# OpenDriveLab/Vista

Hardware: NVIDIA H100
Metric: denoised frames/sec at 25x576x1024, 50 EDM steps; UNet step ms (higher is better)
Workload: dtype f16 (fp32 accumulate, fp32 norms/softmax/sampler state)

## Files before the change

### include/vista_b200.h

```cpp
#ifndef VISTA_B200_H
#define VISTA_B200_H

#include <stdint.h>

#ifdef __cplusplus
extern "C" {
#endif

const char* b200v_last_error(void);
int b200v_version(void);
int b200v_device_info(int32_t* sm_count, int32_t* cc_major, int32_t* cc_minor);

typedef struct b200v_gemm_desc {
  const void* a;
  int64_t lda;
  int64_t tokens;
  int32_t a_mode;
  int32_t W, H, NB;
  int32_t box_w, box_h, box_b;
  int32_t cin;
  int32_t ntaps;
  int32_t dh[9];
  int32_t dw[9];
  const void* b;
  int32_t N;
  int32_t tile_n;
  int32_t bf16;
  void* out;
  int64_t ldo;
  int32_t out_f32;
  int32_t act;
  const float* bias;
  const float* rowvec;
  int64_t ld_rowvec;
  int32_t rv_div, rv_mod;
  const void* res1;
  int64_t ld_res1;
  float s_res1;
  const void* res2;
  int64_t ld_res2;
  float s_res2;
  float s_acc;
  float* stats;
  int64_t stats_ld;
  int32_t stats_col0;
  int32_t h_pad;
} b200v_gemm_desc;

int b200v_gemm(const b200v_gemm_desc* d, void* stream);

int b200v_groupnorm_from_partials(const float* partials, int64_t stats_ld, int32_t n_stats, int32_t frames_per_stat,
                                  int32_t tokens_per_frame, int32_t C, int32_t groups, float eps, float* mean_rstd,
                                  double* raw_sums, void* stream);

int b200v_attention_spatial_v3(const void* q, int64_t ld_q, const void* k, int64_t ld_k, const void* v, int64_t ld_v,
                               void* out, int64_t ld_o, int32_t frames, int32_t seq, int32_t heads, void* stream);


int b200v_attention_spatial_v7(const void* q, int64_t ld_q, const void* k, int64_t ld_k, const void* v, int64_t ld_v,
                               void* out, int64_t ld_o, int32_t frames, int32_t seq, int32_t heads, void* stream);

int b200v_attention_temporal(const void* q, int64_t ld_q, const void* k, int64_t ld_k, const void* v, int64_t ld_v,
                             void* out, int64_t ld_o, int32_t nb, int32_t T, int32_t S, int32_t heads, void* stream);

int b200v_attention_temporal_sharded(const void* q, int64_t ld_q, const void* k, int64_t ld_k, const void* v, int64_t ld_v,
                                     void* out, int64_t ld_o, int32_t nb, int32_t Tq, int32_t T, int32_t S, int32_t heads,
                                     const int64_t* kv_frame_tok, void* stream);

int b200v_groupnorm_chunk(void);
int b200v_groupnorm_chunk_for(int32_t frames, int32_t tokens_per_frame);
int b200v_groupnorm_stats(const void* x, int64_t ldx, int32_t frames, int32_t tokens_per_frame, int32_t C,
                          int32_t groups, int32_t frames_per_stat, float eps, double* partials, int32_t* counters,
                          float* mean_rstd, void* stream);
int b200v_groupnorm_apply(const void* x, int64_t ldx, void* y, int64_t ldy, int32_t frames, int32_t tokens_per_frame,
                          int32_t C, int32_t groups, int32_t frames_per_stat, const float* mean_rstd, const float* gamma,
                          const float* beta, int32_t silu, void* stream);

int b200v_groupnorm_sums(const void* x, int64_t ldx, int32_t frames, int32_t tokens_per_frame, int32_t C, int32_t groups,
                         int32_t frames_per_stat, double* partials, int32_t* counters, double* sums, void* stream);
int b200v_groupnorm_finalize(const double* sums, int32_t n_stat_groups, double count, float eps, float* mean_rstd,
                             void* stream);

int b200v_layernorm(const void* x, int64_t ldx, void* y, int64_t ldy, int64_t tokens, int32_t C, const float* gamma,
                    const float* beta, float eps, const float* addvec, int64_t ld_addvec, int32_t av_div,
                    int32_t av_mod, void* stream);

int b200v_conv3x3_small_cin(const void* x, int32_t cin, const float* w , const float* bias,
                            void* out, int64_t ldo, int32_t NB, int32_t H, int32_t W, int32_t cout, void* stream);
int b200v_conv3x3_small_cout(const void* x, int64_t ldx, int32_t cin, const float* w ,
                             const float* bias, float* out , int32_t NB, int32_t H, int32_t W,
                             int32_t cout, void* stream);

int b200v_im2col_s2(const void* x, int64_t ldx, void* out, int32_t NB, int32_t H, int32_t W, int32_t C, void* stream);
int b200v_im2col_s2_asym(const void* x, int64_t ldx, void* out, int32_t NB, int32_t H, int32_t W, int32_t C, void* stream);
int b200v_upsample2x(const void* x, int64_t ldx, void* out, int64_t ldo, int32_t NB, int32_t H, int32_t W, int32_t C,
                     void* stream);

int b200v_timestep_embedding(const float* t, int32_t n, int32_t dim, float max_period, void* out_f16, int64_t ldo,
                             void* stream);
int b200v_blend_emb(const float* e_plain, const float* e_cond, const float* label, const float* mask, float* emb_f32,
                    void* silu_emb_f16, int32_t rows, int32_t dim, void* stream);

int b200v_sampler_prepare(float* x, const float* cond_frame, const float* mask,
                          const float* concat_u ,
                          const float* concat_c , const float* sigmas, const int32_t* step_idx,
                          void* unet_in_f16 , int64_t ld_in,
                          float* c_noise, int32_t T, int32_t h, int32_t w, void* stream);
int b200v_sampler_update(float* x, const float* net_out ,
                         int64_t ld_net, const float* cond_frame, const float* mask, const float* scales , const float* sigmas, int32_t* step_idx,
                         int32_t num_steps, int32_t T, int32_t h, int32_t w, void* stream);

int b200v_softmax_rows(const float* x, int64_t ld_in, void* y_f16, int64_t ld_out, int64_t rows, int32_t cols,
                       void* stream);
int b200v_time_mix_small(const float* x , int64_t ldx,
                         const float* w , const float* bias,
                         float* out , const int32_t* blend, int32_t T, int32_t HW, int32_t C,
                         int32_t out_frame0, int32_t skip_frames, void* stream);

int b200v_time_mix_small_u8(const float* x, int64_t ldx, const float* w, const float* bias, float* out, uint8_t* out_u8,
                            const int32_t* blend, int32_t T, int32_t HW, int32_t C, int32_t out_frame0,
                            int32_t skip_frames, int32_t keep_f32_from, void* stream);
int b200v_rollout_advance(float* sample, const float* z0, float* samples_z, float* filled, int32_t T, int64_t frame_elems,
                          int32_t dst_frame0, int32_t src_frame0, int32_t n_cond, void* stream);
int b200v_ensemble_reward_scratch(void);
int b200v_ensemble_reward(const float* const* members_dev, int32_t K, int64_t n, double* partial, uint32_t* ticket,
                          float* out2, void* stream);

int b200v_peer_alloc(int64_t bytes, void** ptr, void* handle64);
int b200v_peer_open(const void* handle64, void** ptr);
int b200v_peer_close(void* ptr);
int b200v_peer_free(void* ptr);
int b200v_peer_allreduce_max(void);
int b200v_peer_allreduce_f64(double* data, int32_t n, void* const* windows_dev, int64_t slot_off, int64_t flag_off, int32_t rank,
                             int32_t world, uint32_t* counter, void* stream);
int b200v_peer_put(const void* src, int64_t src_pitch, int64_t rows, int64_t row_bytes, void* const* dsts_dev, int64_t dst_pitch,
                   uint32_t* const* flags_dev, int32_t n_dst, uint32_t* counter, uint32_t* ticket, void* stream);
int b200v_peer_wait(const uint32_t* const* flags_dev, int32_t n, uint32_t* counter, void* stream);

int b200v_clip_preprocess(const float* x, int32_t n, int32_t H, int32_t W, int32_t antialias, void* out, int64_t ldo,
                          int32_t out_f32, void* stream);
int b200v_attention_d80(const void* q, int64_t ld_q, const void* k, int64_t ld_k, const void* v, int64_t ld_v, void* out,
                        int64_t ld_o, int32_t batch, int32_t seq, int32_t heads, void* stream);

int b200v_nchw_to_tokens(const float* x, void* out_f16, int64_t ldo, int32_t NB, int32_t C, int32_t H, int32_t W,
                         void* stream);
int b200v_tokens_to_nchw(const void* x, int32_t x_is_f32, int64_t ldx, float* out, int32_t NB, int32_t C, int32_t H,
                         int32_t W, void* stream);

#ifdef __cplusplus
}
#endif
#endif
```

### vista_b200/clip.py

```python
from __future__ import annotations

import os
from typing import Dict, Optional, Union

import torch
import torch.nn as nn

from . import ops
from .diffusion import instantiate_from_config
from .modules import register_param_tree
from .spec import CLIP_TEXT_LEFTOVERS, ClipConfig, clip_param_specs, clip_preset
from .unet import Lin


class ClipRuntime:

    def __init__(self, cfg: ClipConfig, sd: Dict[str, torch.Tensor], device, prefix: str = "model.visual."):
        assert cfg.patch_size == 14 and cfg.image_size == 224 and cfg.head_width == 80, \
            "the native tower is the 224 px, patch 14, head width 80 ViT"
        self.cfg, self.dev, self.prefix = cfg, torch.device(device), prefix
        self._bufs = {}
        self._sd = sd
        self._pack()
        self._sd = None

    def _t(self, name, dtype=torch.float32):
        return self._sd[self.prefix + name].detach().to(self.dev, dtype).contiguous()

    def _lin(self, w: torch.Tensor, b: Optional[torch.Tensor]) -> Lin:
        return Lin(w.to(torch.float16).contiguous(), b, ops.pick_tile_n(w.shape[0]))

    def _norm(self, p):
        return self._t(f"{p}.weight"), self._t(f"{p}.bias")

    def _pack(self):
        cfg, C = self.cfg, self.cfg.width
        w = self._t("conv1.weight").reshape(C, cfg.patch_k)
        wp = torch.zeros(C, cfg.patch_k_pad, dtype=torch.float32, device=self.dev)
        wp[:, :cfg.patch_k] = w
        self.patch = self._lin(wp, None)
        tok = self._t("positional_embedding").clone()
        tok[0] += self._t("class_embedding")
        self.tok_rowvec = tok.contiguous()
        self.ln_pre = self._norm("ln_pre")
        self.blocks = []
        for i in range(cfg.layers):
            p = f"transformer.resblocks.{i}"
            self.blocks.append(dict(
                ln1=self._norm(f"{p}.ln_1"),
                qkv=self._lin(self._t(f"{p}.attn.in_proj_weight"), self._t(f"{p}.attn.in_proj_bias")),
                out=self._lin(self._t(f"{p}.attn.out_proj.weight"), self._t(f"{p}.attn.out_proj.bias")),
                ln2=self._norm(f"{p}.ln_2"),
                fc=self._lin(self._t(f"{p}.mlp.c_fc.weight"), self._t(f"{p}.mlp.c_fc.bias")),
                proj=self._lin(self._t(f"{p}.mlp.c_proj.weight"), self._t(f"{p}.mlp.c_proj.bias"))))
        self.ln_post = self._norm("ln_post")
        self.proj = self._lin(self._t("proj").t(), None)

    def buf(self, name, rows, cols, dtype=torch.float16):
        key = (name, rows, cols, dtype)
        t = self._bufs.get(key)
        if t is None:
            t = self._bufs[key] = torch.empty(rows, cols, dtype=dtype, device=self.dev)
        return t

    def gemm(self, a, lin: Lin, out, **kw):
        return ops.gemm(a, lin.w, out, bias=lin.b, tile_n=lin.tile_n, **kw)

    def forward(self, x: torch.Tensor, antialias: bool = True) -> torch.Tensor:
        cfg, C = self.cfg, self.cfg.width
        n, L = x.shape[0], cfg.tokens
        M = n * L
        rows = ops.clip_preprocess(x.float().contiguous(), self.buf("c.patch", M, cfg.patch_k_pad), antialias)
        x0 = self.gemm(rows, self.patch, self.buf("c.x1", M, C), rowvec=self.tok_rowvec, rv_mod=L)
        xa = ops.layernorm(x0, self.buf("c.x0", M, C), *self.ln_pre, eps=cfg.ln_eps)
        xb = self.buf("c.x1", M, C)
        h = self.buf("c.h", M, C)
        qkv = self.buf("c.qkv", M, 3 * C)
        o = self.buf("c.o", M, C)
        f = self.buf("c.f", M, cfg.mlp_width)
        for B in self.blocks:
            ops.layernorm(xa, h, *B["ln1"], eps=cfg.ln_eps)
            self.gemm(h, B["qkv"], qkv)
            ops.attention_d80(qkv[:, :C], qkv[:, C:2 * C], qkv[:, 2 * C:], o, n, L, cfg.heads)
            self.gemm(o, B["out"], xb, res1=xa)
            ops.layernorm(xb, h, *B["ln2"], eps=cfg.ln_eps)
            self.gemm(h, B["fc"], f, act=3)
            self.gemm(f, B["proj"], xa, res1=xb)
        cls = self.buf("c.cls", n, C)
        ops.layernorm(xa.view(n, L * C)[:, :C], cls, *self.ln_post, eps=cfg.ln_eps)
        return self.gemm(cls, self.proj, self.buf("c.emb", n, cfg.embed_dim, torch.float32))


class FrozenOpenCLIPImageEmbedder(nn.Module):

    def __init__(self, arch: Union[str, ClipConfig] = "ViT-H-14", version: str = "laion2b_s32b_b79k", device: str = "cuda",
                 max_length: int = 77, freeze: bool = True, antialias: bool = True, ucg_rate: float = 0.0,
                 unsqueeze_dim: bool = False, repeat_to_max_len: bool = False, num_image_crops: int = 0,
                 output_tokens: bool = False, init_device=None):
        super().__init__()
        bad = [k for k, v in dict(arch=not (arch == "ViT-H-14" or isinstance(arch, ClipConfig)), ucg_rate=ucg_rate != 0.0,
                                  num_image_crops=num_image_crops != 0, output_tokens=bool(output_tokens),
                                  unsqueeze_dim=bool(unsqueeze_dim), repeat_to_max_len=bool(repeat_to_max_len)).items() if v]
        if bad:
            raise NotImplementedError(f"vista_b200.clip.FrozenOpenCLIPImageEmbedder: unsupported option(s) {bad}")
        self.b200_config = arch if isinstance(arch, ClipConfig) else clip_preset("vit_h_14")
        self.model = nn.Module()
        self.model.visual = nn.Module()
        register_param_tree(self.model.visual, clip_param_specs(self.b200_config))
        self.device, self.max_length = device, max_length
        self.antialias, self.ucg_rate = antialias, ucg_rate
        self.is_trainable, self.input_key = False, None
        if freeze:
            self.requires_grad_(False)
        self._runtime = None
        self._register_load_state_dict_pre_hook(self._drop_text_leftovers)
        self.register_load_state_dict_post_hook(lambda module, keys: setattr(module, "_runtime", None))

    @staticmethod
    def _drop_text_leftovers(state_dict, prefix, *args):
        for k in CLIP_TEXT_LEFTOVERS:
            state_dict.pop(prefix + "model." + k, None)

    def _apply(self, fn, *args, **kwargs):
        before = tuple((p.device, p.dtype) for p in self.parameters())
        out = super()._apply(fn, *args, **kwargs)
        if tuple((p.device, p.dtype) for p in self.parameters()) != before:
            self._runtime = None
        return out

    def runtime(self, device) -> ClipRuntime:
        if torch.device(device).type != "cuda":
            raise RuntimeError("vista_b200 runs on CUDA (sm_90a) only; there is no CPU fallback")
        if self._runtime is None or self._runtime.dev != torch.device(device):
            self._runtime = ClipRuntime(self.b200_config, self.state_dict(), device)
        return self._runtime

    @torch.no_grad()
    def forward(self, image: torch.Tensor, no_dropout: bool = False):
        if image.dim() == 5:
            raise NotImplementedError("multi-crop input (num_image_crops > 0) is not supported")
        return self.runtime(image.device).forward(image, self.antialias).to(image.dtype)

    def encode(self, image):
        return self(image)


class FrozenOpenCLIPImagePredictionEmbedder(nn.Module):

    def __init__(self, open_clip_embedding_config: Dict, n_cond_frames: int, n_copies: int):
        super().__init__()
        self.n_cond_frames, self.n_copies = n_cond_frames, n_copies
        self.open_clip = instantiate_from_config(open_clip_embedding_config)
        self.is_trainable, self.ucg_rate, self.input_key = False, 0.0, None

    def forward(self, vid: torch.Tensor) -> torch.Tensor:
        z = self.open_clip(vid)
        z = z.reshape(-1, self.n_cond_frames, z.shape[-1])
        return z.repeat_interleave(self.n_copies, dim=0)


def load_open_clip_weights(path: str, prefix: str = "model.") -> Dict[str, torch.Tensor]:
    if not os.path.isfile(path):
        raise FileNotFoundError(path)
    if path.endswith(".safetensors"):
        from safetensors.torch import load_file
        sd = load_file(path)
    else:
        sd = torch.load(path, map_location="cpu", weights_only=True)
        sd = sd.get("state_dict", sd)
    return {prefix + k: v for k, v in sd.items() if not k.startswith("transformer.")}
```

### vista_b200/csrc/gemm_tc.cu

```cuda
#include "gemm_tc.cuh"

namespace vb {
extern template const GemmKern* gemm_variants<32>();
extern template const GemmKern* gemm_variants<64>();
extern template const GemmKern* gemm_variants<96>();
extern template const GemmKern* gemm_variants<128>();
extern template const GemmKern* gemm_variants<160>();
extern template const GemmKern* gemm_variants<192>();
extern template const GemmKern* gemm_variants<224>();
extern template const GemmKern* gemm_variants<256>();
}

extern "C" int b200v_gemm(const b200v_gemm_desc* d, void* stream_) {
  using namespace vb;
  cudaStream_t stream = reinterpret_cast<cudaStream_t>(stream_);
  VB_REQUIRE(d && d->a && d->b && d->out, "b200v_gemm: null pointer");
  VB_REQUIRE(d->cin > 0 && d->cin % 64 == 0, "b200v_gemm: cin=%d must be a positive multiple of 64", d->cin);
  VB_REQUIRE(d->ntaps >= 1 && d->ntaps <= 9, "b200v_gemm: ntaps=%d out of range", d->ntaps);
  VB_REQUIRE(d->N > 0 && d->N % 8 == 0, "b200v_gemm: N=%d must be a multiple of 8", d->N);
  VB_REQUIRE(d->tile_n >= 32 && d->tile_n <= 256 && d->tile_n % 32 == 0, "b200v_gemm: tile_n=%d invalid", d->tile_n);
  VB_REQUIRE(d->lda % 8 == 0 && d->ldo % 8 == 0, "b200v_gemm: lda/ldo must be multiples of 8");
  VB_REQUIRE(d->act >= 0 && d->act <= 3, "b200v_gemm: act=%d invalid", d->act);
  VB_REQUIRE(!(d->act == 2 && (d->tile_n % 64 != 0 || d->N % d->tile_n != 0 || d->out_f32)),
             "b200v_gemm: GEGLU needs tile_n %% 64 == 0, N %% tile_n == 0, 16-bit output");
  VB_REQUIRE(!(d->act == 2 && (d->rowvec || d->res1 || d->res2)), "b200v_gemm: GEGLU epilogue takes bias only");
  VB_REQUIRE(!(d->act == 3 && (d->rowvec || d->res1 || d->res2 || d->bf16 || d->out_f32 || d->stats || getenv("VB_GEMM_GENERIC"))),
             "b200v_gemm: the GELU epilogue takes bias only, fp16 operands and output (compiled variant)");
  VB_REQUIRE(!d->res1 || d->ld_res1 % 8 == 0, "b200v_gemm: ld_res1 must be a multiple of 8");
  VB_REQUIRE(!d->res2 || d->ld_res2 % 8 == 0, "b200v_gemm: ld_res2 must be a multiple of 8");
  VB_REQUIRE(!d->rowvec || (d->ld_rowvec % 4 == 0 && d->rv_div > 0 && d->rv_mod > 0), "b200v_gemm: bad rowvec args");
  VB_REQUIRE((reinterpret_cast<uintptr_t>(d->a) & 15) == 0 && (reinterpret_cast<uintptr_t>(d->b) & 15) == 0 &&
                 (reinterpret_cast<uintptr_t>(d->out) & 15) == 0,
             "b200v_gemm: a/b/out must be 16-byte aligned");

  TGParams p;
  memset(&p, 0, sizeof(p));
  p.a_mode = d->a_mode;
  p.tokens = d->tokens;
  const long long K = (long long)d->ntaps * d->cin;
  CUtensorMap tmA, tmB;
  if (d->a_mode == 0) {
    VB_REQUIRE(d->ntaps == 1 && d->h_pad == 0, "b200v_gemm: linear mode takes one tap and no halo rows");
    VB_REQUIRE(d->tokens > 0 && d->tokens < (1ll << 31) - 256, "b200v_gemm: tokens out of range");
    p.W = (int)d->tokens; p.H = 1; p.NB = 1;
    p.BW = 128; p.BH = 1; p.BB = 1;
    p.tiles_w = (int)((d->tokens + 127) / 128); p.tiles_h = 1;
    p.m_tiles = p.tiles_w;
    uint64_t dims[2] = {(uint64_t)d->cin, (uint64_t)d->tokens};
    uint64_t strides[1] = {(uint64_t)d->lda * 2};
    uint32_t box[2] = {64, 128};
    uint32_t es[2] = {1, 1};
    if (encode_tmap_16bit(&tmA, d->a, 2, dims, strides, box, es, d->bf16)) return 3;
  } else {
    VB_REQUIRE(d->W > 0 && d->H > 0 && d->NB > 0 && (long long)d->W * d->H * d->NB == d->tokens &&
                   d->tokens < (1ll << 31) - 256,
               "b200v_gemm: W*H*NB != tokens (or >= 2^31)");
    VB_REQUIRE(d->box_w > 0 && d->box_h > 0 && d->box_b > 0 && d->box_w * d->box_h * d->box_b == 128,
               "b200v_gemm: box_w*box_h*box_b must be 128");
    p.W = d->W; p.H = d->H; p.NB = d->NB;
    p.BW = d->box_w; p.BH = d->box_h; p.BB = d->box_b;
    p.tiles_w = (d->W + p.BW - 1) / p.BW;
    p.tiles_h = (d->H + p.BH - 1) / p.BH;
    const int tiles_b = (d->NB + p.BB - 1) / p.BB;
    p.m_tiles = p.tiles_w * p.tiles_h * tiles_b;
    VB_REQUIRE(d->h_pad >= 0 && d->h_pad <= 4, "b200v_gemm: h_pad=%d out of range", d->h_pad);
    const uint64_t He = (uint64_t)d->H + 2ull * d->h_pad;
    uint64_t dims[4] = {(uint64_t)d->cin, (uint64_t)d->W, He, (uint64_t)d->NB};
    uint64_t strides[3] = {(uint64_t)d->lda * 2, (uint64_t)d->lda * 2 * d->W, (uint64_t)d->lda * 2 * d->W * He};
    uint32_t box[4] = {64, (uint32_t)p.BW, (uint32_t)p.BH, (uint32_t)p.BB};
    uint32_t es[4] = {1, 1, 1, 1};
    if (encode_tmap_16bit(&tmA, d->a, 4, dims, strides, box, es, d->bf16)) return 3;
  }
  {
    uint64_t dims[2] = {(uint64_t)K, (uint64_t)d->N};
    uint64_t strides[1] = {(uint64_t)K * 2};
    uint32_t box[2] = {64, (uint32_t)d->tile_n};
    uint32_t es[2] = {1, 1};
    if (encode_tmap_16bit(&tmB, d->b, 2, dims, strides, box, es, d->bf16)) return 3;
  }
  p.ntaps = d->ntaps;
  p.kc_per_tap = d->cin / 64;
  for (int i = 0; i < 9; ++i) {
    p.dh[i] = d->dh[i] + (d->a_mode == 1 ? d->h_pad : 0);
    p.dw[i] = d->dw[i];
  }
  p.N = d->N;
  p.n_tiles = (d->N + d->tile_n - 1) / d->tile_n;
  p.stage_bytes = kABytes + ((d->tile_n * 128 + 1023) / 1024) * 1024;
  constexpr int kMaxSmem = 227 * 1024;
  p.nstages = (kMaxSmem - 2048 - kStagingBytes) / p.stage_bytes;
  if (p.nstages > kMaxStages) p.nstages = kMaxStages;
  const long long kMaxLd = (1ll << 31) - 1;
  VB_REQUIRE(d->ldo * (d->out_f32 ? 4 : 2) <= kMaxLd && d->ld_rowvec * 4 <= kMaxLd && d->ld_res1 * 2 <= kMaxLd &&
                 d->ld_res2 * 2 <= kMaxLd,
             "b200v_gemm: row stride too large");
  for (p.bw_sh = 0; (1 << p.bw_sh) < p.BW; ++p.bw_sh) {}
  for (p.bh_sh = 0; (1 << p.bh_sh) < p.BH; ++p.bh_sh) {}
  p.out = d->out; p.ldo_b = (int)(d->ldo * (d->out_f32 ? 4 : 2)); p.out_f32 = d->out_f32; p.act = d->act;
  p.bias = d->bias;
  p.rowvec = d->rowvec; p.ld_rowvec_b = (int)(d->ld_rowvec * 4); p.rv_div = d->rv_div > 0 ? d->rv_div : 1;
  p.rv_mod = d->rv_mod > 0 ? d->rv_mod : 1;
  p.res1 = d->res1; p.ld_res1_b = (int)(d->ld_res1 * 2); p.s_res1 = d->s_res1;
  p.res2 = d->res2; p.ld_res2_b = (int)(d->ld_res2 * 2); p.s_res2 = d->s_res2;
  p.s_acc = d->s_acc;
  VB_REQUIRE(!(d->res2 && !d->res1), "b200v_gemm: res2 without res1");
  p.stats = d->stats; p.stats_ld = (int)d->stats_ld; p.stats_col0 = d->stats_col0;
  if (d->stats) {
    VB_REQUIRE(!d->bf16 && !d->out_f32 && d->act == 0 && !d->res2 && !(d->rowvec && d->res1),
               "b200v_gemm: fused statistics need fp16 output, act 0, <= 1 residual and no rowvec + residual");
    VB_REQUIRE(d->stats_ld >= d->stats_col0 + d->N && d->stats_col0 % 4 == 0 && d->stats_ld % 4 == 0 &&
                   (reinterpret_cast<uintptr_t>(d->stats) & 15) == 0,
               "b200v_gemm: bad stats_ld / stats_col0 / alignment");
    VB_REQUIRE(d->a_mode == 0 || (p.BB == 1 && d->W % p.BW == 0 && d->H % p.BH == 0 && (p.BW == d->W || p.BH == 1)),
               "b200v_gemm: fused statistics need token tiles of 128 consecutive tokens (box %d x %d x %d on %d x %d)",
               p.BW, p.BH, p.BB, d->W, d->H);
  }

  const int smem_bytes = 1024 + 1024 + p.nstages * p.stage_bytes + kStagingBytes;
  int variant = d->bf16 ? 12 : 7;
  if (d->stats) {
    variant = 9 + (d->rowvec ? 2 : (d->res1 ? 1 : 0));
  } else if (!d->bf16 && !d->out_f32 && !getenv("VB_GEMM_GENERIC")) {
    const int nres = (d->res1 ? 1 : 0) + (d->res2 ? 1 : 0);
    if (d->act == 0 && !d->rowvec) variant = nres;
    else if (d->act == 0 && nres <= 1) variant = 3 + nres;
    else if (d->act == 1 && !d->rowvec && nres == 0) variant = 5;
    else if (d->act == 2) variant = 6;
    else if (d->act == 3) variant = 8;
  }
  static const GemmKern* const kByWidth[8] = {gemm_variants<32>(),  gemm_variants<64>(),  gemm_variants<96>(),
                                              gemm_variants<128>(), gemm_variants<160>(), gemm_variants<192>(),
                                              gemm_variants<224>(), gemm_variants<256>()};
  static bool attr_set[64] = {false};
  if (vb::first_use_on_device(attr_set)) {
    for (int w = 0; w < 8; ++w)
      for (int i = 0; i < kGemmVariants; ++i)
        VB_CHECK_CUDA(cudaFuncSetAttribute(kByWidth[w][i], cudaFuncAttributeMaxDynamicSharedMemorySize, kMaxSmem));
  }
  const long long total = (long long)p.m_tiles * p.n_tiles;
  int grid = device_sm_count();
  if (total < grid) grid = (int)total;
  const GemmKern k = kByWidth[d->tile_n / 32 - 1][variant];
  k<<<grid, kGemmThreads, smem_bytes, stream>>>(tmA, tmB, p);
  VB_CHECK_CUDA(cudaGetLastError());
  return 0;
}
```

### vista_b200/csrc/gemm_tc.cuh

```cuda
#pragma once
#include "../../include/vista_b200.h"
#include "host.cuh"
#include "ptx.cuh"

namespace vb {

constexpr int kMaxStages = 8;
constexpr int kABytes = 128 * 64 * 2;
constexpr int kStageBufBytes = 64 * 32 * 4;
constexpr int kStagingBytes = 2 * 2 * kStageBufBytes;
constexpr int kGemmThreads = 384;

struct TGParams {
  int a_mode;
  int W, H, NB;
  int BW, BH, BB;
  int bw_sh, bh_sh;
  int tiles_w, tiles_h;
  int m_tiles, n_tiles;
  int ntaps, kc_per_tap;
  int dh[9], dw[9];
  int N;
  int nstages, stage_bytes;
  long long tokens;
  void* out;
  int ldo_b;
  int out_f32, act;
  const float* bias;
  const float* rowvec;
  int ld_rowvec_b;
  int rv_div, rv_mod;
  const void* res1;
  int ld_res1_b;
  float s_res1;
  const void* res2;
  int ld_res2_b;
  float s_res2;
  float s_acc;
  float* stats;
  int stats_ld, stats_col0;
};

__device__ __forceinline__ float2 unpack2(uint32_t w, int bf16) {
  if (bf16) return make_float2(__uint_as_float(w << 16), __uint_as_float(w & 0xFFFF0000u));
  return __half22float2(*reinterpret_cast<const __half2*>(&w));
}
__device__ __forceinline__ uint32_t pack2(float a, float b, int bf16) {
  if (bf16) {
    __nv_bfloat162 t = __floats2bfloat162_rn(a, b);
    return *reinterpret_cast<uint32_t*>(&t);
  }
  __half2 t = __floats2half2_rn(a, b);
  return *reinterpret_cast<uint32_t*>(&t);
}

template <int TN, bool BF16>
__device__ __forceinline__ void issue_kchunk(float (&acc)[TN / 2], uint64_t adesc, uint64_t bdesc, bool overwrite) {
#pragma unroll
  for (int kk = 0; kk < 4; ++kk)
    wgmma_ss<TN, BF16>(acc, adesc + (uint64_t)(2 * kk), bdesc + (uint64_t)(2 * kk), (overwrite && kk == 0) ? 0 : 1);
}

template <int TN, int ACT_, bool RV_, int NRES_, bool GEN, bool STATS = false, bool BF16 = false>
__global__ void __launch_bounds__(kGemmThreads, 1)
tapgemm_kernel(const __grid_constant__ CUtensorMap tmA, const __grid_constant__ CUtensorMap tmB, const TGParams p) {
  extern __shared__ uint8_t smem_raw[];
  const uint32_t raw = smem_u32(smem_raw);
  uint8_t* smem = smem_raw + (((raw + 1023u) & ~1023u) - raw);
  uint64_t* full = reinterpret_cast<uint64_t*>(smem);
  uint64_t* empty = full + kMaxStages;
  uint8_t* stages = smem + 1024;

  const int warp = threadIdx.x >> 5, lane = threadIdx.x & 31;
  const int KC = p.ntaps * p.kc_per_tap;
  const int total_tiles = p.m_tiles * p.n_tiles;

  if (threadIdx.x == 0) {
    for (int i = 0; i < p.nstages; ++i) {
      mbar_init(&full[i], 1);
      mbar_init(&empty[i], 8);
    }
    fence_barrier_init();
  }
  if (warp == 8 && lane == 0) {
    tma_prefetch_desc(&tmA);
    tma_prefetch_desc(&tmB);
  }
  __syncthreads();

  if (warp >= 8) {
    setmaxnreg_dec<40>();
    if (warp == 8 && lane == 0) {
      int stage = 0;
      uint32_t phase = 0;
      const uint32_t tx = (uint32_t)(kABytes + TN * 128);
      for (int tile = blockIdx.x; tile < total_tiles; tile += gridDim.x) {
        const int m_blk = tile / p.n_tiles, n_blk = tile - m_blk * p.n_tiles;
        const int tw = m_blk % p.tiles_w;
        const int th = (m_blk / p.tiles_w) % p.tiles_h;
        const int tb = m_blk / (p.tiles_w * p.tiles_h);
        const int w0 = tw * p.BW, h0 = th * p.BH, b0 = tb * p.BB;
        const int n0 = n_blk * TN;
        for (int kc = 0; kc < KC; ++kc) {
          mbar_wait_relaxed(&empty[stage], phase ^ 1, 1);
          uint8_t* sA = stages + stage * p.stage_bytes;
          uint8_t* sB = sA + kABytes;
          const int tap = kc / p.kc_per_tap;
          const int c0 = (kc - tap * p.kc_per_tap) * 64;
          mbar_expect_tx(&full[stage], tx);
          if (p.a_mode == 0)
            tma_load_2d(sA, &tmA, &full[stage], c0, w0);
          else
            tma_load_4d(sA, &tmA, &full[stage], c0, w0 + p.dw[tap], h0 + p.dh[tap], b0);
          tma_load_2d(sB, &tmB, &full[stage], kc * 64, n0);
          if (++stage == p.nstages) {
            stage = 0;
            phase ^= 1;
          }
        }
      }
    }
    return;
  }

  setmaxnreg_inc<232>();
  const int wg = warp >> 2, wq = warp & 3;
  const int act = GEN ? p.act : ACT_;
  const bool has_rv = GEN ? (p.rowvec != nullptr) : RV_;
  const bool has_r1 = GEN ? (p.res1 != nullptr) : (NRES_ >= 1);
  const bool has_r2 = GEN ? (p.res2 != nullptr) : (NRES_ >= 2);
  constexpr bool bf16 = BF16;
  const bool f32o = GEN ? (p.out_f32 != 0) : false;
  const bool has_bias = p.bias != nullptr;
  constexpr int half = TN >> 1;
  const int tile_out_cols = (act == 2) ? half : TN;
  const int n_out_total = (act == 2) ? (p.N >> 1) : p.N;
  const int G = tile_out_cols >> 5;
  const int out_es = f32o ? 4 : 2;
  const char* r1p = reinterpret_cast<const char*>(p.res1);
  const char* r2p = reinterpret_cast<const char*>(p.res2);
  const uint64_t desc0 = make_desc_sw128(smem_u32(stages), 16, 1024);
  const uint32_t stage_step = (uint32_t)p.stage_bytes >> 4;
  const uint32_t stg0 = smem_u32(stages + p.nstages * p.stage_bytes) + wg * 2 * kStageBufBytes;
  const int g = lane >> 2, c = lane & 3;
  const int rh = wq & 1, chh = wq >> 1;
  const int ch = lane & 3, rsub = lane >> 2;
  int stage = 0;
  uint32_t phase = 0;
  uint32_t gcount = 0;

  float acc[TN / 2];
  for (int tile = blockIdx.x; tile < total_tiles; tile += gridDim.x) {
    const int m_blk = tile / p.n_tiles, n_blk = tile - m_blk * p.n_tiles;
    int prev = -1;
    for (int kc = 0; kc < KC; ++kc) {
      mbar_wait(&full[stage], phase, 3);
      const uint64_t ad = desc0 + (uint64_t)(stage * stage_step + wg * 512);
      const uint64_t bd = desc0 + (uint64_t)(stage * stage_step + (kABytes >> 4));
      wgmma_fence();
      issue_kchunk<TN, BF16>(acc, ad, bd, kc == 0);
      wgmma_commit();
      if (prev >= 0) {
        wgmma_wait<1>();
        if (lane == 0) mbar_arrive(&empty[prev]);
      }
      prev = stage;
      if (++stage == p.nstages) {
        stage = 0;
        phase ^= 1;
      }
    }
    wgmma_wait<0>();
    if (lane == 0) mbar_arrive(&empty[prev]);
    fence_regs(acc);

    const int r_own = wg * 64 + rh * 32 + lane;
    int token_own, valid_own;
    if (p.a_mode == 0) {
      token_own = m_blk * 128 + r_own;
      valid_own = token_own < p.tokens;
    } else {
      const int tw = m_blk % p.tiles_w;
      const int t2 = m_blk / p.tiles_w;
      const int th = t2 % p.tiles_h;
      const int tb = t2 / p.tiles_h;
      const int ww = r_own & (p.BW - 1), hh = (r_own >> p.bw_sh) & (p.BH - 1), bb = r_own >> (p.bw_sh + p.bh_sh);
      const int w = tw * p.BW + ww, h = th * p.BH + hh, b = tb * p.BB + bb;
      valid_own = (w < p.W) && (h < p.H) && (b < p.NB);
      token_own = (b * p.H + h) * p.W + w;
    }
    if (!valid_own) token_own = 0;
    const uint32_t vrows = __ballot_sync(0xffffffffu, valid_own) >> rsub;
    int tok[4], rvrow[4];
    {
      const int rv_own = has_rv ? (token_own / p.rv_div) % p.rv_mod : 0;
#pragma unroll
      for (int i = 0; i < 4; ++i) {
        tok[i] = __shfl_sync(0xffffffffu, token_own, i * 8 + rsub);
        rvrow[i] = has_rv ? __shfl_sync(0xffffffffu, rv_own, i * 8 + rsub) : 0;
      }
    }
    const int n_out_base = n_blk * tile_out_cols;
#pragma unroll
    for (int k = 0; k < TN / 32; ++k) {
      if (k >= G) break;
      const int c0 = k * 32;
      if (n_out_base + c0 >= n_out_total) break;
      const uint32_t stg = stg0 + (gcount & 1) * kStageBufBytes;
      ++gcount;
      float f[16];
#pragma unroll
      for (int j = 0; j < 16; ++j) f[j] = acc[16 * k + j];
      if (act == 2) {
        float gt[16];
        const int kg = (half >> 5) + k;
#pragma unroll
        for (int j = 0; j < 16; ++j) gt[j] = 0.f;
#pragma unroll
        for (int q = 0; q < TN / 32; ++q)
          if (q == kg) {
#pragma unroll
            for (int j = 0; j < 16; ++j) gt[j] = acc[16 * q + j];
          }
        const int nb = n_blk * TN + c0;
#pragma unroll
        for (int ii = 0; ii < 4; ++ii) {
          float2 bv = make_float2(0.f, 0.f), bg = make_float2(0.f, 0.f);
          if (has_bias) {
            bv = __ldg(reinterpret_cast<const float2*>(p.bias + nb + 8 * ii + 2 * c));
            bg = __ldg(reinterpret_cast<const float2*>(p.bias + nb + half + 8 * ii + 2 * c));
          }
          f[4 * ii + 0] = geglu_fast(f[4 * ii + 0] + bv.x, gt[4 * ii + 0] + bg.x);
          f[4 * ii + 1] = geglu_fast(f[4 * ii + 1] + bv.y, gt[4 * ii + 1] + bg.y);
          f[4 * ii + 2] = geglu_fast(f[4 * ii + 2] + bv.x, gt[4 * ii + 2] + bg.x);
          f[4 * ii + 3] = geglu_fast(f[4 * ii + 3] + bv.y, gt[4 * ii + 3] + bg.y);
        }
      }
#pragma unroll
      for (int ii = 0; ii < 4; ++ii) {
        const int chunk = 2 * ii + (c >> 1), sub = (c & 1) * 8;
#pragma unroll
        for (int hr = 0; hr < 2; ++hr) {
          const int row = wq * 16 + g + 8 * hr;
          asm volatile("st.shared.v2.f32 [%0], {%1, %2};" ::"r"(stg + row * 128 + ((chunk ^ (row & 7)) << 4) + sub),
                       "f"(f[4 * ii + 2 * hr]), "f"(f[4 * ii + 2 * hr + 1])
                       : "memory");
        }
      }
      asm volatile("bar.sync %0, 128;" ::"r"(1 + wg) : "memory");
      {
        const int n = n_out_base + c0 + chh * 16 + ch * 4;
        const bool n_ok = n + 4 <= n_out_total;
        float4 bs = make_float4(0.f, 0.f, 0.f, 0.f);
        float sa = 1.0f;
        if (act != 2) {
          sa = p.s_acc;
          if (has_bias && n_ok) {
            const float4 b4 = __ldg(reinterpret_cast<const float4*>(p.bias + n));
            bs = make_float4(b4.x * sa, b4.y * sa, b4.z * sa, b4.w * sa);
          }
        }
        char* obase = reinterpret_cast<char*>(p.out) + (long long)n * out_es;
        const char* r1base = r1p + (long long)n * 2;
        const char* r2base = r2p + (long long)n * 2;
        const char* rvbase = reinterpret_cast<const char*>(p.rowvec) + (long long)n * 4;
        float cs[4] = {0.f, 0.f, 0.f, 0.f}, cq[4] = {0.f, 0.f, 0.f, 0.f};
        float4 v[4], rv[4];
        uint2 u1[4], u2[4];
#pragma unroll
        for (int i = 0; i < 4; ++i) {
          const int row = rh * 32 + i * 8 + rsub;
          const int chunk = chh * 4 + ch;
          asm volatile("ld.shared.v4.f32 {%0, %1, %2, %3}, [%4];"
                       : "=f"(v[i].x), "=f"(v[i].y), "=f"(v[i].z), "=f"(v[i].w)
                       : "r"(stg + row * 128 + ((chunk ^ (row & 7)) << 4)));
          const bool ok = n_ok && ((vrows >> (8 * i)) & 1u);
          rv[i] = make_float4(0.f, 0.f, 0.f, 0.f);
          u1[i] = make_uint2(0, 0);
          u2[i] = make_uint2(0, 0);
          if (has_rv && ok) rv[i] = __ldg(reinterpret_cast<const float4*>(rvbase + (long long)rvrow[i] * p.ld_rowvec_b));
          if (has_r1 && ok) u1[i] = __ldg(reinterpret_cast<const uint2*>(r1base + (long long)tok[i] * p.ld_res1_b));
          if (has_r2 && ok) u2[i] = __ldg(reinterpret_cast<const uint2*>(r2base + (long long)tok[i] * p.ld_res2_b));
        }
#pragma unroll
        for (int i = 0; i < 4; ++i) {
          const bool ok = n_ok && ((vrows >> (8 * i)) & 1u);
          float4 o = v[i];
          if (act != 2) {
            o.x = fmaf(o.x, sa, bs.x); o.y = fmaf(o.y, sa, bs.y); o.z = fmaf(o.z, sa, bs.z); o.w = fmaf(o.w, sa, bs.w);
            if (has_rv) { o.x += rv[i].x; o.y += rv[i].y; o.z += rv[i].z; o.w += rv[i].w; }
            if (act == 1) { o.x = silu_f(o.x); o.y = silu_f(o.y); o.z = silu_f(o.z); o.w = silu_f(o.w); }
            if (!GEN && act == 3) { o.x = gelu_erf_fast(o.x); o.y = gelu_erf_fast(o.y); o.z = gelu_erf_fast(o.z); o.w = gelu_erf_fast(o.w); }
            if (has_r1) {
              const float2 a = unpack2(u1[i].x, bf16), b = unpack2(u1[i].y, bf16);
              o.x = fmaf(p.s_res1, a.x, o.x); o.y = fmaf(p.s_res1, a.y, o.y);
              o.z = fmaf(p.s_res1, b.x, o.z); o.w = fmaf(p.s_res1, b.y, o.w);
            }
            if (has_r2) {
              const float2 a = unpack2(u2[i].x, bf16), b = unpack2(u2[i].y, bf16);
              o.x = fmaf(p.s_res2, a.x, o.x); o.y = fmaf(p.s_res2, a.y, o.y);
              o.z = fmaf(p.s_res2, b.x, o.z); o.w = fmaf(p.s_res2, b.y, o.w);
            }
          }
          if (STATS && ok) {
            cs[0] += o.x; cs[1] += o.y; cs[2] += o.z; cs[3] += o.w;
            cq[0] = fmaf(o.x, o.x, cq[0]); cq[1] = fmaf(o.y, o.y, cq[1]);
            cq[2] = fmaf(o.z, o.z, cq[2]); cq[3] = fmaf(o.w, o.w, cq[3]);
          }
          char* optr = obase + (long long)tok[i] * p.ldo_b;
          if (f32o) {
            if (ok) *reinterpret_cast<float4*>(optr) = o;
          } else {
            const uint2 pk = make_uint2(pack2(o.x, o.y, bf16), pack2(o.z, o.w, bf16));
            if (ok) *reinterpret_cast<uint2*>(optr) = pk;
          }
        }
        if (STATS) {
#pragma unroll
          for (int off = 4; off < 32; off <<= 1) {
#pragma unroll
            for (int q = 0; q < 4; ++q) {
              cs[q] += __shfl_xor_sync(0xffffffffu, cs[q], off);
              cq[q] += __shfl_xor_sync(0xffffffffu, cq[q], off);
            }
          }
          if (rsub == 0 && n_ok) {
            float* dst = p.stats + (((long long)m_blk * 4 + wg * 2 + rh) * p.stats_ld + p.stats_col0 + n) * 2;
            *reinterpret_cast<float4*>(dst) = make_float4(cs[0], cq[0], cs[1], cq[1]);
            *reinterpret_cast<float4*>(dst + 4) = make_float4(cs[2], cq[2], cs[3], cq[3]);
          }
        }
      }
    }
  }
}

using GemmKern = void (*)(const CUtensorMap, const CUtensorMap, const TGParams);
constexpr int kGemmVariants = 13;

template <int TN>
const GemmKern* gemm_variants() {
  static const GemmKern v[kGemmVariants] = {
      tapgemm_kernel<TN, 0, false, 0, false>,       tapgemm_kernel<TN, 0, false, 1, false>,
      tapgemm_kernel<TN, 0, false, 2, false>,       tapgemm_kernel<TN, 0, true, 0, false>,
      tapgemm_kernel<TN, 0, true, 1, false>,        tapgemm_kernel<TN, 1, false, 0, false>,
      tapgemm_kernel<TN, 2, false, 0, false>,       tapgemm_kernel<TN, 0, true, 2, true>,
      tapgemm_kernel<TN, 3, false, 0, false>,       tapgemm_kernel<TN, 0, false, 0, false, true>,
      tapgemm_kernel<TN, 0, false, 1, false, true>, tapgemm_kernel<TN, 0, true, 0, false, true>,
      tapgemm_kernel<TN, 0, true, 2, true, false, true>};
  return v;
}

}
```

### vista_b200/lib.py

```python
from __future__ import annotations

import ctypes as C
import os
import shutil
import subprocess
import sys
from typing import List, Optional

PKG_DIR = os.path.dirname(os.path.abspath(__file__))
ROOT = os.path.dirname(PKG_DIR)
CSRC = os.path.join(PKG_DIR, "csrc")
LIB_PATH = os.path.join(PKG_DIR, "libvista_b200.so")
SOURCES = ["host.cu", "gemm_tc.cu", "gemm_tn_32_256.cu", "gemm_tn_64_224.cu", "gemm_tn_96_192.cu", "gemm_tn_128_160.cu",
           "attn_tc.cu", "misc.cu", "glue.cu", "peer.cu", "clip.cu"]
NVCC_FLAGS = ["-gencode", "arch=compute_90a,code=sm_90a", "-lineinfo", "-O3", "-std=c++17",
              "-Xcompiler", "-fPIC", "--expt-relaxed-constexpr"]


def _nvcc() -> str:
    for cand in (os.environ.get("NVCC"), shutil.which("nvcc"), "/usr/local/cuda/bin/nvcc"):
        if cand and os.path.isfile(cand):
            return cand
    raise RuntimeError("nvcc not found")


def _stale() -> bool:
    if not os.path.isfile(LIB_PATH):
        return True
    t = os.path.getmtime(LIB_PATH)
    deps = [os.path.join(CSRC, f) for f in os.listdir(CSRC)] + [os.path.join(ROOT, "include", "vista_b200.h")]
    return any(os.path.getmtime(d) > t for d in deps)


def build(force: bool = False, verbose: bool = False) -> str:
    if not force and not _stale():
        return LIB_PATH
    nvcc = _nvcc()
    objdir = os.path.join(PKG_DIR, "build")
    os.makedirs(objdir, exist_ok=True)
    procs = []
    objs = []
    for src in SOURCES:
        obj = os.path.join(objdir, src.replace(".cu", ".o"))
        objs.append(obj)
        cmd = [nvcc] + NVCC_FLAGS + ["-c", os.path.join(CSRC, src), "-o", obj]
        if verbose:
            cmd.insert(1, "-Xptxas=-v")
        procs.append((src, subprocess.Popen(cmd, stdout=subprocess.PIPE, stderr=subprocess.STDOUT, text=True)))
    for src, p in procs:
        out, _ = p.communicate()
        if p.returncode != 0:
            raise RuntimeError(f"nvcc failed on {src}:\n{out}")
        if verbose and out:
            print(out)
    cmd = [nvcc, "-shared", "-o", LIB_PATH] + objs + ["-gencode", "arch=compute_90a,code=sm_90a"]
    r = subprocess.run(cmd, stdout=subprocess.PIPE, stderr=subprocess.STDOUT, text=True)
    if r.returncode != 0:
        raise RuntimeError(f"link failed:\n{r.stdout}")
    return LIB_PATH


class GemmDesc(C.Structure):
    _fields_ = [
        ("a", C.c_void_p), ("lda", C.c_int64), ("tokens", C.c_int64), ("a_mode", C.c_int32),
        ("W", C.c_int32), ("H", C.c_int32), ("NB", C.c_int32),
        ("box_w", C.c_int32), ("box_h", C.c_int32), ("box_b", C.c_int32),
        ("cin", C.c_int32), ("ntaps", C.c_int32), ("dh", C.c_int32 * 9), ("dw", C.c_int32 * 9),
        ("b", C.c_void_p), ("N", C.c_int32), ("tile_n", C.c_int32), ("bf16", C.c_int32),
        ("out", C.c_void_p), ("ldo", C.c_int64), ("out_f32", C.c_int32), ("act", C.c_int32),
        ("bias", C.c_void_p), ("rowvec", C.c_void_p), ("ld_rowvec", C.c_int64),
        ("rv_div", C.c_int32), ("rv_mod", C.c_int32),
        ("res1", C.c_void_p), ("ld_res1", C.c_int64), ("s_res1", C.c_float),
        ("res2", C.c_void_p), ("ld_res2", C.c_int64), ("s_res2", C.c_float),
        ("s_acc", C.c_float),
        ("stats", C.c_void_p), ("stats_ld", C.c_int64), ("stats_col0", C.c_int32), ("h_pad", C.c_int32),
    ]


_P, _I32, _I64, _F = C.c_void_p, C.c_int32, C.c_int64, C.c_float

SIGNATURES = {
    "b200v_version": [],
    "b200v_device_info": [_P, _P, _P],
    "b200v_gemm": [C.POINTER(GemmDesc), _P],
    "b200v_attention_spatial_v3": [_P, _I64, _P, _I64, _P, _I64, _P, _I64, _I32, _I32, _I32, _P],
    "b200v_attention_spatial_v7": [_P, _I64, _P, _I64, _P, _I64, _P, _I64, _I32, _I32, _I32, _P],
    "b200v_attention_temporal": [_P, _I64, _P, _I64, _P, _I64, _P, _I64, _I32, _I32, _I32, _I32, _P],
    "b200v_groupnorm_from_partials": [_P, _I64, _I32, _I32, _I32, _I32, _I32, _F, _P, _P, _P],
    "b200v_groupnorm_chunk": [],
    "b200v_groupnorm_chunk_for": [C.c_int32, C.c_int32],
    "b200v_groupnorm_sums": [_P, _I64, _I32, _I32, _I32, _I32, _I32, _P, _P, _P, _P],
    "b200v_groupnorm_finalize": [_P, _I32, C.c_double, _F, _P, _P],
    "b200v_attention_temporal_sharded": [_P, _I64, _P, _I64, _P, _I64, _P, _I64, _I32, _I32, _I32, _I32, _I32, _P, _P],
    "b200v_groupnorm_stats": [_P, _I64, _I32, _I32, _I32, _I32, _I32, _F, _P, _P, _P, _P],
    "b200v_groupnorm_apply": [_P, _I64, _P, _I64, _I32, _I32, _I32, _I32, _I32, _P, _P, _P, _I32, _P],
    "b200v_layernorm": [_P, _I64, _P, _I64, _I64, _I32, _P, _P, _F, _P, _I64, _I32, _I32, _P],
    "b200v_conv3x3_small_cin": [_P, _I32, _P, _P, _P, _I64, _I32, _I32, _I32, _I32, _P],
    "b200v_conv3x3_small_cout": [_P, _I64, _I32, _P, _P, _P, _I32, _I32, _I32, _I32, _P],
    "b200v_im2col_s2": [_P, _I64, _P, _I32, _I32, _I32, _I32, _P],
    "b200v_im2col_s2_asym": [_P, _I64, _P, _I32, _I32, _I32, _I32, _P],
    "b200v_upsample2x": [_P, _I64, _P, _I64, _I32, _I32, _I32, _I32, _P],
    "b200v_timestep_embedding": [_P, _I32, _I32, _F, _P, _I64, _P],
    "b200v_blend_emb": [_P, _P, _P, _P, _P, _P, _I32, _I32, _P],
    "b200v_sampler_prepare": [_P, _P, _P, _P, _P, _P, _P, _P, _I64, _P, _I32, _I32, _I32, _P],
    "b200v_sampler_update": [_P, _P, _I64, _P, _P, _P, _P, _P, _I32, _I32, _I32, _I32, _P],
    "b200v_softmax_rows": [_P, _I64, _P, _I64, _I64, _I32, _P],
    "b200v_time_mix_small": [_P, _I64, _P, _P, _P, _P, _I32, _I32, _I32, _I32, _I32, _P],
    "b200v_time_mix_small_u8": [_P, _I64, _P, _P, _P, _P, _P, _I32, _I32, _I32, _I32, _I32, _I32, _P],
    "b200v_rollout_advance": [_P, _P, _P, _P, _I32, _I64, _I32, _I32, _I32, _P],
    "b200v_ensemble_reward_scratch": [],
    "b200v_ensemble_reward": [_P, _I32, _I64, _P, _P, _P, _P],
    "b200v_peer_alloc": [_I64, C.POINTER(C.c_void_p), _P],
    "b200v_peer_open": [_P, C.POINTER(C.c_void_p)],
    "b200v_peer_close": [_P],
    "b200v_peer_free": [_P],
    "b200v_peer_allreduce_max": [],
    "b200v_peer_allreduce_f64": [_P, _I32, _P, _I64, _I64, _I32, _I32, _P, _P],
    "b200v_peer_put": [_P, _I64, _I64, _I64, _P, _I64, _P, _I32, _P, _P, _P],
    "b200v_peer_wait": [_P, _I32, _P, _P],
    "b200v_clip_preprocess": [_P, _I32, _I32, _I32, _I32, _P, _I64, _I32, _P],
    "b200v_attention_d80": [_P, _I64, _P, _I64, _P, _I64, _P, _I64, _I32, _I32, _I32, _P],
    "b200v_nchw_to_tokens": [_P, _P, _I64, _I32, _I32, _I32, _I32, _P],
    "b200v_tokens_to_nchw": [_P, _I32, _I64, _P, _I32, _I32, _I32, _I32, _P],
}

_lib: Optional[C.CDLL] = None


def load() -> C.CDLL:
    global _lib
    if _lib is not None:
        return _lib if _tape is None else _Recorder(_lib)
    if os.path.isfile(LIB_PATH) and _stale() and os.environ.get("VISTA_B200_NO_AUTOBUILD") != "1":
        try:
            build()
        except Exception as e:
            sys.stderr.write(f"vista_b200: stale library and rebuild failed: {e}\n")
    if not os.path.isfile(LIB_PATH):
        raise RuntimeError(f"{LIB_PATH} is missing: run `python -c 'import __graft_entry__ as g; g.build()'` "
                           "(there is no fallback path)")
    lib = C.CDLL(LIB_PATH)
    lib.b200v_last_error.restype = C.c_char_p
    lib.b200v_last_error.argtypes = []
    for name, argtypes in SIGNATURES.items():
        fn = getattr(lib, name)
        fn.restype = C.c_int
        fn.argtypes = argtypes
    _lib = lib
    return lib


_tape: Optional[list] = None
_NO_TAPE = {"b200v_peer_alloc", "b200v_peer_open", "b200v_peer_close", "b200v_peer_free", "b200v_peer_allreduce_max", "b200v_ensemble_reward_scratch", "b200v_groupnorm_chunk", "b200v_groupnorm_chunk_for", "b200v_version", "b200v_device_info", "b200v_last_error"}


class _Recorder:
    def __init__(self, lib):
        self._lib = lib

    def __getattr__(self, name):
        fn = getattr(self._lib, name)
        if name in _NO_TAPE:
            return fn

        def call(*args):
            if _tape is not None:
                _tape.append((fn, args))
            return fn(*args)
        return call


def begin_tape():
    global _tape
    _tape = []


def end_tape() -> list:
    global _tape
    t, _tape = _tape, None
    return t


def taping() -> bool:
    return _tape is not None


HOST_PROFILE = None


def tape_host(fn, detail: str = "host"):
    if _tape is not None:
        _tape.append((fn, ()))
    if HOST_PROFILE is not None:
        HOST_PROFILE[0]("nccl+host", detail, 0.0, 0.0)
        r = fn()
        HOST_PROFILE[1]()
        return r
    return fn()


def replay(tape: list):
    for fn, args in tape:
        rc = fn(*args)
        if type(rc) is int and rc != 0:
            check(rc, "replayed call")


def check(rc: int, what: str = ""):
    if rc != 0:
        msg = load().b200v_last_error().decode("utf-8", "replace")
        raise RuntimeError(f"vista_b200 C-ABI call {what} failed (rc={rc}): {msg}")


def exported_symbols() -> List[str]:
    return ["b200v_last_error"] + list(SIGNATURES)


if __name__ == "__main__":
    print(build(force="--force" in sys.argv, verbose="-v" in sys.argv))
```

### vista_b200/ops.py

```python
from __future__ import annotations

import ctypes as C
import os
from typing import Optional, Sequence, Tuple

import torch

from . import lib as _lib

TAPS_3X3 = [(dh, dw) for dh in (-1, 0, 1) for dw in (-1, 0, 1)]
TAPS_T3 = [(-1, 0), (0, 0), (1, 0)]
TAPS_1 = [(0, 0)]


LAUNCHES = 0


def _count(n: int = 1):
    global LAUNCHES
    LAUNCHES += n


TRACE = None


def _trace(name: str, out: torch.Tensor):
    if TRACE is not None:
        torch.cuda.synchronize()
        o = out.double()
        TRACE.append((name, tuple(out.shape), float(o.sum()), float(o.abs().sum())))


PROFILE = None
_prof_open = None


def _prof_begin(family: str, detail: str, flops: float, nbytes: float):
    global _prof_open
    if PROFILE is not None:
        e0 = torch.cuda.Event(enable_timing=True)
        e1 = torch.cuda.Event(enable_timing=True)
        e0.record()
        _prof_open = (family, detail, flops, nbytes, e0, e1)


def _prof_end():
    global _prof_open
    if PROFILE is not None and _prof_open is not None:
        _prof_open[5].record()
        PROFILE.append(_prof_open)
        _prof_open = None


def profile_summary(records):
    fam, det = {}, {}
    for family, detail, flops, nbytes, e0, e1 in records:
        ms = e0.elapsed_time(e1)
        for table, key in ((fam, family), (det, (family, detail))):
            r = table.setdefault(key, dict(ms=0.0, launches=0, flops=0.0, bytes=0.0))
            r["ms"] += ms
            r["launches"] += 1
            r["flops"] += flops
            r["bytes"] += nbytes
    for table in (fam, det):
        for r in table.values():
            r["tflops"] = r["flops"] / (r["ms"] * 1e-3) / 1e12 if r["ms"] > 0 else 0.0
            r["gbs"] = r["bytes"] / (r["ms"] * 1e-3) / 1e9 if r["ms"] > 0 else 0.0
    return fam, det


def _stream() -> int:
    return torch.cuda.current_stream().cuda_stream


def _ptr(t: Optional[torch.Tensor]) -> Optional[int]:
    return None if t is None else t.data_ptr()


def _rows(t: torch.Tensor) -> Tuple[int, int]:
    assert t.dim() == 2 and t.stride(1) == 1, "token-major 2-D view with unit channel stride expected"
    if t.is_cuda and t.device.index != torch.cuda.current_device():
        raise RuntimeError(f"vista_b200: tensor on cuda:{t.device.index} but the current device is cuda:{torch.cuda.current_device()}; "
                           "wrap the call in torch.cuda.device(tensor.device)")
    return t.shape[0], t.stride(0)


def pick_box(W: int, H: int, NB: int) -> Tuple[int, int, int]:
    best, best_cost = None, None
    for bw in (128, 64, 32, 16, 8, 4, 2, 1):
        for bh in (1, 2, 4, 8, 16, 32, 64, 128):
            if bw * bh > 128:
                continue
            bb = 128 // (bw * bh)
            tiles = -(-W // bw) * -(-H // bh) * -(-NB // bb)
            cost = (tiles, -bw)
            if best_cost is None or cost < best_cost:
                best, best_cost = (bw, bh, bb), cost
    return best


def stats_box(W: int, H: int, NB: int) -> Optional[Tuple[int, int, int]]:
    if W >= 128:
        return (128, 1, 1) if W % 128 == 0 else None
    if 128 % W == 0 and H % (128 // W) == 0:
        return (W, 128 // W, 1)
    return None


def pick_tile_n(N: int, geglu: bool = False) -> int:
    step = 64 if geglu else 32
    best, best_cost = None, None
    for tn in range(256, step - 1, -step):
        if geglu and N % tn:
            continue
        tiles = -(-N // tn)
        cost = (round(tiles * (61.0 + 0.22 * max(tn, 128)), 3), tiles, tiles * tn - N)
        if best_cost is None or cost < best_cost:
            best, best_cost = tn, cost
    if best is None:
        raise ValueError(f"no tile_n for N={N} geglu={geglu}")
    return best


def gemm(a: torch.Tensor, w: torch.Tensor, out: torch.Tensor, *, taps: Sequence[Tuple[int, int]] = TAPS_1,
         geom: Optional[Tuple[int, int, int]] = None, bias: Optional[torch.Tensor] = None,
         rowvec: Optional[torch.Tensor] = None, rv_div: int = 1, rv_mod: int = 1,
         res1: Optional[torch.Tensor] = None, s_res1: float = 1.0,
         res2: Optional[torch.Tensor] = None, s_res2: float = 1.0,
         s_acc: float = 1.0, act: int = 0, tile_n: Optional[int] = None, cin: Optional[int] = None,
         stats: Optional[torch.Tensor] = None, h_pad: int = 0) -> torch.Tensor:
    tokens, lda = _rows(a)
    if h_pad:
        assert geom is not None and tokens == geom[2] * (geom[1] + 2 * h_pad) * geom[0]
        tokens = geom[0] * geom[1] * geom[2]
    N, K = w.shape
    ntaps = len(taps)
    cin = cin if cin is not None else K // ntaps
    assert K == ntaps * cin and w.is_contiguous()
    d = _lib.GemmDesc()
    d.a, d.lda, d.tokens = a.data_ptr(), lda, tokens
    if geom is None:
        assert ntaps == 1
        d.a_mode = 0
    else:
        d.a_mode = 1
        d.W, d.H, d.NB = geom
        assert geom[0] * geom[1] * geom[2] == tokens
        d.box_w, d.box_h, d.box_b = pick_box(*geom) if stats is None else stats_box(*geom)
    d.cin, d.ntaps = cin, ntaps
    for i, (dh, dw) in enumerate(taps):
        d.dh[i], d.dw[i] = dh, dw
    d.b, d.N = w.data_ptr(), N
    d.tile_n = tile_n if tile_n is not None else pick_tile_n(N, act == 2)
    d.bf16 = 1 if a.dtype == torch.bfloat16 else 0
    _, ldo = _rows(out)
    d.out, d.ldo, d.out_f32, d.act = out.data_ptr(), ldo, int(out.dtype == torch.float32), act
    d.bias = _ptr(bias)
    if rowvec is not None:
        d.rowvec, d.ld_rowvec, d.rv_div, d.rv_mod = rowvec.data_ptr(), rowvec.stride(0), rv_div, rv_mod
    if res1 is not None:
        d.res1, d.ld_res1, d.s_res1 = res1.data_ptr(), res1.stride(0), s_res1
    if res2 is not None:
        d.res2, d.ld_res2, d.s_res2 = res2.data_ptr(), res2.stride(0), s_res2
    d.s_acc = s_acc
    if stats is not None:
        assert stats.dtype == torch.float32 and stats.dim() == 3 and stats.shape[2] == 2 and stats.stride(2) == 1 \
            and stats.stride(1) == 2 and stats.stride(0) % 2 == 0 and stats.shape[1] >= (N // 2 if act == 2 else N)
        assert stats.shape[0] >= -(-tokens // 128) * 4
        d.stats, d.stats_ld, d.stats_col0 = stats.data_ptr(), stats.stride(0) // 2, 0
    d.h_pad = h_pad
    _count()
    n_out = N // 2 if act == 2 else N
    _prof_begin("gemm", f"M={tokens} N={N} K={K} taps={ntaps} act={act}", 2.0 * tokens * N * K,
                2.0 * tokens * cin + 2.0 * N * K + out.element_size() * tokens * n_out
                + (2.0 * tokens * n_out if res1 is not None else 0) + (2.0 * tokens * n_out if res2 is not None else 0))
    _lib.check(_lib.load().b200v_gemm(C.byref(d), _stream()), "b200v_gemm")
    _prof_end()
    _trace(f"gemm taps={ntaps} act={act} N={N} K={K}", out)
    return out




def attention_spatial(q, k, v, out, frames: int, seq: int, heads: int, impl: Optional[int] = None):
    l = _lib.load()
    fn = l.b200v_attention_spatial_v3 if impl == 3 else l.b200v_attention_spatial_v7
    _count(1)
    _prof_begin("attn_spatial", f"frames={frames} seq={seq} heads={heads}", 4.0 * 64 * heads * frames * seq * seq,
                2.0 * 4 * frames * seq * heads * 64)
    _lib.check(fn(q.data_ptr(), q.stride(0), k.data_ptr(), k.stride(0), v.data_ptr(), v.stride(0), out.data_ptr(),
                  out.stride(0), frames, seq, heads, _stream()), "b200v_attention_spatial")
    _prof_end()
    _trace("attn_spatial", out)
    return out


def attention_d80(q, k, v, out, batch: int, seq: int, heads: int):
    for t in (q, k, v, out):
        _rows(t)
    _count(1)
    _prof_begin("attn_d80", f"batch={batch} seq={seq} heads={heads}", 4.0 * 80 * heads * batch * seq * seq,
                2.0 * 4 * batch * seq * heads * 80)
    _lib.check(_lib.load().b200v_attention_d80(q.data_ptr(), q.stride(0), k.data_ptr(), k.stride(0), v.data_ptr(),
                                               v.stride(0), out.data_ptr(), out.stride(0), batch, seq, heads, _stream()),
               "b200v_attention_d80")
    _prof_end()
    _trace("attn_d80", out)
    return out


def clip_preprocess(x, out, antialias: bool = True):
    n, c, H, W = x.shape
    assert c == 3 and x.dtype == torch.float32 and x.is_contiguous()
    _, ldo = _rows(out)
    assert out.shape[0] == n * 257 and out.dtype in (torch.float16, torch.float32)
    _count(1)
    _prof_begin("other", f"clip_preprocess n={n} {H}x{W}", 0.0, 4.0 * x.numel() + 2.0 * out.numel())
    _lib.check(_lib.load().b200v_clip_preprocess(x.data_ptr(), n, H, W, int(bool(antialias)), out.data_ptr(), ldo,
                                                 int(out.dtype == torch.float32), _stream()), "b200v_clip_preprocess")
    _prof_end()
    _trace("clip_preprocess", out)
    return out


def attention_temporal(q, k, v, out, nb: int, T: int, S: int, heads: int):
    _count(1)
    _prof_begin("attn_temporal", f"nb={nb} T={T} S={S} heads={heads}", 4.0 * 64 * heads * nb * S * T * T,
                2.0 * 4 * nb * T * S * heads * 64)
    _lib.check(_lib.load().b200v_attention_temporal(q.data_ptr(), q.stride(0), k.data_ptr(), k.stride(0),
                                                    v.data_ptr(), v.stride(0), out.data_ptr(), out.stride(0),
                                                    nb, T, S, heads, _stream()), "b200v_attention_temporal")
    _prof_end()
    _trace("attn_temporal", out)
    return out


def groupnorm_scratch(frames: int, tokens_per_frame: int, groups: int = 32) -> int:
    chunk = _lib.load().b200v_groupnorm_chunk_for(frames, tokens_per_frame)
    return frames * (-(-tokens_per_frame // chunk)) * groups * 2


class GNWorkspace:

    def __init__(self, device, max_stats: int = 4096):
        self.device = device
        self.partials = torch.empty(1 << 16, dtype=torch.float64, device=device)
        self.counters = torch.zeros(max_stats, dtype=torch.int32, device=device)
        self._retired = []

    def reserve(self, n_doubles: int):
        if self.partials.numel() < n_doubles:
            self._retired.append(self.partials)
            self.partials = torch.empty(n_doubles, dtype=torch.float64, device=self.device)


_default_ws = {}


def groupnorm(x, y, frames: int, tokens_per_frame: int, gamma, beta, eps: float, silu: bool,
              stats: Optional[torch.Tensor] = None, frames_per_stat: int = 1, groups: int = 32,
              ws: Optional[GNWorkspace] = None):
    Cc = gamma.numel()
    l = _lib.load()
    if ws is None:
        ws = _default_ws.setdefault(x.device, GNWorkspace(x.device))
    if stats is None:
        stats = torch.empty(frames // frames_per_stat, groups, 2, dtype=torch.float32, device=x.device)
    ws.reserve(groupnorm_scratch(frames, tokens_per_frame, groups))
    assert frames // frames_per_stat <= ws.counters.numel()
    _count(2)
    _prof_begin("groupnorm", f"tokens={frames * tokens_per_frame} C={Cc} fps={frames_per_stat}", 0.0,
                2.0 * 3 * frames * tokens_per_frame * Cc)
    _lib.check(l.b200v_groupnorm_stats(x.data_ptr(), x.stride(0), frames, tokens_per_frame, Cc, groups,
                                       frames_per_stat, eps, ws.partials.data_ptr(), ws.counters.data_ptr(),
                                       stats.data_ptr(), _stream()), "b200v_groupnorm_stats")
    _lib.check(l.b200v_groupnorm_apply(x.data_ptr(), x.stride(0), y.data_ptr(), y.stride(0), frames,
                                       tokens_per_frame, Cc, groups, frames_per_stat, stats.data_ptr(),
                                       gamma.data_ptr(), beta.data_ptr(), int(silu), _stream()),
               "b200v_groupnorm_apply")
    _prof_end()
    _trace(f"groupnorm fps={frames_per_stat}", y)
    return y


def groupnorm_from_partials(partials, frames: int, tokens_per_frame: int, Cc: int, eps: float, stats: Optional[torch.Tensor],
                            frames_per_stat: int = 1, groups: int = 32, raw_sums: Optional[torch.Tensor] = None):
    _count(1)
    _prof_begin("groupnorm", f"from_partials tokens={frames * tokens_per_frame} C={Cc} fps={frames_per_stat}", 0.0,
                4.0 * 2 * (frames * tokens_per_frame // 32) * Cc)
    assert partials.stride(1) == 2 and partials.stride(2) == 1 and partials.shape[1] == Cc
    _lib.check(_lib.load().b200v_groupnorm_from_partials(partials.data_ptr(), partials.stride(0) // 2, frames // frames_per_stat,
                                                         frames_per_stat, tokens_per_frame, Cc, groups, eps, _ptr(stats),
                                                         _ptr(raw_sums), _stream()), "b200v_groupnorm_from_partials")
    _prof_end()
    return stats


def groupnorm_apply(x, y, frames: int, tokens_per_frame: int, gamma, beta, silu: bool, stats: torch.Tensor,
                    frames_per_stat: int = 1, groups: int = 32):
    Cc = gamma.numel()
    _count(1)
    _prof_begin("groupnorm", f"apply tokens={frames * tokens_per_frame} C={Cc} fps={frames_per_stat}", 0.0,
                2.0 * 2 * frames * tokens_per_frame * Cc)
    _lib.check(_lib.load().b200v_groupnorm_apply(x.data_ptr(), x.stride(0), y.data_ptr(), y.stride(0), frames,
                                                 tokens_per_frame, Cc, groups, frames_per_stat, stats.data_ptr(),
                                                 gamma.data_ptr(), beta.data_ptr(), int(silu), _stream()),
               "b200v_groupnorm_apply")
    _prof_end()
    _trace(f"groupnorm(apply) fps={frames_per_stat}", y)
    return y


def groupnorm_sums(x, frames: int, tokens_per_frame: int, Cc: int, sums: torch.Tensor, frames_per_stat: int,
                   groups: int = 32, ws: Optional[GNWorkspace] = None):
    l = _lib.load()
    if ws is None:
        ws = _default_ws.setdefault(x.device, GNWorkspace(x.device))
    ws.reserve(groupnorm_scratch(frames, tokens_per_frame, groups))
    _count(1)
    _prof_begin("groupnorm", f"sums tokens={frames * tokens_per_frame} C={Cc} fps={frames_per_stat}", 0.0,
                2.0 * frames * tokens_per_frame * Cc)
    _lib.check(l.b200v_groupnorm_sums(x.data_ptr(), x.stride(0), frames, tokens_per_frame, Cc, groups, frames_per_stat,
                                      ws.partials.data_ptr(), ws.counters.data_ptr(), sums.data_ptr(), _stream()),
               "b200v_groupnorm_sums")
    _prof_end()
    return sums


def groupnorm_finalize_apply(x, y, frames: int, tokens_per_frame: int, gamma, beta, eps: float, silu: bool,
                             sums: torch.Tensor, count: float, stats: torch.Tensor, frames_per_stat: int, groups: int = 32):
    l = _lib.load()
    Cc = gamma.numel()
    _count(2)
    _prof_begin("groupnorm", f"finalize+apply tokens={frames * tokens_per_frame} C={Cc} fps={frames_per_stat}", 0.0,
                2.0 * 2 * frames * tokens_per_frame * Cc)
    _lib.check(l.b200v_groupnorm_finalize(sums.data_ptr(), sums.numel() // 2, float(count), eps, stats.data_ptr(), _stream()),
               "b200v_groupnorm_finalize")
    _lib.check(l.b200v_groupnorm_apply(x.data_ptr(), x.stride(0), y.data_ptr(), y.stride(0), frames, tokens_per_frame, Cc,
                                       groups, frames_per_stat, stats.data_ptr(), gamma.data_ptr(), beta.data_ptr(),
                                       int(silu), _stream()), "b200v_groupnorm_apply")
    _prof_end()
    return y


def attention_temporal_sharded(q, k, v, out, nb: int, Tq: int, T: int, S: int, heads: int, kv_frame_tok: torch.Tensor):
    _count(1)
    _prof_begin("attn_temporal", f"sharded nb={nb} Tq={Tq} T={T} S={S} heads={heads}", 4.0 * 64 * heads * nb * S * Tq * T,
                2.0 * (2 * nb * Tq + 2 * nb * T) * S * heads * 64)
    _lib.check(_lib.load().b200v_attention_temporal_sharded(q.data_ptr(), q.stride(0), k.data_ptr(), k.stride(0),
                                                            v.data_ptr(), v.stride(0), out.data_ptr(), out.stride(0),
                                                            nb, Tq, T, S, heads, kv_frame_tok.data_ptr(), _stream()),
               "b200v_attention_temporal_sharded")
    _prof_end()
    return out


def layernorm(x, y, gamma, beta, eps: float = 1e-5, addvec=None, av_div: int = 1, av_mod: int = 1):
    tokens, ldx = _rows(x)
    _count(1)
    _prof_begin("layernorm", f"tokens={tokens} C={gamma.numel()}", 0.0, 2.0 * 2 * tokens * gamma.numel())
    _lib.check(_lib.load().b200v_layernorm(x.data_ptr(), ldx, y.data_ptr(), y.stride(0), tokens, gamma.numel(),
                                           gamma.data_ptr(), beta.data_ptr(), eps, _ptr(addvec),
                                           addvec.stride(0) if addvec is not None else 0, av_div, av_mod,
                                           _stream()), "b200v_layernorm")
    _prof_end()
    _trace("layernorm", y)
    return y


def conv3x3_small_cin(x8, cin: int, w, bias, out, NB: int, H: int, W: int):
    _count(1)
    _prof_begin("other", "conv3x3_small_cin", 0.0, 0.0)
    _lib.check(_lib.load().b200v_conv3x3_small_cin(x8.data_ptr(), cin, w.data_ptr(), _ptr(bias), out.data_ptr(),
                                                   out.stride(0), NB, H, W, w.shape[0], _stream()),
               "b200v_conv3x3_small_cin")
    _prof_end()
    return out


def conv3x3_small_cout(x, w, bias, out, NB: int, H: int, W: int):
    _count(1)
    _prof_begin("other", "conv3x3_small_cout", 0.0, 0.0)
    _lib.check(_lib.load().b200v_conv3x3_small_cout(x.data_ptr(), x.stride(0), w.shape[1], w.data_ptr(), _ptr(bias),
                                                    out.data_ptr(), NB, H, W, w.shape[0], _stream()),
               "b200v_conv3x3_small_cout")
    _prof_end()
    return out


def im2col_s2(x, out, NB: int, H: int, W: int, Cc: int):
    _count(1)
    _prof_begin("other", "im2col_s2", 0.0, 0.0)
    _lib.check(_lib.load().b200v_im2col_s2(x.data_ptr(), x.stride(0), out.data_ptr(), NB, H, W, Cc, _stream()),
               "b200v_im2col_s2")
    _prof_end()
    return out


def im2col_s2_asym(x, out, NB: int, H: int, W: int, Cc: int):
    _count(1)
    _prof_begin("other", "im2col_s2_asym", 0.0, 0.0)
    _lib.check(_lib.load().b200v_im2col_s2_asym(x.data_ptr(), x.stride(0), out.data_ptr(), NB, H, W, Cc, _stream()),
               "b200v_im2col_s2_asym")
    _prof_end()
    return out


def upsample2x(x, out, NB: int, H: int, W: int, Cc: int):
    _count(1)
    _prof_begin("other", "upsample2x", 0.0, 0.0)
    _lib.check(_lib.load().b200v_upsample2x(x.data_ptr(), x.stride(0), out.data_ptr(), out.stride(0), NB, H, W, Cc,
                                            _stream()), "b200v_upsample2x")
    _prof_end()
    return out


def timestep_embedding(t, out, dim: int, max_period: float = 10000.0):
    _count(1)
    _prof_begin("other", "timestep_embedding", 0.0, 0.0)
    _lib.check(_lib.load().b200v_timestep_embedding(t.data_ptr(), t.numel(), dim, max_period, out.data_ptr(),
                                                    out.stride(0), _stream()), "b200v_timestep_embedding")
    _prof_end()
    return out


def blend_emb(e_plain, e_cond, label, mask, emb, silu_emb):
    rows, dim = e_plain.shape
    _count(1)
    _prof_begin("other", "blend_emb", 0.0, 0.0)
    _lib.check(_lib.load().b200v_blend_emb(e_plain.data_ptr(), _ptr(e_cond), _ptr(label), _ptr(mask), _ptr(emb),
                                           _ptr(silu_emb), rows, dim, _stream()), "b200v_blend_emb")
    _prof_end()


def sampler_prepare(x, cond_frame, mask, concat_u, concat_c, sigmas, step_idx, unet_in, c_noise, T, h, w):
    _count(1)
    _prof_begin("other", "sampler_prepare", 0.0, 0.0)
    _lib.check(_lib.load().b200v_sampler_prepare(x.data_ptr(), _ptr(cond_frame), _ptr(mask), _ptr(concat_u),
                                                 _ptr(concat_c), sigmas.data_ptr(), step_idx.data_ptr(), unet_in.data_ptr(),
                                                 unet_in.stride(0), _ptr(c_noise), T, h, w, _stream()), "b200v_sampler_prepare")
    _prof_end()


def sampler_update(x, net_out, cond_frame, mask, scales, sigmas, step_idx, num_steps, T, h, w):
    _count(2)
    _prof_begin("other", "sampler_update", 0.0, 0.0)
    _lib.check(_lib.load().b200v_sampler_update(x.data_ptr(), net_out.data_ptr(), net_out.stride(0), _ptr(cond_frame), _ptr(mask),
                                                scales.data_ptr(), sigmas.data_ptr(), step_idx.data_ptr(), num_steps,
                                                T, h, w, _stream()), "b200v_sampler_update")
    _prof_end()


def nchw_to_tokens(x, out, NB, Cc, H, W):
    _count(1)
    _prof_begin("other", "nchw_to_tokens", 0.0, 0.0)
    _lib.check(_lib.load().b200v_nchw_to_tokens(x.data_ptr(), out.data_ptr(), out.stride(0), NB, Cc, H, W, _stream()),
               "b200v_nchw_to_tokens")
    _prof_end()
    return out


def tokens_to_nchw(x, out, NB, Cc, H, W):
    _count(1)
    _prof_begin("other", "tokens_to_nchw", 0.0, 0.0)
    _lib.check(_lib.load().b200v_tokens_to_nchw(x.data_ptr(), int(x.dtype == torch.float32), x.stride(0),
                                                out.data_ptr(), NB, Cc, H, W, _stream()), "b200v_tokens_to_nchw")
    _prof_end()
    return out


def softmax_rows(x, y):
    rows, cols = x.shape
    _count(1)
    _prof_begin("other", "softmax_rows", 0.0, 0.0)
    _lib.check(_lib.load().b200v_softmax_rows(x.data_ptr(), x.stride(0), y.data_ptr(), y.stride(0), rows, cols, _stream()),
               "b200v_softmax_rows")
    _prof_end()
    return y


def time_mix_small(x, w, bias, out, blend, T, HW, Cc, out_frame0=0, skip_frames=0):
    _count(1)
    _prof_begin("other", "time_mix_small", 0.0, 0.0)
    _lib.check(_lib.load().b200v_time_mix_small(x.data_ptr(), x.stride(0), w.data_ptr(), _ptr(bias), out.data_ptr(), _ptr(blend),
                                                T, HW, Cc, out_frame0, skip_frames, _stream()), "b200v_time_mix_small")
    _prof_end()
    return out


def time_mix_small_u8(x, w, bias, out, out_u8, blend, T, HW, Cc, out_frame0=0, skip_frames=0, keep_f32_from=-1):
    assert out_u8.dtype == torch.uint8 and out_u8.is_contiguous()
    _count(1)
    _prof_begin("other", "time_mix_small_u8", 0.0, 0.0)
    _lib.check(_lib.load().b200v_time_mix_small_u8(x.data_ptr(), x.stride(0), w.data_ptr(), _ptr(bias), out.data_ptr(),
                                                   out_u8.data_ptr(), _ptr(blend), T, HW, Cc, out_frame0, skip_frames,
                                                   keep_f32_from, _stream()), "b200v_time_mix_small_u8")
    _prof_end()
    return out_u8


def rollout_advance(sample, z0, samples_z, filled, dst_frame0: int, src_frame0: int, n_cond: int):
    T = sample.shape[0]
    E = sample[0].numel()
    assert sample.is_contiguous() and samples_z.is_contiguous() and sample.dtype == torch.float32
    assert filled is None or (filled.is_contiguous() and filled.shape == sample.shape)
    assert samples_z.shape[0] >= dst_frame0 + T
    _count(1)
    _lib.check(_lib.load().b200v_rollout_advance(sample.data_ptr(), _ptr(z0), samples_z.data_ptr(), _ptr(filled), T, E,
                                                 dst_frame0, src_frame0, n_cond, _stream()), "b200v_rollout_advance")
    return samples_z


_reward_ws = {}


def ensemble_reward(members: Sequence[torch.Tensor]) -> torch.Tensor:
    K, n, dev = len(members), members[0].numel(), members[0].device
    assert all(m.is_contiguous() and m.dtype == torch.float32 and m.numel() == n for m in members)
    l = _lib.load()
    ws = _reward_ws.get(dev)
    if ws is None:
        ws = _reward_ws[dev] = (torch.empty(l.b200v_ensemble_reward_scratch(), dtype=torch.float64, device=dev),
                                torch.zeros(1, dtype=torch.int32, device=dev))
    ptrs = torch.tensor([m.data_ptr() for m in members], dtype=torch.int64).to(dev)
    out = torch.empty(2, dtype=torch.float32, device=dev)
    _count(1)
    _lib.check(l.b200v_ensemble_reward(ptrs.data_ptr(), K, n, ws[0].data_ptr(), ws[1].data_ptr(), out.data_ptr(), _stream()),
               "b200v_ensemble_reward")
    out._keepalive = (ptrs, tuple(members))
    return out


def peer_allreduce_f64(data: torch.Tensor, windows_dev: torch.Tensor, slot_off: int, flag_off: int, rank: int, world: int,
                       counter: torch.Tensor):
    assert data.dtype == torch.float64 and data.is_contiguous()
    _count(1)
    _prof_begin("peer", f"allreduce_f64 n={data.numel()}", 0.0, 8.0 * data.numel() * world)
    _lib.check(_lib.load().b200v_peer_allreduce_f64(data.data_ptr(), data.numel(), windows_dev.data_ptr(), slot_off, flag_off,
                                                    rank, world, counter.data_ptr(), _stream()), "b200v_peer_allreduce_f64")
    _prof_end()
    return data


def peer_put(src_ptr: int, src_pitch: int, rows: int, row_bytes: int, dsts_dev: torch.Tensor, dst_pitch: int,
             flags_dev: torch.Tensor, n_dst: int, counter: torch.Tensor, ticket: torch.Tensor, detail: str = ""):
    _count(1)
    _prof_begin("peer", f"put {detail} bytes={rows * row_bytes} x{n_dst}", 0.0, float(rows * row_bytes * (n_dst + 1)))
    _lib.check(_lib.load().b200v_peer_put(src_ptr, src_pitch, rows, row_bytes, dsts_dev.data_ptr(), dst_pitch, flags_dev.data_ptr(),
                                          n_dst, counter.data_ptr(), ticket.data_ptr(), _stream()), "b200v_peer_put")
    _prof_end()


def peer_wait(flags_dev: torch.Tensor, n: int, counter: torch.Tensor, detail: str = ""):
    _count(1)
    _prof_begin("peer", f"wait {detail}", 0.0, 0.0)
    _lib.check(_lib.load().b200v_peer_wait(flags_dev.data_ptr(), n, counter.data_ptr(), _stream()), "b200v_peer_wait")
    _prof_end()
```

### vista_b200/sharded.py

```python
from __future__ import annotations

from typing import Dict, List, Optional

import torch
import torch.distributed as dist

from . import lib as _lib
from . import ops
from .parallel import frame_shards, halo_neighbours
from .spec import UNetConfig
from .unet import Lin, UNetRuntime


class HaloExchange:

    def __init__(self, group, prev: Optional[int], nxt: Optional[int], first, last):
        self.copies, self.p2p, self.pending = [], [], []
        if prev is not None:
            stage, src, send, recv = first
            self.copies.append((stage, src))
            self.p2p.append(dist.P2POp(dist.isend, send, prev, group))
            self.p2p.append(dist.P2POp(dist.irecv, recv, prev, group))
        if nxt is not None:
            stage, src, send, recv = last
            self.copies.append((stage, src))
            self.p2p.append(dist.P2POp(dist.isend, send, nxt, group))
            self.p2p.append(dist.P2POp(dist.irecv, recv, nxt, group))

    def start(self):
        for dst, src in self.copies:
            dst.copy_(src)
        self.pending = list(dist.batch_isend_irecv(self.p2p)) if self.p2p else []

    def wait(self):
        for r in self.pending:
            r.wait()
        self.pending = []


class ShardedUNetRuntime(UNetRuntime):
    has_collectives = True

    def __init__(self, cfg: UNetConfig, sd: Dict[str, torch.Tensor], device, num_frames: int = 25, group=None):
        self.group = group
        self.world = dist.get_world_size(group)
        self.rank = dist.get_rank(group)
        self.T_full = num_frames
        self.shards = frame_shards(num_frames, self.world)
        self.t0, self.t1 = self.shards[self.rank]
        self.T_pad = max(b - a for a, b in self.shards)
        super().__init__(cfg, sd, device, num_frames=self.t1 - self.t0)
        prev, nxt = halo_neighbours(self.rank, self.world)
        to_global = (lambda r: r) if group is None else (lambda r: dist.get_global_rank(group, r))
        self.prev = None if prev is None else to_global(prev)
        self.next = None if nxt is None else to_global(nxt)
        self._tap_w: Dict[int, tuple] = {}
        self._frame_tables: Dict[tuple, torch.Tensor] = {}
        self.comm_bytes = 0
        self.win = None
        self._ext: Dict[tuple, tuple] = {}
        self._ext_of: Dict[int, tuple] = {}
        self._peer_state: Dict[str, dict] = {}

    def attach_window(self, win):
        self.win = win
        self.has_collectives = False
        granks = list(range(self.world)) if self.group is None else dist.get_process_group_ranks(self.group)
        wranks = list(range(win.world)) if win.group is None else dist.get_process_group_ranks(win.group)
        self.wr = [wranks.index(g) for g in granks]
        W = self.world
        amax = ops._lib.load().b200v_peer_allreduce_max()
        self._ar = dict(slot=win.region("gn.ar.slots", 2 * 16 * amax * 8), flag=win.region("gn.ar.flags", 2 * 16 * 4), counter=win.counter("gn.ar"))
        self._ar["windows"] = win.ptr_array([win.bases[r] for r in self.wr])
        hf = win.region("halo.flags", 1024)
        me = self.rank
        st = dict(c_put_prev=win.counter("halo.put_prev"), t_put_prev=win.counter("halo.ticket_prev"),
                  c_put_next=win.counter("halo.put_next"), t_put_next=win.counter("halo.ticket_next"), c_wait=win.counter("halo.wait"))
        wait = []
        if me > 0:
            st["flag_on_prev"] = win.ptr_array([win.remote(self.wr[me - 1], hf + 256)])
            wait.append(win.local(hf))
        if me < W - 1:
            st["flag_on_next"] = win.ptr_array([win.remote(self.wr[me + 1], hf)])
            wait.append(win.local(hf + 256))
        st["wait"] = win.ptr_array(wait) if wait else None
        st["n_wait"] = len(wait)
        self._halo = st
        kf = win.region("kv.flags", 16 * 256)
        peers = [r for r in range(W) if r != me]
        self._kv = dict(flag_off=kf, peers=peers, c_put=win.counter("kv.put"), t_put=win.counter("kv.ticket"), c_wait=win.counter("kv.wait"),
                        flags_remote=win.ptr_array([win.remote(self.wr[r], kf + me * 256) for r in peers]),
                        flags_local=win.ptr_array([win.local(kf + r * 256) for r in peers]))

    def _peer_on(self, nb: int) -> bool:
        return self.win is not None and nb == 1

    def _ext_buffer(self, hw: int, Cc: int, which: int):
        key = (hw, Cc, which)
        hit = self._ext.get(key)
        if hit is None:
            fb = hw * Cc * 2
            off = self.win.region(f"ext.{hw}.{Cc}.{which}", (self.T_pad + 2) * fb)
            ext = self.win.tensor(off, ((self.T + 2) * hw, Cc), torch.float16)
            mid = ext[hw:(self.T + 1) * hw]
            hit = self._ext[key] = (ext, mid, off, fb)
            self._ext_of[mid.data_ptr()] = hit
        return hit

    def set_conditioning(self, context: torch.Tensor, y: torch.Tensor):
        Tf, T = self.T_full, self.T
        nb = context.shape[0] // Tf
        ctx = context.reshape(nb, Tf, -1)
        yy = y.reshape(nb, Tf, -1)
        local_ctx = ctx[:, self.t0:self.t1].reshape(nb * T, 1, -1)
        local_y = yy[:, self.t0:self.t1].reshape(nb * T, -1)
        first_ctx = ctx[:, :1].reshape(nb, 1, -1)
        super().set_conditioning(local_ctx, local_y)
        cond = self.cond
        t16 = self.buf("cond.tctx", nb, first_ctx.numel() // nb)
        t16.copy_(first_ctx.reshape(nb, -1))
        frames = torch.arange(Tf, dtype=torch.float32, device=self.dev)
        for t in self.plan.transformers():
            L = self.layers[t.prefix]
            cond["tm"][t.prefix] = self._attn2_const(L["tattn2"], t16, f"cond.tm.{t.prefix}")
            temb = self.buf("cond.temb_full", Tf, t.ch)
            ops.timestep_embedding(frames, temb, t.ch)
            full = self._mlp(temb, *L["pos"], f"cond.posfull.{t.prefix}")
            cond["pos"][t.prefix] = full[self.t0:self.t1]

    def _fuse_stats(self, B, h, w) -> bool:
        if self._peer_on(B // self.T):
            return super()._fuse_stats(B, h, w)
        return False

    def _gn_temporal(self, x, y, B, hw, norm, eps, silu, idx, fps, part=None):
        nb = B // fps
        Cc = norm[0].numel()
        sums = self.buf(f"gn.sums{nb}", nb * self.cfg.num_groups, 2, torch.float64)
        if part is not None:
            ops.groupnorm_from_partials(part, B, hw, Cc, eps, None, fps, self.cfg.num_groups, raw_sums=sums)
        else:
            ops.groupnorm_sums(x, B, hw, Cc, sums, fps, groups=self.cfg.num_groups, ws=self.gn_ws)
        if self._peer_on(nb):
            ar = self._ar
            ops.peer_allreduce_f64(sums.view(-1), ar["windows"], ar["slot"], ar["flag"], self.rank, self.world, ar["counter"])
            which = 0 if y.data_ptr() == self.buf("rb.a1", y.shape[0], y.shape[1]).data_ptr() else 1
            y = self._ext_buffer(hw, Cc, which)[1]
        else:
            _lib.tape_host(lambda: dist.all_reduce(sums, group=self.group), "gn-sum all_reduce")
        self.comm_bytes += sums.numel() * 8
        count = float(Cc // self.cfg.num_groups) * hw * self.T_full
        return ops.groupnorm_finalize_apply(x, y, B, hw, norm[0], norm[1], eps, silu, sums, count,
                                            self.gn_stats[idx, :nb], fps, groups=self.cfg.num_groups)

    def _tap_weights(self, lin: Lin):
        key = lin.w.data_ptr()
        tw = self._tap_w.get(key)
        if tw is None:
            Cc = lin.w.shape[1] // 3
            tw = (Lin(lin.w[:, :Cc].contiguous(), None, lin.tile_n), Lin(lin.w[:, 2 * Cc:].contiguous(), None, lin.tile_n))
            self._tap_w[key] = tw
        return tw

    def _tconv(self, a, lin: Lin, out, hw: int, nb: int, **epi):
        T, Cc = self.T, a.shape[1]
        ext = self._ext_of.get(a.data_ptr()) if self._peer_on(nb) else None
        if ext is not None:
            ext_t, _, off, fb = ext
            h, win, me = self._halo, self.win, self.rank
            if me > 0:
                t_prev = self.shards[me - 1][1] - self.shards[me - 1][0]
                dst = self._peer_ptrs(("hp", off, fb), lambda: [win.remote(self.wr[me - 1], off + (t_prev + 1) * fb)])
                ops.peer_put(a.data_ptr(), fb, 1, fb, dst, fb, h["flag_on_prev"], 1, h["c_put_prev"], h["t_put_prev"], "halo->prev")
            if me < self.world - 1:
                dst = self._peer_ptrs(("hn", off, fb), lambda: [win.remote(self.wr[me + 1], off)])
                ops.peer_put(a.data_ptr() + (T - 1) * fb, fb, 1, fb, dst, fb, h["flag_on_next"], 1, h["c_put_next"], h["t_put_next"], "halo->next")
            if h["n_wait"]:
                ops.peer_wait(h["wait"], h["n_wait"], h["c_wait"], "halo")
            self.comm_bytes += fb * ((me > 0) + (me < self.world - 1))
            return self.gemm(ext_t, lin, out, taps=ops.TAPS_T3, geom=(hw, T, nb), h_pad=1, **epi)
        send_first = self.buf("halo.sf", nb * hw, Cc)
        send_last = self.buf("halo.sl", nb * hw, Cc)
        recv_prev = self.buf("halo.rp", nb * hw, Cc)
        recv_next = self.buf("halo.rn", nb * hw, Cc)
        a4 = a.reshape(nb, T, hw, Cc) if a.is_contiguous() else None
        av = a4 if a4 is not None else a.as_strided((nb, T, hw, Cc), (T * hw * a.stride(0), hw * a.stride(0), a.stride(0), 1))
        halo = HaloExchange(self.group, self.prev, self.next,
                            first=(send_first.view(nb, hw, Cc), av[:, 0], send_first, recv_prev),
                            last=(send_last.view(nb, hw, Cc), av[:, T - 1], send_last, recv_next))
        start_halo, wait_halo = halo.start, halo.wait
        _lib.tape_host(start_halo, "halo copy + isend/irecv")
        self.comm_bytes += 2 * nb * hw * Cc * 2 * ((self.prev is not None) + (self.next is not None))
        self.gemm(a, lin, out, taps=ops.TAPS_T3, geom=(hw, T, nb), **epi)
        _lib.tape_host(wait_halo, "halo wait")
        s_acc = epi.get("s_acc", 1.0)
        w0, w2 = self._tap_weights(lin)
        ov = out.as_strided((nb, T, hw, out.shape[1]), (T * hw * out.stride(0), hw * out.stride(0), out.stride(0), 1))
        for b in range(nb):
            if self.prev is not None:
                o = ov[b, 0]
                self.gemm(recv_prev[b * hw:(b + 1) * hw], w0, o, s_acc=s_acc, res1=o)
            if self.next is not None:
                o = ov[b, T - 1]
                self.gemm(recv_next[b * hw:(b + 1) * hw], w2, o, s_acc=s_acc, res1=o)
        return out

    def _peer_ptrs(self, key, make):
        t = self._peer_state.get(key)
        if t is None:
            t = self._peer_state[key] = self.win.ptr_array(make())
        return t

    def _frame_table(self, nb: int, hw: int) -> torch.Tensor:
        key = (nb, hw)
        tab = self._frame_tables.get(key)
        if tab is None:
            rows = []
            for b in range(nb):
                for t in range(self.T_full):
                    r = next(i for i, (a, e) in enumerate(self.shards) if a <= t < e)
                    tl = t - self.shards[r][0]
                    rows.append(((r * nb + b) * self.T_pad + tl) * hw)
            tab = torch.tensor(rows, dtype=torch.int64, device=self.dev)
            self._frame_tables[key] = tab
        return tab

    def _kv_direct(self, nb: int) -> bool:
        return nb == 1 or self.T == self.T_pad

    def _svt_tqkv(self, n, L, M: int, Cc: int, nb: int, hw: int):
        if not self._kv_direct(nb):
            return super()._svt_tqkv(n, L, M, Cc, nb, hw)
        lin = L["tqkv"]
        sub = self._tap_w.get(("qkv", lin.w.data_ptr()))
        if sub is None:
            sub = (Lin(lin.w[:Cc], None, ops.pick_tile_n(Cc)), Lin(lin.w[Cc:], None, ops.pick_tile_n(2 * Cc)))
            self._tap_w[("qkv", lin.w.data_ptr())] = sub
        qkv = self.buf("tr.qkv", M, 3 * Cc)
        send = self._kv_recv(nb, hw, Cc)[1] if self._peer_on(nb) else self.buf("kv.send", nb * self.T_pad * hw, 2 * Cc)
        self.gemm(n, sub[0], qkv[:, :Cc])
        self.gemm(n, sub[1], send[:M])
        return qkv

    def _kv_recv(self, nb: int, hw: int, Cc: int):
        key = ("kv", hw, Cc)
        hit = self._peer_state.get(key)
        if hit is None:
            slab = self.T_pad * hw * 2 * Cc * 2
            off = self.win.region("kv.recv", self.world * slab)
            recv = self.win.tensor(off, (self.world * self.T_pad * hw, 2 * Cc), torch.float16)
            mine = recv[self.rank * self.T_pad * hw:(self.rank + 1) * self.T_pad * hw]
            dsts = self.win.ptr_array([self.win.remote(self.wr[r], off + self.rank * slab) for r in self._kv["peers"]])
            hit = self._peer_state[key] = (recv, mine, slab, off, dsts)
        return hit

    def _attn_temporal(self, qkv, o, nb: int, hw: int, heads: int, Cc: int):
        T, Tp, W = self.T, self.T_pad, self.world
        if self._peer_on(nb):
            recv, mine, slab, off, dsts = self._kv_recv(nb, hw, Cc)
            kv = self._kv
            nbytes = T * hw * 2 * Cc * 2
            ops.peer_put(mine.data_ptr(), nbytes, 1, nbytes, dsts, nbytes, kv["flags_remote"], len(kv["peers"]), kv["c_put"], kv["t_put"],
                         f"kv C={Cc} hw={hw}")
            ops.peer_wait(kv["flags_local"], len(kv["peers"]), kv["c_wait"], "kv")
            self.comm_bytes += nbytes * len(kv["peers"])
            tab = self._frame_table(nb, hw)
            return ops.attention_temporal_sharded(qkv[:, :Cc], recv[:, :Cc], recv[:, Cc:], o, nb, T, self.T_full, hw, heads, tab)
        send = self.buf("kv.send", nb * Tp * hw, 2 * Cc)
        recv = self.buf("kv.recv", W * nb * Tp * hw, 2 * Cc)
        if not self._kv_direct(nb):
            kv = qkv.as_strided((nb, T, hw, 2 * Cc), (T * hw * qkv.stride(0), hw * qkv.stride(0), qkv.stride(0), 1),
                                qkv.storage_offset() + Cc)
            dst = send.view(nb, Tp, hw, 2 * Cc)[:, :T]
            _lib.tape_host(lambda: dst.copy_(kv), "kv staging copy")
        _lib.tape_host(lambda: dist.all_gather_into_tensor(recv, send, group=self.group), f"kv all_gather C={Cc} hw={hw}")
        self.comm_bytes += recv.numel() * 2
        tab = self._frame_table(nb, hw)
        return ops.attention_temporal_sharded(qkv[:, :Cc], recv[:, :Cc], recv[:, Cc:], o, nb, T, self.T_full, hw, heads, tab)


def gather_latent(x_local: torch.Tensor, num_frames: int, group=None) -> torch.Tensor:
    world = dist.get_world_size(group)
    shards = frame_shards(num_frames, world)
    pad = max(b - a for a, b in shards)
    buf = x_local.new_zeros((pad,) + tuple(x_local.shape[1:]))
    buf[: x_local.shape[0]] = x_local
    out = x_local.new_empty((world * pad,) + tuple(x_local.shape[1:]))
    dist.all_gather_into_tensor(out, buf, group=group)
    parts = out.reshape(world, pad, *x_local.shape[1:])
    return torch.cat([parts[r, : b - a] for r, (a, b) in enumerate(shards)], dim=0)


from .vae import DecoderRuntime, _decode_chunks


class ShardedDecoderRuntime(DecoderRuntime):
    def __init__(self, cfg, sd, device, group=None):
        super().__init__(cfg, sd, device)
        self.group = group
        self.world, self.rank = dist.get_world_size(group), dist.get_rank(group)
        self._to_global = (lambda r: r) if group is None else (lambda r: dist.get_global_rank(group, r))
        self._tap_w: Dict[int, tuple] = {}
        self.T_full, self.prev, self.next = 0, None, None

    def _set_chunk(self, n_frames: int):
        self.T_full = n_frames
        self.shards = frame_shards(n_frames, min(self.world, n_frames))
        self.active = self.rank < len(self.shards)
        self.t0, self.t1 = self.shards[self.rank] if self.active else (0, 0)
        last = len(self.shards) - 1
        self.prev = self._to_global(self.rank - 1) if self.active and self.rank > 0 else None
        self.next = self._to_global(self.rank + 1) if self.active and self.rank < last else None

    def _fuse_stats(self, T, h, w) -> bool:
        return False

    def _gn(self, x, y, T, hw, norm, eps, idx, fps=1, part=None, silu=True):
        if fps == 1:
            return super()._gn(x, y, T, hw, norm, eps, idx, fps, silu=silu)
        Cc, G = norm[0].numel(), self.cfg.num_groups
        sums = self.buf("gn.sums", G, 2, torch.float64)
        ops.groupnorm_sums(x, T, hw, Cc, sums, T, groups=G, ws=self.gn_ws)
        dist.all_reduce(sums, group=self.group)
        count = float(Cc // G) * hw * self.T_full
        return ops.groupnorm_finalize_apply(x, y, T, hw, norm[0], norm[1], eps, True, sums, count,
                                            self.gn_stats[idx, :1], T, groups=G)

    def _tap_weights(self, lin: Lin):
        key = lin.w.data_ptr()
        tw = self._tap_w.get(key)
        if tw is None:
            Cc = lin.w.shape[1] // 3
            tw = (Lin(lin.w[:, :Cc].contiguous(), None, lin.tile_n), Lin(lin.w[:, 2 * Cc:].contiguous(), None, lin.tile_n))
            self._tap_w[key] = tw
        return tw

    def _tconv(self, a, lin: Lin, out, T: int, hw: int, **epi):
        Cc = a.shape[1]
        send_first, send_last = self.buf("halo.sf", hw, Cc), self.buf("halo.sl", hw, Cc)
        recv_prev, recv_next = self.buf("halo.rp", hw, Cc), self.buf("halo.rn", hw, Cc)
        halo = HaloExchange(self.group, self.prev, self.next,
                            first=(send_first, a[:hw], send_first, recv_prev),
                            last=(send_last, a[(T - 1) * hw:T * hw], send_last, recv_next))
        halo.start()
        self.gemm(a, lin, out, taps=ops.TAPS_T3, geom=(hw, T, 1), **epi)
        halo.wait()
        s_acc = epi.get("s_acc", 1.0)
        w0, w2 = self._tap_weights(lin)
        if self.prev is not None:
            o = out[:hw]
            self.gemm(recv_prev, w0, o, s_acc=s_acc, res1=o)
        if self.next is not None:
            o = out[(T - 1) * hw:T * hw]
            self.gemm(recv_next, w2, o, s_acc=s_acc, res1=o)
        return out

    def _resblock(self, L, x, T, h, w, name):
        rb = L["spec"]
        hw, M, gi = h * w, T * h * w, L["gn_idx"]
        a1 = self._gn(x, self.buf("d.a1", M, rb.cin), T, hw, L["gn1"], 1e-6, gi)
        h1 = self.gemm(a1, L["conv1"], self.buf("d.h1", M, rb.cout), taps=ops.TAPS_3X3, geom=(w, h, T))
        a2 = self._gn(h1, self.buf("d.a2", M, rb.cout), T, hw, L["gn2"], 1e-6, gi + 1)
        xs = x if L["skip"] is None else self.gemm(x, L["skip"], self.buf("d.xs", M, rb.cout))
        xsp = self.gemm(a2, L["conv2"], self.buf("d.xsp", M, rb.cout), taps=ops.TAPS_3X3, geom=(w, h, T), res1=xs)
        a3 = self._gn(xsp, self.buf("d.a1", M, rb.cout), T, hw, L["tgn1"], 1e-5, gi + 2, fps=T)
        h2 = self._tconv(a3, L["tconv1"], self.buf("d.h1", M, rb.cout), T, hw)
        a4 = self._gn(h2, self.buf("d.a2", M, rb.cout), T, hw, L["tgn2"], 1e-5, gi + 3, fps=T)
        out = self.buf(name, M, rb.cout)
        self._tconv(a4, L["tconv2"], out, T, hw, s_acc=L["alpha"], res1=xsp)
        return out

    def forward_local(self, z_tokens: torch.Tensor, T: int, h: int, w: int) -> torch.Tensor:
        cfg = self.cfg
        if not hasattr(self, "gn_stats") or self.gn_stats.shape[1] < max(T, 1):
            self._bufs.setdefault(("gn.retired",), []).append(getattr(self, "gn_stats", None))
            self.gn_stats = torch.zeros(self.n_gn, max(T, 1), cfg.num_groups, 2, dtype=torch.float32, device=self.dev)
        if not hasattr(self, "gn_ws"):
            self.gn_ws = ops.GNWorkspace(self.dev)
        up_total = 2 ** (len(cfg.ch_mult) - 1)
        self.gn_ws.reserve(ops.groupnorm_scratch(T, h * w * up_total * up_total, cfg.num_groups))
        x = ops.conv3x3_small_cin(z_tokens, cfg.z_channels, self.conv_in_w, self.conv_in_b,
                                  self.buf("d.in", T * h * w, self.plan.block_in), T, h, w)
        x = self._resblock(self.res[self.plan.mid[0].prefix], x, T, h, w, "d.r0")
        x, _ = self._attn(x, T, h, w)
        x = self._resblock(self.res[self.plan.mid[1].prefix], x, T, h, w, "d.r1")
        for blocks, up, ch in self.plan.levels:
            for bi, rb in enumerate(blocks):
                x = self._resblock(self.res[rb.prefix], x, T, h, w, f"d.r{bi % 2}")
            if up is not None:
                xu = ops.upsample2x(x, self.buf("d.up", T * 4 * h * w, ch), T, h, w, ch)
                h, w = 2 * h, 2 * w
                x = self.gemm(xu, self.ups[up], self.buf("d.upc", T * h * w, ch), taps=ops.TAPS_3X3, geom=(w, h, T))
        hw, M = h * w, T * h * w
        a = ops.groupnorm(x, self.buf("d.a1", M, self.plan.final_ch), T, hw, self.norm_out[0], self.norm_out[1], 1e-6,
                          True, self.gn_stats[self.norm_out_idx, :T], groups=cfg.num_groups, ws=self.gn_ws)
        y_ext = self.buf("d.yext", (T + 2) * hw, 8, torch.float32)
        y_ext.zero_()
        y = y_ext[hw:(T + 1) * hw]
        self.gemm(a, self.out_conv, y, taps=ops.TAPS_3X3, geom=(w, h, T))
        send_first, send_last = self.buf("halo.yf", hw, 8, torch.float32), self.buf("halo.yl", hw, 8, torch.float32)
        halo = HaloExchange(self.group, self.prev, self.next,
                            first=(send_first, y[:hw], send_first, y_ext[:hw]),
                            last=(send_last, y[(T - 1) * hw:], send_last, y_ext[(T + 1) * hw:]))
        halo.start()
        halo.wait()
        ext = torch.empty(T + 2, cfg.out_ch, h, w, dtype=torch.float32, device=self.dev)
        ops.time_mix_small(y_ext, self.tmix_w, self.tmix_b, ext, None, T + 2, hw, cfg.out_ch, 0, 0)
        return ext[1:T + 1]


def decode_first_stage_sharded(rt: ShardedDecoderRuntime, z: torch.Tensor, scale_factor: float = 0.18215,
                               n_samples: Optional[int] = 14, overlap: int = 3, chunk_ids=None, world_group=None,
                               owners=None) -> torch.Tensor:
    F_, zc, h, w = z.shape
    n_samples = F_ if n_samples is None else n_samples
    up = 2 ** (len(rt.cfg.ch_mult) - 1)
    H, W = h * up, w * up
    out = torch.empty(F_, rt.cfg.out_ch, H, W, dtype=torch.float32, device=z.device)
    zs = (z.float() / scale_factor).contiguous()
    chunks = _decode_chunks(F_, n_samples, overlap)
    if any(nov > n or o0 != f0 for f0, n, o0, nov in chunks):
        raise NotImplementedError("decode_first_stage_sharded: chunks shorter than the overlap")
    for ci, (f0, n, o0, nov) in enumerate(chunks):
        if chunk_ids is not None and ci not in chunk_ids:
            chunk = torch.empty(n, rt.cfg.out_ch, H, W, dtype=torch.float32, device=z.device)
            dist.broadcast(chunk, src=owners[ci], group=world_group)
            if nov:
                out[o0:o0 + nov] = 0.5 * (out[o0:o0 + nov] + chunk[:nov])
            out[o0 + nov:o0 + n] = chunk[nov:]
            continue
        rt._set_chunk(n)
        pad = max(b - a for a, b in rt.shards)
        mine = torch.zeros(pad, rt.cfg.out_ch, H, W, dtype=torch.float32, device=z.device)
        if rt.active:
            T = rt.t1 - rt.t0
            tok = rt.buf("d.z", T * h * w, 8)
            tok.zero_()
            ops.nchw_to_tokens(zs[f0 + rt.t0:f0 + rt.t1].contiguous(), tok, T, zc, h, w)
            mine[:T] = rt.forward_local(tok, T, h, w)
        else:
            raise NotImplementedError("decode_first_stage_sharded: more ranks than frames in a chunk")
        gathered = torch.empty(rt.world * pad, rt.cfg.out_ch, H, W, dtype=torch.float32, device=z.device)
        dist.all_gather_into_tensor(gathered, mine, group=rt.group)
        parts = gathered.reshape(rt.world, pad, rt.cfg.out_ch, H, W)
        chunk = torch.cat([parts[r, : b - a] for r, (a, b) in enumerate(rt.shards)], dim=0)
        if chunk_ids is not None:
            dist.broadcast(chunk, src=owners[ci], group=world_group)
        if nov:
            out[o0:o0 + nov] = 0.5 * (out[o0:o0 + nov] + chunk[:nov])
        out[o0 + nov:o0 + n] = chunk[nov:]
    return out


def decode_groups(world_group, n_chunks: int, max_group: int = 4):
    ranks = list(range(dist.get_world_size())) if world_group is None else dist.get_process_group_ranks(world_group)
    W = len(ranks)
    G = max(1, min(n_chunks, W // 2))
    per = min(max_group, W // G)
    groups = [ranks[i * (W // G): i * (W // G) + per] for i in range(G)]
    pgs = [dist.new_group(g) for g in groups]
    me = dist.get_rank()
    mine = next((i for i, g in enumerate(groups) if me in g), None)
    return groups, pgs, mine


def decode_first_stage_grouped(cfg, make_rt, cache: dict, z: torch.Tensor, scale_factor: float = 0.18215,
                               n_samples: Optional[int] = 14, overlap: int = 3, world_group=None) -> torch.Tensor:
    F_ = z.shape[0]
    n_s = F_ if n_samples is None else n_samples
    chunks = _decode_chunks(F_, n_s, overlap)
    key = ("groups", len(chunks))
    if key not in cache:
        groups, pgs, mine = decode_groups(world_group, len(chunks))
        cache[key] = (groups, pgs, mine, make_rt(pgs[mine]) if mine is not None else None)
    groups, pgs, mine, rt = cache[key]
    G = len(groups)
    owners = {ci: groups[ci % G][0] for ci in range(len(chunks))}
    if rt is None:
        import types
        return decode_first_stage_sharded(types.SimpleNamespace(cfg=cfg), z, scale_factor, n_samples, overlap, chunk_ids=set(),
                                          world_group=world_group, owners=owners)
    mine_ids = {ci for ci in range(len(chunks)) if ci % G == mine}
    return decode_first_stage_sharded(rt, z, scale_factor, n_samples, overlap, chunk_ids=mine_ids, world_group=world_group, owners=owners)
```

### vista_b200/unet.py

```python
from __future__ import annotations

import math
import os
from dataclasses import dataclass
from typing import Dict, List, Optional, Tuple

import torch

from . import ops
from .spec import ConvSpec, ResBlockSpec, SVTSpec, UNetConfig, build_unet_plan
from .weights import conv_weight_to_taps, permute_geglu


@dataclass
class Lin:
    w: torch.Tensor
    b: Optional[torch.Tensor]
    tile_n: int
    geglu: bool = False


FUSE_GN_STATS = os.environ.get("VISTA_B200_FUSE_GN", "1") != "0"

IN_PAD = 64


def padded_input_rows(rows: int, device) -> torch.Tensor:
    return torch.zeros(rows, IN_PAD, dtype=torch.float16, device=device)[:, :8]


class UNetRuntime:
    has_collectives = False

    def __init__(self, cfg: UNetConfig, sd: Dict[str, torch.Tensor], device, num_frames: int = 25):
        self.cfg, self.dev, self.T = cfg, torch.device(device), num_frames
        self.plan = build_unet_plan(cfg)
        self._bufs: Dict[Tuple, torch.Tensor] = {}
        self._sd = sd
        self._pack()
        self._sd = None
        self.cond = None

    def _f32(self, name):
        return self._sd[name].detach().to(self.dev, torch.float32).contiguous()

    def _lin(self, prefix, geglu=False, bias=True, tile_n=None) -> Lin:
        w = self._sd[f"{prefix}.weight"].detach().to(self.dev, torch.float32)
        b = self._f32(f"{prefix}.bias") if bias and f"{prefix}.bias" in self._sd else None
        if w.dim() > 2:
            w = conv_weight_to_taps(w)
        tn = tile_n or ops.pick_tile_n(w.shape[0], geglu)
        if geglu:
            w, b = permute_geglu(w, b, tn)
        return Lin(w.to(torch.float16).contiguous(), b, tn, geglu)

    def _norm(self, prefix):
        return self._f32(f"{prefix}.weight"), self._f32(f"{prefix}.bias")

    def _attn2_weights(self, p):
        return dict(v=self._lin(f"{p}.to_v", bias=False),
                    va=self._lin(f"{p}.v_adapter_action_control", bias=False) if f"{p}.v_adapter_action_control.weight" in self._sd else None,
                    out=self._lin(f"{p}.to_out.0"))

    def _pack(self):
        cfg, sd = self.cfg, self._sd
        self.time_embed = (self._lin("time_embed.0"), self._lin("time_embed.2"))
        self.cond_embed = (self._lin("cond_time_stack_embed.0"), self._lin("cond_time_stack_embed.2"))
        self.label_emb = (self._lin("label_emb.0.0"), self._lin("label_emb.0.2"))
        self.layers: Dict[str, dict] = {}
        emb_w, emb_b, off = [], [], 0
        self.n_gn = 0
        for layer in self.plan.all_layers():
            if isinstance(layer, ResBlockSpec):
                p = layer.prefix
                L = dict(spec=layer, gn1=self._norm(f"{p}.in_layers.0"), conv1=self._lin(f"{p}.in_layers.2"),
                         gn2=self._norm(f"{p}.out_layers.0"), conv2=self._lin(f"{p}.out_layers.3"),
                         skip=self._lin(f"{p}.skip_connection") if layer.has_skip else None,
                         tgn1=self._norm(f"{p}.time_stack.in_layers.0"), tconv1=self._lin(f"{p}.time_stack.in_layers.2"),
                         tgn2=self._norm(f"{p}.time_stack.out_layers.0"), tconv2=self._lin(f"{p}.time_stack.out_layers.3"),
                         alpha=float(torch.sigmoid(sd[f"{p}.time_mixer.mix_factor"].float()).item()),
                         gn_idx=self.n_gn)
                self.n_gn += 4
                for key, q in (("emb_off", f"{p}.emb_layers.1"), ("embt_off", f"{p}.time_stack.emb_layers.1")):
                    L[key] = off
                    emb_w.append(sd[f"{q}.weight"].detach().to(self.dev, torch.float32))
                    emb_b.append(sd[f"{q}.bias"].detach().to(self.dev, torch.float32))
                    off += layer.cout
                self.layers[p] = L
            elif isinstance(layer, SVTSpec):
                p, s, m = layer.prefix, f"{layer.prefix}.transformer_blocks.0", f"{layer.prefix}.time_stack.0"

                def qkv(a):
                    w = torch.cat([sd[f"{a}.to_q.weight"], sd[f"{a}.to_k.weight"], sd[f"{a}.to_v.weight"]], 0)
                    w = w.detach().to(self.dev, torch.float16).contiguous()
                    return Lin(w, None, ops.pick_tile_n(w.shape[0]))

                L = dict(spec=layer, norm=self._norm(f"{p}.norm"), proj_in=self._lin(f"{p}.proj_in"),
                         ln1=self._norm(f"{s}.norm1"), qkv=qkv(f"{s}.attn1"), out=self._lin(f"{s}.attn1.to_out.0"),
                         attn2=self._attn2_weights(f"{s}.attn2"),
                         ln3=self._norm(f"{s}.norm3"), ff1=self._lin(f"{s}.ff.net.0.proj", geglu=True), ff2=self._lin(f"{s}.ff.net.2"),
                         ln_in=self._norm(f"{m}.norm_in"), ffin1=self._lin(f"{m}.ff_in.net.0.proj", geglu=True),
                         ffin2=self._lin(f"{m}.ff_in.net.2"),
                         tln1=self._norm(f"{m}.norm1"), tqkv=qkv(f"{m}.attn1"), tout=self._lin(f"{m}.attn1.to_out.0"),
                         tattn2=self._attn2_weights(f"{m}.attn2"),
                         tln3=self._norm(f"{m}.norm3"), tff1=self._lin(f"{m}.ff.net.0.proj", geglu=True), tff2=self._lin(f"{m}.ff.net.2"),
                         pos=(self._lin(f"{p}.time_pos_embed.0"), self._lin(f"{p}.time_pos_embed.2")),
                         alpha=float(torch.sigmoid(sd[f"{p}.time_mixer.mix_factor"].float()).item()),
                         proj_out=self._lin(f"{p}.proj_out"), gn_idx=self.n_gn)
                self.n_gn += 1
                self.layers[p] = L
            elif isinstance(layer, ConvSpec):
                if layer.kind == "conv_in":
                    w = self._f32(f"{layer.prefix}.weight")
                    wp = torch.zeros(w.shape[0], IN_PAD, 3, 3, dtype=torch.float32, device=self.dev)
                    wp[:, :w.shape[1]] = w
                    b = self._f32(f"{layer.prefix}.bias")
                    self.layers[layer.prefix] = dict(spec=layer, w=w, b=b,
                                                     conv=Lin(conv_weight_to_taps(wp).to(torch.float16).contiguous(), b,
                                                              ops.pick_tile_n(w.shape[0])))
                else:
                    self.layers[layer.prefix] = dict(spec=layer, conv=self._lin(layer.prefix))
        self.emb_all = Lin(torch.cat(emb_w, 0).to(torch.float16).contiguous(), torch.cat(emb_b, 0).contiguous(),
                           ops.pick_tile_n(off))
        self.emb_total = off
        self.out_norm = self._norm("out.0")
        self.out_gn_idx = self.n_gn
        self.n_gn += 1
        ow = conv_weight_to_taps(self._f32("out.2.weight"))
        oc = ow.shape[0]
        assert oc <= 8
        w8 = torch.zeros(8, ow.shape[1], dtype=torch.float16, device=self.dev)
        w8[:oc] = ow.to(torch.float16)
        b8 = torch.zeros(8, dtype=torch.float32, device=self.dev)
        b8[:oc] = self._f32("out.2.bias")
        self.out_conv = Lin(w8.contiguous(), b8, 32)

    def buf(self, name: str, rows: int, cols: int, dtype=torch.float16) -> torch.Tensor:
        key = (name, rows, cols, dtype)
        t = self._bufs.get(key)
        if t is None:
            t = torch.empty(rows, cols, dtype=dtype, device=self.dev)
            self._bufs[key] = t
        return t

    def gemm(self, a, lin: Lin, out, **kw):
        return ops.gemm(a, lin.w, out, bias=lin.b, tile_n=lin.tile_n, act=2 if lin.geglu else kw.pop("act", 0), **kw)

    def _gn(self, x, y, B, hw, norm, eps, silu, idx, fps=1, part=None):
        if fps != 1:
            return self._gn_temporal(x, y, B, hw, norm, eps, silu, idx, fps, part)
        stats = self.gn_stats[idx, : B // fps]
        if part is None:
            return ops.groupnorm(x, y, B, hw, norm[0], norm[1], eps, silu, stats, frames_per_stat=fps,
                                 groups=self.cfg.num_groups, ws=self.gn_ws)
        ops.groupnorm_from_partials(part, B, hw, norm[0].numel(), eps, stats, fps, self.cfg.num_groups)
        return ops.groupnorm_apply(x, y, B, hw, norm[0], norm[1], silu, stats, fps, self.cfg.num_groups)

    def _gn_temporal(self, x, y, B, hw, norm, eps, silu, idx, fps, part=None):
        stats = self.gn_stats[idx, : B // fps]
        if part is None:
            return ops.groupnorm(x, y, B, hw, norm[0], norm[1], eps, silu, stats, frames_per_stat=fps,
                                 groups=self.cfg.num_groups, ws=self.gn_ws)
        ops.groupnorm_from_partials(part, B, hw, norm[0].numel(), eps, stats, fps, self.cfg.num_groups)
        return ops.groupnorm_apply(x, y, B, hw, norm[0], norm[1], silu, stats, fps, self.cfg.num_groups)

    def part(self, name: str, tokens: int, cols: int) -> torch.Tensor:
        key = ("part." + name, tokens, cols)
        t = self._bufs.get(key)
        if t is None:
            t = self._bufs[key] = torch.zeros(-(-tokens // 128) * 4, cols, 2, dtype=torch.float32, device=self.dev)
        return t

    def _ln(self, x, y, norm, **kw):
        return ops.layernorm(x, y, norm[0], norm[1], 1e-5, **kw)

    def _mlp(self, x16, l0: Lin, l2: Lin, name: str) -> torch.Tensor:
        rows = x16.shape[0]
        hmid = self.buf(f"{name}.mid", rows, l0.w.shape[0])
        self.gemm(x16, l0, hmid, act=1)
        out = self.buf(f"{name}.out", rows, l2.w.shape[0], torch.float32)
        self.gemm(hmid, l2, out)
        return out

    def _attn2_const(self, W: dict, ctx16: torch.Tensor, name: str) -> torch.Tensor:
        rows, D = ctx16.shape[0], self.cfg.context_dim
        Cc = W["v"].w.shape[0]
        v = self.buf("a2.v", rows, Cc)
        self.gemm(ctx16[:, :D], W["v"], v)
        if W["va"] is not None:
            v2 = self.buf("a2.v2", rows, Cc)
            self.gemm(ctx16[:, D:], W["va"], v2, res1=v)
            v = v2
        out = self.buf(name, rows, Cc, torch.float32)
        self.gemm(v, W["out"], out)
        return out

    def set_conditioning(self, context: torch.Tensor, y: torch.Tensor):
        T = self.T
        B = context.shape[0]
        from .spec import ACTION_DIM
        want = self.cfg.context_dim + (ACTION_DIM if self.cfg.action_control else 0)
        if context.dim() != 3 or context.shape[1] != 1 or context.shape[2] != want:
            raise NotImplementedError(f"vista_b200: crossattn context must be (B, 1, {want}); got {tuple(context.shape)}")
        ctx16 = self.buf("cond.ctx", B, context.numel() // B)
        ctx16.copy_(context.reshape(B, -1))
        y16 = self.buf("cond.y", B, y.shape[-1])
        y16.copy_(y)
        cond = dict(B=B, label=self._mlp(y16, *self.label_emb, "label"), sp={}, tm={}, pos={})
        tctx16 = self.buf("cond.tctx", B // T, ctx16.shape[1])
        tctx16.copy_(ctx16[::T])
        frames = torch.arange(T, dtype=torch.float32, device=self.dev)
        for t in self.plan.transformers():
            L = self.layers[t.prefix]
            cond["sp"][t.prefix] = self._attn2_const(L["attn2"], ctx16, f"cond.sp.{t.prefix}")
            cond["tm"][t.prefix] = self._attn2_const(L["tattn2"], tctx16, f"cond.tm.{t.prefix}")
            temb = self.buf("cond.temb", T, t.ch)
            ops.timestep_embedding(frames, temb, t.ch)
            cond["pos"][t.prefix] = self._mlp(temb, *L["pos"], f"cond.pos.{t.prefix}")
        self.cond = cond

    def _fuse_stats(self, B, h, w) -> bool:
        return FUSE_GN_STATS and ops.stats_box(w, h, B) is not None

    def _resblock(self, L, x, dst, B, h, w, xp=None, dp=None):
        rb: ResBlockSpec = L["spec"]
        T, hw, M, nb = self.T, h * w, B * h * w, B // self.T
        gi = L["gn_idx"]
        fuse = self._fuse_stats(B, h, w)
        p1 = self.part("rb.h1", M, rb.cout) if fuse else None
        p2 = self.part("rb.xsp", M, rb.cout) if fuse else None
        a1 = self._gn(x, self.buf("rb.a1", M, rb.cin), B, hw, L["gn1"], 1e-5, True, gi, part=xp)
        h1 = self.gemm(a1, L["conv1"], self.buf("rb.h1", M, rb.cout), taps=ops.TAPS_3X3, geom=(w, h, B),
                       rowvec=self.emb_out[:, L["emb_off"]:L["emb_off"] + rb.cout], rv_div=hw, rv_mod=B, stats=p1)
        a2 = self._gn(h1, self.buf("rb.a2", M, rb.cout), B, hw, L["gn2"], 1e-5, True, gi + 1, part=p1)
        xs = x if L["skip"] is None else self.gemm(x, L["skip"], self.buf("rb.xs", M, rb.cout))
        xsp = self.gemm(a2, L["conv2"], self.buf("rb.xsp", M, rb.cout), taps=ops.TAPS_3X3, geom=(w, h, B), res1=xs,
                        stats=p2)
        a3 = self._gn(xsp, self.buf("rb.a1", M, rb.cout), B, hw, L["tgn1"], 1e-5, True, gi + 2, fps=T, part=p2)
        h2 = self._tconv(a3, L["tconv1"], self.buf("rb.h1", M, rb.cout), hw, nb,
                         rowvec=self.emb_out[:, L["embt_off"]:L["embt_off"] + rb.cout], rv_div=hw, rv_mod=B, stats=p1)
        a4 = self._gn(h2, self.buf("rb.a2", M, rb.cout), B, hw, L["tgn2"], 1e-5, True, gi + 3, fps=T, part=p1)
        self._tconv(a4, L["tconv2"], dst, hw, nb, s_acc=1.0 - L["alpha"], res1=xsp, stats=dp if fuse else None)
        return dst

    def _tconv(self, a, lin: Lin, out, hw: int, nb: int, **epi):
        return self.gemm(a, lin, out, taps=ops.TAPS_T3, geom=(hw, self.T, nb), **epi)

    def _svt_tqkv(self, n, L, M: int, Cc: int, nb: int, hw: int):
        return self.gemm(n, L["tqkv"], self.buf("tr.qkv", M, 3 * Cc))

    def _attn_temporal(self, qkv, o, nb: int, hw: int, heads: int, Cc: int):
        return ops.attention_temporal(qkv[:, :Cc], qkv[:, Cc:2 * Cc], qkv[:, 2 * Cc:], o, nb, self.T, hw, heads)

    def _svt(self, L, x, dst, B, h, w, xp=None, dp=None):
        t: SVTSpec = L["spec"]
        T, hw, M, nb, Cc = self.T, h * w, B * h * w, B // self.T, t.ch
        p = t.prefix
        al = L["alpha"]
        xn = self._gn(x, self.buf("tr.n", M, Cc), B, hw, L["norm"], 1e-6, False, L["gn_idx"], part=xp)
        t0 = self.gemm(xn, L["proj_in"], self.buf("tr.t0", M, Cc))
        n = self._ln(t0, self.buf("tr.n", M, Cc), L["ln1"])
        qkv = self.gemm(n, L["qkv"], self.buf("tr.qkv", M, 3 * Cc))
        o = self.buf("tr.o", M, Cc)
        ops.attention_spatial(qkv[:, :Cc], qkv[:, Cc:2 * Cc], qkv[:, 2 * Cc:], o, B, hw, t.heads)
        t1 = self.gemm(o, L["out"], self.buf("tr.t1", M, Cc), res1=t0, rowvec=self.cond["sp"][p], rv_div=hw, rv_mod=B)
        n = self._ln(t1, self.buf("tr.n", M, Cc), L["ln3"])
        g = self.gemm(n, L["ff1"], self.buf("tr.g", M, 4 * Cc))
        t2 = self.gemm(g, L["ff2"], self.buf("tr.t2", M, Cc), res1=t1)
        pos = self.cond["pos"][p]
        n = self._ln(t2, self.buf("tr.n", M, Cc), L["ln_in"], addvec=pos, av_div=hw, av_mod=T)
        g = self.gemm(n, L["ffin1"], self.buf("tr.g", M, 4 * Cc))
        u1 = self.gemm(g, L["ffin2"], self.buf("tr.u1", M, Cc), res1=t2, rowvec=pos, rv_div=hw, rv_mod=T)
        n = self._ln(u1, self.buf("tr.n", M, Cc), L["tln1"])
        qkv = self._svt_tqkv(n, L, M, Cc, nb, hw)
        self._attn_temporal(qkv, o, nb, hw, t.heads, Cc)
        u2 = self.gemm(o, L["tout"], self.buf("tr.t1", M, Cc), res1=u1, rowvec=self.cond["tm"][p], rv_div=T * hw, rv_mod=nb)
        n = self._ln(u2, self.buf("tr.n", M, Cc), L["tln3"])
        g = self.gemm(n, L["tff1"], self.buf("tr.g", M, 4 * Cc))
        x3 = self.gemm(g, L["tff2"], self.buf("tr.u1", M, Cc), s_acc=1.0 - al, res1=u2, s_res1=1.0 - al, res2=t2, s_res2=al)
        self.gemm(x3, L["proj_out"], dst, res1=x, stats=dp if self._fuse_stats(B, h, w) else None)
        return dst

    def _down(self, L, x, dst, B, h, w, dp=None):
        c: ConvSpec = L["spec"]
        ho, wo = (h - 1) // 2 + 1, (w - 1) // 2 + 1
        col = self.buf("down.col", B * ho * wo, 9 * c.cin)
        ops.im2col_s2(x, col, B, h, w, c.cin)
        self.gemm(col, L["conv"], dst, stats=dp if self._fuse_stats(B, ho, wo) else None)
        return dst

    def _up(self, L, x, dst, B, h, w, dp=None):
        c: ConvSpec = L["spec"]
        up = self.buf("up.x", B * 4 * h * w, c.cin)
        ops.upsample2x(x, up, B, h, w, c.cin)
        self.gemm(up, L["conv"], dst, taps=ops.TAPS_3X3, geom=(2 * w, 2 * h, B),
                  stats=dp if self._fuse_stats(B, 2 * h, 2 * w) else None)
        return dst

    def forward(self, x_tokens: torch.Tensor, c_noise: torch.Tensor, cond_mask: Optional[torch.Tensor],
                h: int, w: int, net_out: Optional[torch.Tensor] = None) -> torch.Tensor:
        assert self.cond is not None, "call set_conditioning() first"
        cfg, T = self.cfg, self.T
        B = c_noise.numel()
        assert B % T == 0 and x_tokens.shape[0] == B * h * w and self.cond["B"] == B
        mc, ed = cfg.model_channels, cfg.time_embed_dim
        key = ("gn.stats", B)
        if key not in self._bufs:
            self._bufs[key] = torch.zeros(self.n_gn, B, cfg.num_groups, 2, dtype=torch.float32, device=self.dev)
        self.gn_stats = self._bufs[key]
        if not hasattr(self, "gn_ws"):
            self.gn_ws = ops.GNWorkspace(self.dev)
        self.gn_ws.reserve(ops.groupnorm_scratch(B, h * w, cfg.num_groups))
        temb = ops.timestep_embedding(c_noise, self.buf("emb.t", B, mc), mc)
        e_plain = self._mlp_step(temb, self.time_embed, "emb.plain")
        e_cond = self._mlp_step(temb, self.cond_embed, "emb.cond") if cond_mask is not None else None
        semb = self.buf("emb.silu", B, ed)
        ops.blend_emb(e_plain, e_cond, self.cond["label"], cond_mask, None, semb)
        self.emb_out = self.gemm(semb, self.emb_all, self.buf("emb.out", B, self.emb_total, torch.float32))

        plan = self.plan
        hs: List[Tuple[torch.Tensor, int, int]] = []
        n_out = len(plan.output_blocks)
        ch_in_h = []
        ch = plan.middle_block.layers[-1].cout
        for blk in plan.output_blocks:
            ch_in_h.append(ch)
            ch = blk.layers[0].cout
        sizes = []
        hh, ww = h, w
        in_sizes = []
        for blk in plan.input_blocks:
            if isinstance(blk.layers[0], ConvSpec) and blk.layers[0].kind == "down":
                hh, ww = (hh - 1) // 2 + 1, (ww - 1) // 2 + 1
            in_sizes.append((hh, ww))
        cat_bufs = []
        for j, blk in enumerate(plan.output_blocks):
            sh, sw = in_sizes[len(in_sizes) - 1 - j]
            cskip = plan.skip_channels[len(in_sizes) - 1 - j]
            cat_bufs.append(self.buf(f"cat{j}", B * sh * sw, ch_in_h[j] + cskip))
            sizes.append((sh, sw))

        def run_block(blk, x, dst, bh, bw, xp=None, dp=None):
            n_layers = len(blk.layers)
            filled = False
            for li, layer in enumerate(blk.layers):
                last = li == n_layers - 1
                L = self.layers[layer.prefix]
                if isinstance(layer, ResBlockSpec) or isinstance(layer, SVTSpec):
                    cch = layer.cout if isinstance(layer, ResBlockSpec) else layer.ch
                    fuse = self._fuse_stats(B, bh, bw)
                    d = dst if last else self.buf("blk.tmp%d" % li, B * bh * bw, cch)
                    p_out = (dp if last else self.part("blk.tmp%d" % li, B * bh * bw, cch)) if fuse else None
                    fn = self._resblock if isinstance(layer, ResBlockSpec) else self._svt
                    x = fn(L, x, d, B, bh, bw, xp=xp, dp=p_out)
                    xp = p_out
                    filled = p_out is not None
                elif layer.kind == "down":
                    ho, wo = (bh - 1) // 2 + 1, (bw - 1) // 2 + 1
                    x = self._down(L, x, dst, B, bh, bw, dp=dp)
                    filled = dp is not None and self._fuse_stats(B, ho, wo)
                elif layer.kind == "up":
                    x = self._up(L, x, dst, B, bh, bw, dp=dp)
                    filled = dp is not None and self._fuse_stats(B, 2 * bh, 2 * bw)
                elif layer.kind == "conv_in":
                    if x.stride(0) == IN_PAD:
                        a = x.as_strided((x.shape[0], IN_PAD), (IN_PAD, 1))
                        fuse = dp is not None and self._fuse_stats(B, bh, bw)
                        x = self.gemm(a, L["conv"], dst, taps=ops.TAPS_3X3, geom=(bw, bh, B), stats=dp if fuse else None)
                        filled = fuse
                    else:
                        x = ops.conv3x3_small_cin(x, layer.cin, L["w"], L["b"], dst, B, bh, bw)
            return x, filled

        cat_parts = [self.part(f"cat{j}", cat_bufs[j].shape[0], cat_bufs[j].shape[1]) if self._fuse_stats(B, *sizes[j]) else None
                     for j in range(n_out)]
        cat_ok = [[False, False] for _ in range(n_out)]
        cur, cur_p = x_tokens, None
        hh, ww = h, w
        for i, blk in enumerate(plan.input_blocks):
            j = n_out - 1 - i
            dp = cat_parts[j][:, ch_in_h[j]:] if cat_parts[j] is not None else None
            cur, cat_ok[j][1] = run_block(blk, cur, cat_bufs[j][:, ch_in_h[j]:], hh, ww, xp=cur_p, dp=dp)
            cur_p = dp if cat_ok[j][1] else None
            hh, ww = in_sizes[i]
        dp = cat_parts[0][:, :ch_in_h[0]] if cat_parts[0] is not None else None
        cur, cat_ok[0][0] = run_block(plan.middle_block, cur, cat_bufs[0][:, :ch_in_h[0]], hh, ww, xp=cur_p, dp=dp)
        last_p = None
        for j, blk in enumerate(plan.output_blocks):
            bh, bw = sizes[j]
            if j + 1 < n_out:
                dst = cat_bufs[j + 1][:, :ch_in_h[j + 1]]
                dp = cat_parts[j + 1][:, :ch_in_h[j + 1]] if cat_parts[j + 1] is not None else None
            else:
                cl = blk.layers[-1].cout if not isinstance(blk.layers[-1], SVTSpec) else blk.layers[-1].ch
                dst = self.buf("unet.last", B * bh * bw, cl)
                dp = self.part("unet.last", B * bh * bw, cl) if self._fuse_stats(B, bh, bw) else None
            xp = cat_parts[j] if (cat_parts[j] is not None and all(cat_ok[j])) else None
            cur, ok = run_block(blk, cat_bufs[j], dst, bh, bw, xp=xp, dp=dp)
            if j + 1 < n_out:
                cat_ok[j + 1][0] = ok
            else:
                last_p = dp if ok else None
        M = B * h * w
        a = self._gn(cur, self.buf("out.a", M, mc), B, h * w, self.out_norm, 1e-5, True, self.out_gn_idx, part=last_p)
        if net_out is None:
            net_out = self.buf("unet.out", M, 8, torch.float32)
        self.gemm(a, self.out_conv, net_out, taps=ops.TAPS_3X3, geom=(w, h, B))
        return net_out

    def _mlp_step(self, temb, mlp, name):
        l0, l2 = mlp
        B = temb.shape[0]
        mid = self.gemm(temb, l0, self.buf(name + ".mid", B, l0.w.shape[0]), act=1)
        return self.gemm(mid, l2, self.buf(name + ".out", B, l2.w.shape[0], torch.float32))
```

### vista_b200/vae.py

```python
from __future__ import annotations

from typing import Dict, Optional

import torch
import torch.nn as nn

from . import ops
from .modules import register_param_tree
from .spec import DecoderConfig, DecResBlockSpec, build_decoder_plan, decoder_param_specs
from .unet import Lin
from .weights import conv_weight_to_taps


class DecoderRuntime:
    def __init__(self, cfg: DecoderConfig, sd: Dict[str, torch.Tensor], device):
        self.cfg, self.dev = cfg, torch.device(device)
        self.plan = build_decoder_plan(cfg)
        self._bufs = {}
        self._sd = sd
        self._pack()
        self._sd = None

    def _f32(self, name):
        return self._sd[name].detach().to(self.dev, torch.float32).contiguous()

    def _lin(self, prefix) -> Lin:
        w = self._sd[f"{prefix}.weight"].detach().to(self.dev, torch.float32)
        w = conv_weight_to_taps(w) if w.dim() > 2 else w
        return Lin(w.to(torch.float16).contiguous(), self._f32(f"{prefix}.bias"), ops.pick_tile_n(w.shape[0]))

    def _norm(self, prefix):
        return self._f32(f"{prefix}.weight"), self._f32(f"{prefix}.bias")

    def _pack(self):
        sd = self._sd
        self.n_gn = 0
        self.res: Dict[str, dict] = {}

        def pack_res(rb: DecResBlockSpec):
            p, t = rb.prefix, f"{rb.prefix}.time_stack"
            self.res[p] = dict(spec=rb, gn1=self._norm(f"{p}.norm1"), conv1=self._lin(f"{p}.conv1"),
                               gn2=self._norm(f"{p}.norm2"), conv2=self._lin(f"{p}.conv2"),
                               skip=self._lin(f"{p}.nin_shortcut") if rb.has_skip else None,
                               tgn1=self._norm(f"{t}.in_layers.0"), tconv1=self._lin(f"{t}.in_layers.2"),
                               tgn2=self._norm(f"{t}.out_layers.0"), tconv2=self._lin(f"{t}.out_layers.3"),
                               alpha=float(torch.sigmoid(sd[f"{p}.mix_factor"].float()).item()), gn_idx=self.n_gn)
            self.n_gn += 4

        self.conv_in_w, self.conv_in_b = self._f32("conv_in.weight"), self._f32("conv_in.bias")
        pack_res(self.plan.mid[0])
        a = "mid.attn_1"
        wq = self._lin(f"{a}.q")
        self.attn = dict(norm=self._norm(f"{a}.norm"), q=wq, k=self._lin(f"{a}.k"),
                         v_w=conv_weight_to_taps(sd[f"{a}.v.weight"].detach().to(self.dev, torch.float32)).to(torch.float16).contiguous(),
                         v_b=self._f32(f"{a}.v.bias"), proj=self._lin(f"{a}.proj_out"), gn_idx=self.n_gn)
        self.n_gn += 1
        pack_res(self.plan.mid[1])
        self.ups = {}
        for blocks, up, ch in self.plan.levels:
            for rb in blocks:
                pack_res(rb)
            if up is not None:
                self.ups[up] = self._lin(up)
        self.norm_out = self._norm("norm_out")
        self.norm_out_idx = self.n_gn
        self.n_gn += 1
        ow = conv_weight_to_taps(self._f32("conv_out.weight"))
        w8 = torch.zeros(8, ow.shape[1], dtype=torch.float16, device=self.dev)
        w8[: ow.shape[0]] = ow.to(torch.float16)
        b8 = torch.zeros(8, dtype=torch.float32, device=self.dev)
        b8[: ow.shape[0]] = self._f32("conv_out.bias")
        self.out_conv = Lin(w8.contiguous(), b8, 32)
        self.tmix_w = self._f32("conv_out.time_mix_conv.weight").reshape(self.cfg.out_ch, self.cfg.out_ch, 3).contiguous()
        self.tmix_b = self._f32("conv_out.time_mix_conv.bias")

    def buf(self, name, rows, cols, dtype=torch.float16):
        key = (name, rows, cols, dtype)
        t = self._bufs.get(key)
        if t is None:
            t = self._bufs[key] = torch.empty(rows, cols, dtype=dtype, device=self.dev)
        return t

    def gemm(self, a, lin: Lin, out, **kw):
        return ops.gemm(a, lin.w, out, bias=lin.b, tile_n=lin.tile_n, **kw)

    def _gn(self, x, y, T, hw, norm, eps, idx, fps=1, part=None, silu=True):
        stats = self.gn_stats[idx, : T // fps]
        if part is None:
            return ops.groupnorm(x, y, T, hw, norm[0], norm[1], eps, silu, stats, frames_per_stat=fps,
                                 groups=self.cfg.num_groups, ws=self.gn_ws)
        ops.groupnorm_from_partials(part, T, hw, norm[0].numel(), eps, stats, fps, self.cfg.num_groups)
        return ops.groupnorm_apply(x, y, T, hw, norm[0], norm[1], silu, stats, fps, self.cfg.num_groups)

    def part(self, name: str, tokens: int, cols: int) -> torch.Tensor:
        key = ("part." + name, tokens, cols)
        t = self._bufs.get(key)
        if t is None:
            t = self._bufs[key] = torch.zeros(-(-tokens // 128) * 4, cols, 2, dtype=torch.float32, device=self.dev)
        return t

    def _fuse_stats(self, T, h, w) -> bool:
        from .unet import FUSE_GN_STATS
        return FUSE_GN_STATS and ops.stats_box(w, h, T) is not None

    def _resblock(self, L, x, T, h, w, name, xp=None):
        rb: DecResBlockSpec = L["spec"]
        hw, M, gi = h * w, T * h * w, L["gn_idx"]
        fuse = self._fuse_stats(T, h, w)
        p1 = self.part("d.h1", M, rb.cout) if fuse else None
        p2 = self.part("d.xsp", M, rb.cout) if fuse else None
        pd = self.part(name, M, rb.cout) if fuse else None
        a1 = self._gn(x, self.buf("d.a1", M, rb.cin), T, hw, L["gn1"], 1e-6, gi, part=xp)
        h1 = self.gemm(a1, L["conv1"], self.buf("d.h1", M, rb.cout), taps=ops.TAPS_3X3, geom=(w, h, T), stats=p1)
        a2 = self._gn(h1, self.buf("d.a2", M, rb.cout), T, hw, L["gn2"], 1e-6, gi + 1, part=p1)
        xs = x if L["skip"] is None else self.gemm(x, L["skip"], self.buf("d.xs", M, rb.cout))
        xsp = self.gemm(a2, L["conv2"], self.buf("d.xsp", M, rb.cout), taps=ops.TAPS_3X3, geom=(w, h, T), res1=xs, stats=p2)
        a3 = self._gn(xsp, self.buf("d.a1", M, rb.cout), T, hw, L["tgn1"], 1e-5, gi + 2, fps=T, part=p2)
        h2 = self.gemm(a3, L["tconv1"], self.buf("d.h1", M, rb.cout), taps=ops.TAPS_T3, geom=(hw, T, 1), stats=p1)
        a4 = self._gn(h2, self.buf("d.a2", M, rb.cout), T, hw, L["tgn2"], 1e-5, gi + 3, fps=T, part=p1)
        out = self.buf(name, M, rb.cout)
        self.gemm(a4, L["tconv2"], out, taps=ops.TAPS_T3, geom=(hw, T, 1), s_acc=L["alpha"], res1=xsp, stats=pd)
        return out, pd

    def _attn(self, x, T, h, w, xp=None):
        A = self.attn
        Cc, hw, M = x.shape[1], h * w, T * h * w
        assert hw % 64 == 0, "decoder attention needs h*w to be a multiple of 64"
        y = self.buf("d.attn_y", M, Cc)
        yp = self.part("d.attn_y", M, Cc) if self._fuse_stats(T, h, w) else None
        xn = self._gn(x, self.buf("d.a1", M, Cc), T, hw, A["norm"], 1e-6, A["gn_idx"], part=xp, silu=False)
        q = self.gemm(xn, A["q"], self.buf("d.q", M, Cc))
        k = self.gemm(xn, A["k"], self.buf("d.k", M, Cc))
        o = self.buf("d.o", M, Cc)
        s = self.buf("d.s", hw, hw, torch.float32)
        p = self.buf("d.p", hw, hw)
        vT = self.buf("d.vT", Cc, hw)
        for f in range(T):
            rows = slice(f * hw, (f + 1) * hw)
            ops.gemm(A["v_w"], xn[rows], vT)
            ops.gemm(q[rows], k[rows], s, s_acc=float(Cc) ** -0.5)
            ops.softmax_rows(s, p)
            ops.gemm(p, vT, o[rows], bias=A["v_b"])
        self.gemm(o, A["proj"], y, res1=x, stats=yp)
        return y, yp

    def forward(self, z_tokens: torch.Tensor, T: int, h: int, w: int, out: torch.Tensor, out_frame0: int = 0,
                blend: Optional[torch.Tensor] = None, skip_frames: int = 0, out_u8: Optional[torch.Tensor] = None,
                keep_f32_from: int = -1) -> torch.Tensor:
        cfg = self.cfg
        if not hasattr(self, "gn_stats") or self.gn_stats.shape[1] < T:
            self._bufs.setdefault(("gn.retired",), []).append(getattr(self, "gn_stats", None))
            self.gn_stats = torch.zeros(self.n_gn, T, cfg.num_groups, 2, dtype=torch.float32, device=self.dev)
        if not hasattr(self, "gn_ws"):
            self.gn_ws = ops.GNWorkspace(self.dev)
        up_total = 2 ** (len(cfg.ch_mult) - 1)
        self.gn_ws.reserve(ops.groupnorm_scratch(T, h * w * up_total * up_total, cfg.num_groups))
        M = T * h * w
        x = ops.conv3x3_small_cin(z_tokens, cfg.z_channels, self.conv_in_w, self.conv_in_b,
                                  self.buf("d.in", M, self.plan.block_in), T, h, w)
        x, xp = self._resblock(self.res[self.plan.mid[0].prefix], x, T, h, w, "d.r0")
        x, xp = self._attn(x, T, h, w, xp)
        x, xp = self._resblock(self.res[self.plan.mid[1].prefix], x, T, h, w, "d.r1", xp)
        for li, (blocks, up, ch) in enumerate(self.plan.levels):
            for bi, rb in enumerate(blocks):
                x, xp = self._resblock(self.res[rb.prefix], x, T, h, w, f"d.r{bi % 2}", xp)
            if up is not None:
                xu = ops.upsample2x(x, self.buf("d.up", T * 4 * h * w, ch), T, h, w, ch)
                h, w = 2 * h, 2 * w
                xp = self.part("d.upc", T * h * w, ch) if self._fuse_stats(T, h, w) else None
                x = self.gemm(xu, self.ups[up], self.buf("d.upc", T * h * w, ch), taps=ops.TAPS_3X3, geom=(w, h, T), stats=xp)
        M = T * h * w
        a = self._gn(x, self.buf("d.a1", M, self.plan.final_ch), T, h * w, self.norm_out, 1e-6, self.norm_out_idx, part=xp)
        y = self.gemm(a, self.out_conv, self.buf("d.y", M, 8, torch.float32), taps=ops.TAPS_3X3, geom=(w, h, T))
        if out_u8 is not None:
            ops.time_mix_small_u8(y, self.tmix_w, self.tmix_b, out, out_u8, blend, T, h * w, cfg.out_ch, out_frame0,
                                  skip_frames, keep_f32_from)
        else:
            ops.time_mix_small(y, self.tmix_w, self.tmix_b, out, blend, T, h * w, cfg.out_ch, out_frame0, skip_frames)
        return out


def decode_first_stage(rt: DecoderRuntime, z: torch.Tensor, scale_factor: float = 0.18215, n_samples: Optional[int] = 14,
                       overlap: int = 3, u8: bool = False) -> torch.Tensor:
    F_, zc, h, w = z.shape
    n_samples = F_ if n_samples is None else n_samples
    up = 2 ** (len(rt.cfg.ch_mult) - 1)
    out = torch.empty(F_, rt.cfg.out_ch, h * up, w * up, dtype=torch.float32, device=z.device)
    zs = (z.float() / scale_factor).contiguous()
    if u8:
        out8 = torch.empty(F_, h * up, w * up, rt.cfg.out_ch, dtype=torch.uint8, device=z.device)
        chunks = _decode_chunks(F_, n_samples, overlap)
        for ci, (f0, n, o0, nov) in enumerate(chunks):
            tok = rt.buf("d.z", n * h * w, 8)
            tok.zero_()
            ops.nchw_to_tokens(zs[f0:f0 + n].contiguous(), tok, n, zc, h, w)
            blend = None
            if nov:
                blend = torch.zeros(n, dtype=torch.int32, device=z.device)
                blend[:nov] = 1
            keep = n if ci + 1 == len(chunks) else max(0, chunks[ci + 1][2] - o0)
            rt.forward(tok, n, h, w, out, out_frame0=o0, blend=blend, out_u8=out8, keep_f32_from=keep)
        return out8

    def run(frames: torch.Tensor, out_frame0: int, n_overlap: int):
        T = frames.shape[0]
        tok = rt.buf("d.z", T * h * w, 8)
        tok.zero_()
        ops.nchw_to_tokens(frames.contiguous(), tok, T, zc, h, w)
        blend = None
        if n_overlap:
            blend = torch.zeros(T, dtype=torch.int32, device=z.device)
            blend[:n_overlap] = 1
        rt.forward(tok, T, h, w, out, out_frame0=out_frame0, blend=blend)

    for f0, n, o0, nov in _decode_chunks(F_, n_samples, overlap):
        run(zs[f0:f0 + n], o0, nov)
    return out


class EncoderRuntime(DecoderRuntime):

    def __init__(self, cfg, sd: Dict[str, torch.Tensor], device, post=None):
        from .spec import build_encoder_plan
        self.cfg, self.dev = cfg, torch.device(device)
        self._post = post
        self.levels, self.mid_ch = build_encoder_plan(cfg)
        self._bufs = {}
        self._sd = sd
        self._pack()
        self._sd = None

    def _pack(self):
        self.n_gn = 0
        self.res = {}

        def pack_res(rb: DecResBlockSpec):
            p = rb.prefix
            self.res[p] = dict(spec=rb, gn1=self._norm(f"{p}.norm1"), conv1=self._lin(f"{p}.conv1"),
                               gn2=self._norm(f"{p}.norm2"), conv2=self._lin(f"{p}.conv2"),
                               skip=self._lin(f"{p}.nin_shortcut") if rb.has_skip else None, gn_idx=self.n_gn)
            self.n_gn += 2

        self.conv_in_w, self.conv_in_b = self._f32("conv_in.weight"), self._f32("conv_in.bias")
        self.downs = {}
        for blocks, down, ch in self.levels:
            for rb in blocks:
                pack_res(rb)
            if down is not None:
                self.downs[down] = self._lin(down)
        pack_res(DecResBlockSpec("mid.block_1", self.mid_ch, self.mid_ch))
        a, sd = "mid.attn_1", self._sd
        self.attn = dict(norm=self._norm(f"{a}.norm"), q=self._lin(f"{a}.q"), k=self._lin(f"{a}.k"),
                         v_w=conv_weight_to_taps(sd[f"{a}.v.weight"].detach().to(self.dev, torch.float32)).to(torch.float16).contiguous(),
                         v_b=self._f32(f"{a}.v.bias"), proj=self._lin(f"{a}.proj_out"), gn_idx=self.n_gn)
        self.n_gn += 1
        pack_res(DecResBlockSpec("mid.block_2", self.mid_ch, self.mid_ch))
        self.norm_out = self._norm("norm_out")
        self.norm_out_idx = self.n_gn
        self.n_gn += 1
        ow = conv_weight_to_taps(self._f32("conv_out.weight"))
        ob = self._f32("conv_out.bias")
        if getattr(self, "_post", None) is not None:
            pw, pb = (t.to(self.dev, torch.float32) for t in self._post)
            ow, ob = pw @ ow, pw @ ob + pb
        assert ow.shape[0] <= 8
        w8 = torch.zeros(8, ow.shape[1], dtype=torch.float16, device=self.dev)
        w8[: ow.shape[0]] = ow.to(torch.float16)
        b8 = torch.zeros(8, dtype=torch.float32, device=self.dev)
        b8[: ow.shape[0]] = ob
        self.out_conv = Lin(w8.contiguous(), b8, 32)
        self.n_moments = ow.shape[0]

    def _fuse_stats(self, n, h, w) -> bool:
        return False

    def _enc_resblock(self, L, x, n, h, w, name):
        rb: DecResBlockSpec = L["spec"]
        hw, M, gi = h * w, n * h * w, L["gn_idx"]
        a1 = self._gn(x, self.buf("e.a1", M, rb.cin), n, hw, L["gn1"], 1e-6, gi)
        h1 = self.gemm(a1, L["conv1"], self.buf("e.h1", M, rb.cout), taps=ops.TAPS_3X3, geom=(w, h, n))
        a2 = self._gn(h1, self.buf("e.a2", M, rb.cout), n, hw, L["gn2"], 1e-6, gi + 1)
        xs = x if L["skip"] is None else self.gemm(x, L["skip"], self.buf("e.xs", M, rb.cout))
        return self.gemm(a2, L["conv2"], self.buf(name, M, rb.cout), taps=ops.TAPS_3X3, geom=(w, h, n), res1=xs)

    def forward(self, x_tokens: torch.Tensor, n: int, h: int, w: int) -> torch.Tensor:
        cfg = self.cfg
        if not hasattr(self, "gn_stats") or self.gn_stats.shape[1] < n:
            self._bufs.setdefault(("gn.retired",), []).append(getattr(self, "gn_stats", None))
            self.gn_stats = torch.zeros(self.n_gn, n, cfg.num_groups, 2, dtype=torch.float32, device=self.dev)
        if not hasattr(self, "gn_ws"):
            self.gn_ws = ops.GNWorkspace(self.dev)
        self.gn_ws.reserve(ops.groupnorm_scratch(n, h * w, cfg.num_groups))
        x = ops.conv3x3_small_cin(x_tokens, cfg.in_channels, self.conv_in_w, self.conv_in_b,
                                  self.buf("e.in", n * h * w, cfg.ch), n, h, w)
        for blocks, down, ch in self.levels:
            for bi, rb in enumerate(blocks):
                x = self._enc_resblock(self.res[rb.prefix], x, n, h, w, f"e.r{bi % 2}")
            if down is not None:
                ho, wo = (h - 2) // 2 + 1, (w - 2) // 2 + 1
                col = ops.im2col_s2_asym(x, self.buf("e.col", n * ho * wo, 9 * ch), n, h, w, ch)
                h, w = ho, wo
                x = self.gemm(col, self.downs[down], self.buf("e.down", n * h * w, ch))
        x = self._enc_resblock(self.res["mid.block_1"], x, n, h, w, "e.m0")
        x, _ = self._attn(x, n, h, w)
        x = self._enc_resblock(self.res["mid.block_2"], x, n, h, w, "e.m1")
        M = n * h * w
        a = ops.groupnorm(x, self.buf("e.a1", M, self.mid_ch), n, h * w, self.norm_out[0], self.norm_out[1], 1e-6,
                          True, self.gn_stats[self.norm_out_idx, :n], groups=cfg.num_groups, ws=self.gn_ws)
        return self.gemm(a, self.out_conv, self.buf("e.y", M, 8, torch.float32), taps=ops.TAPS_3X3, geom=(w, h, n))


def encode_first_stage(rt: EncoderRuntime, x: torch.Tensor, scale_factor: float = 0.18215,
                       n_samples: Optional[int] = None, noise: Optional[torch.Tensor] = None) -> torch.Tensor:
    n_all, cin, H, W = x.shape
    n_samples = n_all if n_samples is None else n_samples
    down = 2 ** (len(rt.cfg.ch_mult) - 1)
    zc = rt.cfg.z_channels
    out = torch.empty(n_all, zc, H // down, W // down, dtype=torch.float32, device=x.device)
    for i in range(0, n_all, n_samples):
        xs = x[i:i + n_samples].float().contiguous()
        n = xs.shape[0]
        tok = rt.buf("e.x", n * H * W, 8)
        tok.zero_()
        ops.nchw_to_tokens(xs, tok, n, cin, H, W)
        mom_tok = rt.forward(tok, n, H, W)
        mom = torch.empty(n, 8, H // down, W // down, dtype=torch.float32, device=x.device)
        ops.tokens_to_nchw(mom_tok, mom, n, 8, H // down, W // down)
        mean, logvar = mom[:, :zc], mom[:, zc:2 * zc]
        z = mean if noise is None else mean + torch.exp(0.5 * logvar.clamp(-30.0, 20.0)) * noise[i:i + n].to(mean)
        out[i:i + n] = z * scale_factor
    return out


class Encoder(nn.Module):

    def __init__(self, *, ch, ch_mult=(1, 2, 4, 8), num_res_blocks, attn_resolutions=(), dropout=0.0, resamp_with_conv=True,
                 in_channels=3, resolution=256, z_channels=4, double_z=True, use_linear_attn=False, attn_type="vanilla",
                 **ignore_kwargs):
        super().__init__()
        from .spec import EncoderConfig, encoder_param_specs
        bad = [k for k, v in dict(attn_resolutions=len(list(attn_resolutions)) != 0, dropout=dropout != 0.0,
                                  resamp_with_conv=not resamp_with_conv, use_linear_attn=use_linear_attn,
                                  attn_type=attn_type != "vanilla", double_z=not double_z).items() if v]
        if bad:
            raise NotImplementedError(f"vista_b200.Encoder: unsupported option(s) {bad}")
        self.b200_config = EncoderConfig(ch=ch, in_channels=in_channels, ch_mult=tuple(ch_mult),
                                         num_res_blocks=num_res_blocks, z_channels=z_channels, double_z=double_z)
        register_param_tree(self, encoder_param_specs(self.b200_config))
        self._runtime = None
        self.register_load_state_dict_post_hook(lambda module, keys: setattr(module, "_runtime", None))

    def _apply(self, fn, *args, **kwargs):
        before = tuple((p.device, p.dtype) for p in self.parameters())
        out = super()._apply(fn, *args, **kwargs)
        if tuple((p.device, p.dtype) for p in self.parameters()) != before:
            self._runtime = None
        return out

    def runtime(self, device) -> EncoderRuntime:
        if torch.device(device).type != "cuda":
            raise RuntimeError("vista_b200 runs on CUDA (sm_90a) only; there is no CPU fallback")
        if self._runtime is None:
            self._runtime = EncoderRuntime(self.b200_config, self.state_dict(), device)
        return self._runtime

    def forward(self, x: torch.Tensor) -> torch.Tensor:
        rt = self.runtime(x.device)
        n, cin, H, W = x.shape
        down = 2 ** (len(rt.cfg.ch_mult) - 1)
        tok = rt.buf("e.x", n * H * W, 8)
        tok.zero_()
        ops.nchw_to_tokens(x.float().contiguous(), tok, n, cin, H, W)
        mom_tok = rt.forward(tok, n, H, W)
        mom = torch.empty(n, 8, H // down, W // down, dtype=torch.float32, device=x.device)
        ops.tokens_to_nchw(mom_tok, mom, n, 8, H // down, W // down)
        return mom[:, : rt.n_moments]


def _decode_chunks(F_: int, n_samples: int, overlap: int):
    chunks = []
    if overlap == 0 and n_samples < F_:
        raise NotImplementedError("decode_first_stage: overlap = 0 with more than one chunk is ill-defined in the reference")
    if overlap < n_samples:
        pos, first, prev_len = overlap, True, overlap
        while pos < F_:
            cur = min(n_samples - overlap, F_ - pos)
            chunks.append((pos - prev_len, prev_len + cur, pos - overlap, 0 if first else overlap))
            pos += cur
            prev_len = min(overlap, cur)
            first = False
    else:
        pos = 0
        while pos < F_:
            cur = min(n_samples, F_ - pos)
            chunks.append((pos, cur, pos, 0))
            pos += cur
    return chunks


def decode_first_stage_parallel(rt: DecoderRuntime, z: torch.Tensor, scale_factor: float = 0.18215,
                                n_samples: Optional[int] = 14, overlap: int = 3, group=None) -> torch.Tensor:
    import torch.distributed as dist
    world, rank = dist.get_world_size(group), dist.get_rank(group)
    F_, zc, h, w = z.shape
    n_samples = F_ if n_samples is None else n_samples
    up = 2 ** (len(rt.cfg.ch_mult) - 1)
    out = torch.empty(F_, rt.cfg.out_ch, h * up, w * up, dtype=torch.float32, device=z.device)
    zs = (z.float() / scale_factor).contiguous()
    chunks = _decode_chunks(F_, n_samples, overlap)
    if any(nov > n or o0 != f0 for f0, n, o0, nov in chunks):
        raise NotImplementedError("decode_first_stage_parallel: chunks shorter than the overlap")
    to_global = (lambda r: r) if group is None else (lambda r: dist.get_global_rank(group, r))
    bufs = []
    for i, (f0, n, o0, nov) in enumerate(chunks):
        cb = rt.__dict__.setdefault("_chunk_out", {}).get((i, n))
        if cb is None:
            cb = rt._chunk_out[(i, n)] = torch.empty(n, rt.cfg.out_ch, h * up, w * up, dtype=torch.float32, device=z.device)
        bufs.append(cb)
        if i % world == rank:
            tok = rt.buf("d.z", n * h * w, 8)
            tok.zero_()
            ops.nchw_to_tokens(zs[f0:f0 + n].contiguous(), tok, n, zc, h, w)
            rt.forward(tok, n, h, w, cb)
    for i, (f0, n, o0, nov) in enumerate(chunks):
        if world > 1:
            dist.broadcast(bufs[i], src=to_global(i % world), group=group)
        if nov:
            out[o0:o0 + nov] = 0.5 * (out[o0:o0 + nov] + bufs[i][:nov])
        out[o0 + nov:o0 + n] = bufs[i][nov:]
    return out


class VideoDecoder(nn.Module):

    def __init__(self, *, ch, out_ch, ch_mult=(1, 2, 4, 8), num_res_blocks, attn_resolutions=(), dropout=0.0,
                 resamp_with_conv=True, in_channels=3, resolution=256, z_channels=4, give_pre_end=False, tanh_out=False,
                 use_linear_attn=False, attn_type="vanilla", video_kernel_size=3, alpha: float = 0.0,
                 merge_strategy: str = "learned", time_mode: str = "conv-only", **ignorekwargs):
        super().__init__()
        vks = [3, 1, 1] if video_kernel_size is None else video_kernel_size
        bad = [n for n, v in dict(attn_resolutions=len(list(attn_resolutions)) != 0, dropout=dropout != 0.0,
                                  resamp_with_conv=not resamp_with_conv, give_pre_end=give_pre_end, tanh_out=tanh_out,
                                  use_linear_attn=use_linear_attn, attn_type=attn_type != "vanilla",
                                  video_kernel_size=isinstance(vks, int) or list(vks) != [3, 1, 1],
                                  merge_strategy=merge_strategy != "learned", time_mode=time_mode != "conv-only").items() if v]
        if bad:
            raise NotImplementedError(f"vista_b200.VideoDecoder: unsupported option(s) {bad}")
        self.b200_config = DecoderConfig(ch=ch, out_ch=out_ch, ch_mult=tuple(ch_mult), num_res_blocks=num_res_blocks,
                                         z_channels=z_channels)
        register_param_tree(self, decoder_param_specs(self.b200_config))
        self._runtime = None
        self.register_load_state_dict_post_hook(lambda module, keys: setattr(module, "_runtime", None))

    def _apply(self, fn, *args, **kwargs):
        before = tuple((p.device, p.dtype) for p in self.parameters())
        out = super()._apply(fn, *args, **kwargs)
        if tuple((p.device, p.dtype) for p in self.parameters()) != before:
            self._runtime = None
        return out

    def runtime(self, device) -> DecoderRuntime:
        if torch.device(device).type != "cuda":
            raise RuntimeError("vista_b200 runs on CUDA (sm_90a) only; there is no CPU fallback")
        if self._runtime is None:
            self._runtime = DecoderRuntime(self.b200_config, self.state_dict(), device)
        return self._runtime

    def forward(self, z: torch.Tensor, timesteps: Optional[int] = None, **kwargs) -> torch.Tensor:
        rt = self.runtime(z.device)
        T, zc, h, w = z.shape
        assert timesteps in (None, T), "one clip per call (decode_first_stage passes timesteps == batch)"
        up = 2 ** (len(rt.cfg.ch_mult) - 1)
        out = torch.empty(T, rt.cfg.out_ch, h * up, w * up, dtype=torch.float32, device=z.device)
        tok = rt.buf("d.z", T * h * w, 8)
        tok.zero_()
        ops.nchw_to_tokens(z.float().contiguous(), tok, T, zc, h, w)
        return rt.forward(tok, T, h, w, out)

    def get_last_layer(self, skip_time_mix=False, **kwargs):
        return self.conv_out.time_mix_conv.weight if not skip_time_mix else self.conv_out.weight


def bench_decode(dcfg: DecoderConfig, rand_sd, dev, T: int, h: int, w: int, reps: int = 1, parallel: bool = False) -> float:
    import os
    sd = rand_sd(decoder_param_specs(dcfg))
    frame_sharded = parallel and os.environ.get("VISTA_B200_SHARDED_DECODE") == "1"
    if frame_sharded:
        from .sharded import ShardedDecoderRuntime, decode_first_stage_sharded
        rt = ShardedDecoderRuntime(dcfg, sd, dev)
    else:
        rt = DecoderRuntime(dcfg, sd, dev)
    z = torch.randn(T, dcfg.z_channels, h, w, device=dev) * 0.18215
    if parallel:
        import torch.distributed as dist
        dist.broadcast(z, src=0)
    if frame_sharded:
        fn = lambda: decode_first_stage_sharded(rt, z)
    else:
        fn = (lambda: decode_first_stage_parallel(rt, z)) if parallel else (lambda: decode_first_stage(rt, z))
    fn()
    torch.cuda.synchronize()
    e0, e1 = torch.cuda.Event(enable_timing=True), torch.cuda.Event(enable_timing=True)
    e0.record()
    for _ in range(reps):
        fn()
    e1.record()
    torch.cuda.synchronize()
    return e0.elapsed_time(e1) / 1e3 / reps
```

Before: 1.304.

## Add ping-pong warpgroup GEMM schedule for small-K, wide-N linear layers

Adds a ping-pong schedule to the tap GEMM kernel. The two consumer warpgroups take alternate output tiles, each computing the full 128-row tile, and an ordering barrier lets one warpgroup's epilogue overlap the other's MMA mainloop. A heuristic (gemm_config) turns this on for single-tap GEMMs with K<=640 and wide N or residual/rowvec loads, and also changes tile_n choices. Residual and rowvec loads are hoisted ahead of the shared-memory staging. The cost is larger epilogue staging buffers, which leave fewer pipeline stages, plus more instantiated kernel variants and more register pressure from a doubled accumulator.

New measurement: 1.305 (median of 6 runs). No clear change (+0.1%).

```diff
diff --git a/include/vista_b200.h b/include/vista_b200.h
--- a/include/vista_b200.h
+++ b/include/vista_b200.h
@@ -45,6 +45,7 @@
   int64_t stats_ld;
   int32_t stats_col0;
   int32_t h_pad;
+  int32_t schedule;
 } b200v_gemm_desc;
 
 int b200v_gemm(const b200v_gemm_desc* d, void* stream);
diff --git a/vista_b200/clip.py b/vista_b200/clip.py
--- a/vista_b200/clip.py
+++ b/vista_b200/clip.py
@@ -28,7 +28,7 @@
         return self._sd[self.prefix + name].detach().to(self.dev, dtype).contiguous()
 
     def _lin(self, w: torch.Tensor, b: Optional[torch.Tensor]) -> Lin:
-        return Lin(w.to(torch.float16).contiguous(), b, ops.pick_tile_n(w.shape[0]))
+        return Lin(w.to(torch.float16).contiguous(), b, ops.gemm_config(*w.shape)[0])
 
     def _norm(self, p):
         return self._t(f"{p}.weight"), self._t(f"{p}.bias")
@@ -64,7 +64,7 @@
         return t
 
     def gemm(self, a, lin: Lin, out, **kw):
-        return ops.gemm(a, lin.w, out, bias=lin.b, tile_n=lin.tile_n, **kw)
+        return ops.gemm(a, lin.w, out, bias=lin.b, **kw)
 
     def forward(self, x: torch.Tensor, antialias: bool = True) -> torch.Tensor:
         cfg, C = self.cfg, self.cfg.width
diff --git a/vista_b200/csrc/gemm_pp_32_128.cu b/vista_b200/csrc/gemm_pp_32_128.cu
--- /dev/null
+++ b/vista_b200/csrc/gemm_pp_32_128.cu
@@ -0,0 +1,6 @@
+#include "gemm_tc.cuh"
+
+namespace vb {
+template const GemmKern* gemm_variants<32, true>();
+template const GemmKern* gemm_variants<128, true>();
+}
diff --git a/vista_b200/csrc/gemm_pp_64_96.cu b/vista_b200/csrc/gemm_pp_64_96.cu
--- /dev/null
+++ b/vista_b200/csrc/gemm_pp_64_96.cu
@@ -0,0 +1,6 @@
+#include "gemm_tc.cuh"
+
+namespace vb {
+template const GemmKern* gemm_variants<64, true>();
+template const GemmKern* gemm_variants<96, true>();
+}
diff --git a/vista_b200/csrc/gemm_tc.cu b/vista_b200/csrc/gemm_tc.cu
--- a/vista_b200/csrc/gemm_tc.cu
+++ b/vista_b200/csrc/gemm_tc.cu
@@ -9,6 +9,10 @@
 extern template const GemmKern* gemm_variants<192>();
 extern template const GemmKern* gemm_variants<224>();
 extern template const GemmKern* gemm_variants<256>();
+extern template const GemmKern* gemm_variants<32, true>();
+extern template const GemmKern* gemm_variants<64, true>();
+extern template const GemmKern* gemm_variants<96, true>();
+extern template const GemmKern* gemm_variants<128, true>();
 }
 
 extern "C" int b200v_gemm(const b200v_gemm_desc* d, void* stream_) {
@@ -19,6 +23,9 @@
   VB_REQUIRE(d->ntaps >= 1 && d->ntaps <= 9, "b200v_gemm: ntaps=%d out of range", d->ntaps);
   VB_REQUIRE(d->N > 0 && d->N % 8 == 0, "b200v_gemm: N=%d must be a multiple of 8", d->N);
   VB_REQUIRE(d->tile_n >= 32 && d->tile_n <= 256 && d->tile_n % 32 == 0, "b200v_gemm: tile_n=%d invalid", d->tile_n);
+  VB_REQUIRE(d->schedule == 0 || d->schedule == 1, "b200v_gemm: schedule=%d invalid", d->schedule);
+  VB_REQUIRE(d->schedule == 0 || d->tile_n <= 128, "b200v_gemm: the ping-pong schedule needs tile_n <= 128 (got %d)",
+             d->tile_n);
   VB_REQUIRE(d->lda % 8 == 0 && d->ldo % 8 == 0, "b200v_gemm: lda/ldo must be multiples of 8");
   VB_REQUIRE(d->act >= 0 && d->act <= 3, "b200v_gemm: act=%d invalid", d->act);
   VB_REQUIRE(!(d->act == 2 && (d->tile_n % 64 != 0 || d->N % d->tile_n != 0 || d->out_f32)),
@@ -88,7 +95,8 @@
   p.n_tiles = (d->N + d->tile_n - 1) / d->tile_n;
   p.stage_bytes = kABytes + ((d->tile_n * 128 + 1023) / 1024) * 1024;
   constexpr int kMaxSmem = 227 * 1024;
-  p.nstages = (kMaxSmem - 2048 - kStagingBytes) / p.stage_bytes;
+  const bool pp = d->schedule == 1;
+  p.nstages = (kMaxSmem - 2048 - staging_bytes(pp)) / p.stage_bytes;
   if (p.nstages > kMaxStages) p.nstages = kMaxStages;
   const long long kMaxLd = (1ll << 31) - 1;
   VB_REQUIRE(d->ldo * (d->out_f32 ? 4 : 2) <= kMaxLd && d->ld_rowvec * 4 <= kMaxLd && d->ld_res1 * 2 <= kMaxLd &&
@@ -116,7 +124,7 @@
                p.BW, p.BH, p.BB, d->W, d->H);
   }
 
-  const int smem_bytes = 1024 + 1024 + p.nstages * p.stage_bytes + kStagingBytes;
+  const int smem_bytes = 1024 + 1024 + p.nstages * p.stage_bytes + staging_bytes(pp);
   int variant = d->bf16 ? 12 : 7;
   if (d->stats) {
     variant = 9 + (d->rowvec ? 2 : (d->res1 ? 1 : 0));
@@ -131,16 +139,21 @@
   static const GemmKern* const kByWidth[8] = {gemm_variants<32>(),  gemm_variants<64>(),  gemm_variants<96>(),
                                               gemm_variants<128>(), gemm_variants<160>(), gemm_variants<192>(),
                                               gemm_variants<224>(), gemm_variants<256>()};
+  static const GemmKern* const kPingPong[4] = {gemm_variants<32, true>(), gemm_variants<64, true>(),
+                                               gemm_variants<96, true>(), gemm_variants<128, true>()};
   static bool attr_set[64] = {false};
   if (vb::first_use_on_device(attr_set)) {
     for (int w = 0; w < 8; ++w)
-      for (int i = 0; i < kGemmVariants; ++i)
+      for (int i = 0; i < kGemmVariants; ++i) {
         VB_CHECK_CUDA(cudaFuncSetAttribute(kByWidth[w][i], cudaFuncAttributeMaxDynamicSharedMemorySize, kMaxSmem));
+        if (w < 4)
+          VB_CHECK_CUDA(cudaFuncSetAttribute(kPingPong[w][i], cudaFuncAttributeMaxDynamicSharedMemorySize, kMaxSmem));
+      }
   }
   const long long total = (long long)p.m_tiles * p.n_tiles;
   int grid = device_sm_count();
   if (total < grid) grid = (int)total;
-  const GemmKern k = kByWidth[d->tile_n / 32 - 1][variant];
+  const GemmKern k = (pp ? kPingPong : kByWidth)[d->tile_n / 32 - 1][variant];
   k<<<grid, kGemmThreads, smem_bytes, stream>>>(tmA, tmB, p);
   VB_CHECK_CUDA(cudaGetLastError());
   return 0;
diff --git a/vista_b200/csrc/gemm_tc.cuh b/vista_b200/csrc/gemm_tc.cuh
--- a/vista_b200/csrc/gemm_tc.cuh
+++ b/vista_b200/csrc/gemm_tc.cuh
@@ -7,9 +7,9 @@
 
 constexpr int kMaxStages = 8;
 constexpr int kABytes = 128 * 64 * 2;
-constexpr int kStageBufBytes = 64 * 32 * 4;
-constexpr int kStagingBytes = 2 * 2 * kStageBufBytes;
 constexpr int kGemmThreads = 384;
+__host__ __device__ constexpr int stage_buf_bytes(bool pp) { return (pp ? 128 : 64) * 32 * 4; }
+__host__ __device__ constexpr int staging_bytes(bool pp) { return 2 * 2 * stage_buf_bytes(pp); }
 
 struct TGParams {
   int a_mode;
@@ -61,14 +61,16 @@
     wgmma_ss<TN, BF16>(acc, adesc + (uint64_t)(2 * kk), bdesc + (uint64_t)(2 * kk), (overwrite && kk == 0) ? 0 : 1);
 }
 
-template <int TN, int ACT_, bool RV_, int NRES_, bool GEN, bool STATS = false, bool BF16 = false>
+template <int TN, int ACT_, bool RV_, int NRES_, bool GEN, bool STATS = false, bool BF16 = false, bool PP = false>
 __global__ void __launch_bounds__(kGemmThreads, 1)
 tapgemm_kernel(const __grid_constant__ CUtensorMap tmA, const __grid_constant__ CUtensorMap tmB, const TGParams p) {
+  static_assert(!PP || TN <= 128, "ping-pong: the 128-row accumulator of a warpgroup holds at most 128 columns");
   extern __shared__ uint8_t smem_raw[];
   const uint32_t raw = smem_u32(smem_raw);
   uint8_t* smem = smem_raw + (((raw + 1023u) & ~1023u) - raw);
   uint64_t* full = reinterpret_cast<uint64_t*>(smem);
   uint64_t* empty = full + kMaxStages;
+  uint64_t* order = empty + kMaxStages;
   uint8_t* stages = smem + 1024;
 
   const int warp = threadIdx.x >> 5, lane = threadIdx.x & 31;
@@ -78,8 +80,10 @@
   if (threadIdx.x == 0) {
     for (int i = 0; i < p.nstages; ++i) {
       mbar_init(&full[i], 1);
-      mbar_init(&empty[i], 8);
-    }
+      mbar_init(&empty[i], PP ? 4 : 8);
+    }
+    mbar_init(&order[0], 4);
+    mbar_init(&order[1], 4);
     fence_barrier_init();
   }
   if (warp == 8 && lane == 0) {
@@ -141,24 +145,41 @@
   const char* r2p = reinterpret_cast<const char*>(p.res2);
   const uint64_t desc0 = make_desc_sw128(smem_u32(stages), 16, 1024);
   const uint32_t stage_step = (uint32_t)p.stage_bytes >> 4;
-  const uint32_t stg0 = smem_u32(stages + p.nstages * p.stage_bytes) + wg * 2 * kStageBufBytes;
+  constexpr int kBuf = stage_buf_bytes(PP);
+  const uint32_t stg0 = smem_u32(stages + p.nstages * p.stage_bytes) + wg * 2 * kBuf;
   const int g = lane >> 2, c = lane & 3;
   const int rh = wq & 1, chh = wq >> 1;
   const int ch = lane & 3, rsub = lane >> 2;
+  constexpr int NH = PP ? 2 : 1;
+  const int srow0 = PP ? 32 * wq : 32 * rh;
+  const int quarter = PP ? wq : 2 * wg + rh;
   int stage = 0;
   uint32_t phase = 0;
+  uint32_t ord_phase = 0;
   uint32_t gcount = 0;
 
-  float acc[TN / 2];
-  for (int tile = blockIdx.x; tile < total_tiles; tile += gridDim.x) {
+  float acc[NH][TN / 2];
+  int jt = 0;
+  for (int tile = blockIdx.x; tile < total_tiles; tile += gridDim.x, ++jt) {
+    if (PP && (jt & 1) != wg) {
+      const int s = stage + KC;
+      phase ^= (uint32_t)(s / p.nstages) & 1u;
+      stage = s % p.nstages;
+      continue;
+    }
+    if (PP && jt > 0) {
+      mbar_wait(&order[wg], ord_phase, 4);
+      ord_phase ^= 1;
+    }
     const int m_blk = tile / p.n_tiles, n_blk = tile - m_blk * p.n_tiles;
     int prev = -1;
     for (int kc = 0; kc < KC; ++kc) {
       mbar_wait(&full[stage], phase, 3);
-      const uint64_t ad = desc0 + (uint64_t)(stage * stage_step + wg * 512);
+      const uint64_t ad = desc0 + (uint64_t)(stage * stage_step + (PP ? 0 : wg * 512));
       const uint64_t bd = desc0 + (uint64_t)(stage * stage_step + (kABytes >> 4));
       wgmma_fence();
-      issue_kchunk<TN, BF16>(acc, ad, bd, kc == 0);
+#pragma unroll
+      for (int h = 0; h < NH; ++h) issue_kchunk<TN, BF16>(acc[h], ad + (uint64_t)(h * 512), bd, kc == 0);
       wgmma_commit();
       if (prev >= 0) {
         wgmma_wait<1>();
@@ -170,11 +191,13 @@
         phase ^= 1;
       }
     }
+    if (PP && lane == 0) mbar_arrive(&order[wg ^ 1]);
     wgmma_wait<0>();
     if (lane == 0) mbar_arrive(&empty[prev]);
-    fence_regs(acc);
-
-    const int r_own = wg * 64 + rh * 32 + lane;
+#pragma unroll
+    for (int h = 0; h < NH; ++h) fence_regs(acc[h]);
+
+    const int r_own = (PP ? 0 : wg * 64) + srow0 + lane;
     int token_own, valid_own;
     if (p.a_mode == 0) {
       token_own = m_blk * 128 + r_own;
@@ -206,50 +229,77 @@
       if (k >= G) break;
       const int c0 = k * 32;
       if (n_out_base + c0 >= n_out_total) break;
-      const uint32_t stg = stg0 + (gcount & 1) * kStageBufBytes;
+      const uint32_t stg = stg0 + (gcount & 1) * kBuf;
       ++gcount;
-      float f[16];
-#pragma unroll
-      for (int j = 0; j < 16; ++j) f[j] = acc[16 * k + j];
-      if (act == 2) {
-        float gt[16];
-        const int kg = (half >> 5) + k;
-#pragma unroll
-        for (int j = 0; j < 16; ++j) gt[j] = 0.f;
-#pragma unroll
-        for (int q = 0; q < TN / 32; ++q)
-          if (q == kg) {
-#pragma unroll
-            for (int j = 0; j < 16; ++j) gt[j] = acc[16 * q + j];
-          }
-        const int nb = n_blk * TN + c0;
+      float4 rv[NH][4];
+      uint2 u1[NH][4], u2[NH][4];
+      auto load_operands = [&](int hh) {
+        const int n = n_out_base + c0 + (PP ? hh : chh) * 16 + ch * 4;
+        const bool n_ok = n + 4 <= n_out_total;
+        const char* rvbase = reinterpret_cast<const char*>(p.rowvec) + (long long)n * 4;
+#pragma unroll
+        for (int i = 0; i < 4; ++i) {
+          const bool ok = n_ok && ((vrows >> (8 * i)) & 1u);
+          rv[hh][i] = make_float4(0.f, 0.f, 0.f, 0.f);
+          u1[hh][i] = make_uint2(0, 0);
+          u2[hh][i] = make_uint2(0, 0);
+          if (has_rv && ok)
+            rv[hh][i] = __ldg(reinterpret_cast<const float4*>(rvbase + (long long)rvrow[i] * p.ld_rowvec_b));
+          if (has_r1 && ok)
+            u1[hh][i] = __ldg(reinterpret_cast<const uint2*>(r1p + ((long long)n * 2 + (long long)tok[i] * p.ld_res1_b)));
+          if (has_r2 && ok)
+            u2[hh][i] = __ldg(reinterpret_cast<const uint2*>(r2p + ((long long)n * 2 + (long long)tok[i] * p.ld_res2_b)));
+        }
+      };
+      load_operands(0);
+#pragma unroll
+      for (int h = 0; h < NH; ++h) {
+        float f[16];
+#pragma unroll
+        for (int j = 0; j < 16; ++j) f[j] = acc[h][16 * k + j];
+        if (act == 2) {
+          float gt[16];
+          const int kg = (half >> 5) + k;
+#pragma unroll
+          for (int j = 0; j < 16; ++j) gt[j] = 0.f;
+#pragma unroll
+          for (int q = 0; q < TN / 32; ++q)
+            if (q == kg) {
+#pragma unroll
+              for (int j = 0; j < 16; ++j) gt[j] = acc[h][16 * q + j];
+            }
+          const int nb = n_blk * TN + c0;
+#pragma unroll
+          for (int ii = 0; ii < 4; ++ii) {
+            float2 bv = make_float2(0.f, 0.f), bg = make_float2(0.f, 0.f);
+            if (has_bias) {
+              bv = __ldg(reinterpret_cast<const float2*>(p.bias + nb + 8 * ii + 2 * c));
+              bg = __ldg(reinterpret_cast<const float2*>(p.bias + nb + half + 8 * ii + 2 * c));
+            }
+            f[4 * ii + 0] = geglu_fast(f[4 * ii + 0] + bv.x, gt[4 * ii + 0] + bg.x);
+            f[4 * ii + 1] = geglu_fast(f[4 * ii + 1] + bv.y, gt[4 * ii + 1] + bg.y);
+            f[4 * ii + 2] = geglu_fast(f[4 * ii + 2] + bv.x, gt[4 * ii + 2] + bg.x);
+            f[4 * ii + 3] = geglu_fast(f[4 * ii + 3] + bv.y, gt[4 * ii + 3] + bg.y);
+          }
+        }
 #pragma unroll
         for (int ii = 0; ii < 4; ++ii) {
-          float2 bv = make_float2(0.f, 0.f), bg = make_float2(0.f, 0.f);
-          if (has_bias) {
-            bv = __ldg(reinterpret_cast<const float2*>(p.bias + nb + 8 * ii + 2 * c));
-            bg = __ldg(reinterpret_cast<const float2*>(p.bias + nb + half + 8 * ii + 2 * c));
-          }
-          f[4 * ii + 0] = geglu_fast(f[4 * ii + 0] + bv.x, gt[4 * ii + 0] + bg.x);
-          f[4 * ii + 1] = geglu_fast(f[4 * ii + 1] + bv.y, gt[4 * ii + 1] + bg.y);
-          f[4 * ii + 2] = geglu_fast(f[4 * ii + 2] + bv.x, gt[4 * ii + 2] + bg.x);
-          f[4 * ii + 3] = geglu_fast(f[4 * ii + 3] + bv.y, gt[4 * ii + 3] + bg.y);
-        }
-      }
-#pragma unroll
-      for (int ii = 0; ii < 4; ++ii) {
-        const int chunk = 2 * ii + (c >> 1), sub = (c & 1) * 8;
-#pragma unroll
-        for (int hr = 0; hr < 2; ++hr) {
-          const int row = wq * 16 + g + 8 * hr;
-          asm volatile("st.shared.v2.f32 [%0], {%1, %2};" ::"r"(stg + row * 128 + ((chunk ^ (row & 7)) << 4) + sub),
-                       "f"(f[4 * ii + 2 * hr]), "f"(f[4 * ii + 2 * hr + 1])
-                       : "memory");
+          const int chunk = 2 * ii + (c >> 1), sub = (c & 1) * 8;
+#pragma unroll
+          for (int hr = 0; hr < 2; ++hr) {
+            const int row = 64 * h + wq * 16 + g + 8 * hr;
+            asm volatile("st.shared.v2.f32 [%0], {%1, %2};" ::"r"(stg + row * 128 + ((chunk ^ (row & 7)) << 4) + sub),
+                         "f"(f[4 * ii + 2 * hr]), "f"(f[4 * ii + 2 * hr + 1])
+                         : "memory");
+          }
         }
       }
       asm volatile("bar.sync %0, 128;" ::"r"(1 + wg) : "memory");
-      {
-        const int n = n_out_base + c0 + chh * 16 + ch * 4;
+#pragma unroll
+      for (int hh = 0; hh < NH; ++hh) {
+        const int chx = PP ? hh : chh;
+        if (hh > 0) load_operands(hh);
+        const int n = n_out_base + c0 + chx * 16 + ch * 4;
         const bool n_ok = n + 4 <= n_out_total;
         float4 bs = make_float4(0.f, 0.f, 0.f, 0.f);
         float sa = 1.0f;
@@ -261,26 +311,15 @@
           }
         }
         char* obase = reinterpret_cast<char*>(p.out) + (long long)n * out_es;
-        const char* r1base = r1p + (long long)n * 2;
-        const char* r2base = r2p + (long long)n * 2;
-        const char* rvbase = reinterpret_cast<const char*>(p.rowvec) + (long long)n * 4;
         float cs[4] = {0.f, 0.f, 0.f, 0.f}, cq[4] = {0.f, 0.f, 0.f, 0.f};
-        float4 v[4], rv[4];
-        uint2 u1[4], u2[4];
+        float4 v[4];
 #pragma unroll
         for (int i = 0; i < 4; ++i) {
-          const int row = rh * 32 + i * 8 + rsub;
-          const int chunk = chh * 4 + ch;
+          const int row = srow0 + i * 8 + rsub;
+          const int chunk = chx * 4 + ch;
           asm volatile("ld.shared.v4.f32 {%0, %1, %2, %3}, [%4];"
                        : "=f"(v[i].x), "=f"(v[i].y), "=f"(v[i].z), "=f"(v[i].w)
                        : "r"(stg + row * 128 + ((chunk ^ (row & 7)) << 4)));
-          const bool ok = n_ok && ((vrows >> (8 * i)) & 1u);
-          rv[i] = make_float4(0.f, 0.f, 0.f, 0.f);
-          u1[i] = make_uint2(0, 0);
-          u2[i] = make_uint2(0, 0);
-          if (has_rv && ok) rv[i] = __ldg(reinterpret_cast<const float4*>(rvbase + (long long)rvrow[i] * p.ld_rowvec_b));
-          if (has_r1 && ok) u1[i] = __ldg(reinterpret_cast<const uint2*>(r1base + (long long)tok[i] * p.ld_res1_b));
-          if (has_r2 && ok) u2[i] = __ldg(reinterpret_cast<const uint2*>(r2base + (long long)tok[i] * p.ld_res2_b));
         }
 #pragma unroll
         for (int i = 0; i < 4; ++i) {
@@ -288,16 +327,16 @@
           float4 o = v[i];
           if (act != 2) {
             o.x = fmaf(o.x, sa, bs.x); o.y = fmaf(o.y, sa, bs.y); o.z = fmaf(o.z, sa, bs.z); o.w = fmaf(o.w, sa, bs.w);
-            if (has_rv) { o.x += rv[i].x; o.y += rv[i].y; o.z += rv[i].z; o.w += rv[i].w; }
+            if (has_rv) { o.x += rv[hh][i].x; o.y += rv[hh][i].y; o.z += rv[hh][i].z; o.w += rv[hh][i].w; }
             if (act == 1) { o.x = silu_f(o.x); o.y = silu_f(o.y); o.z = silu_f(o.z); o.w = silu_f(o.w); }
             if (!GEN && act == 3) { o.x = gelu_erf_fast(o.x); o.y = gelu_erf_fast(o.y); o.z = gelu_erf_fast(o.z); o.w = gelu_erf_fast(o.w); }
             if (has_r1) {
-              const float2 a = unpack2(u1[i].x, bf16), b = unpack2(u1[i].y, bf16);
+              const float2 a = unpack2(u1[hh][i].x, bf16), b = unpack2(u1[hh][i].y, bf16);
               o.x = fmaf(p.s_res1, a.x, o.x); o.y = fmaf(p.s_res1, a.y, o.y);
               o.z = fmaf(p.s_res1, b.x, o.z); o.w = fmaf(p.s_res1, b.y, o.w);
             }
             if (has_r2) {
-              const float2 a = unpack2(u2[i].x, bf16), b = unpack2(u2[i].y, bf16);
+              const float2 a = unpack2(u2[hh][i].x, bf16), b = unpack2(u2[hh][i].y, bf16);
               o.x = fmaf(p.s_res2, a.x, o.x); o.y = fmaf(p.s_res2, a.y, o.y);
               o.z = fmaf(p.s_res2, b.x, o.z); o.w = fmaf(p.s_res2, b.y, o.w);
             }
@@ -325,7 +364,7 @@
             }
           }
           if (rsub == 0 && n_ok) {
-            float* dst = p.stats + (((long long)m_blk * 4 + wg * 2 + rh) * p.stats_ld + p.stats_col0 + n) * 2;
+            float* dst = p.stats + (((long long)m_blk * 4 + quarter) * p.stats_ld + p.stats_col0 + n) * 2;
             *reinterpret_cast<float4*>(dst) = make_float4(cs[0], cq[0], cs[1], cq[1]);
             *reinterpret_cast<float4*>(dst + 4) = make_float4(cs[2], cq[2], cs[3], cq[3]);
           }
@@ -338,16 +377,16 @@
 using GemmKern = void (*)(const CUtensorMap, const CUtensorMap, const TGParams);
 constexpr int kGemmVariants = 13;
 
-template <int TN>
+template <int TN, bool PP = false>
 const GemmKern* gemm_variants() {
   static const GemmKern v[kGemmVariants] = {
-      tapgemm_kernel<TN, 0, false, 0, false>,       tapgemm_kernel<TN, 0, false, 1, false>,
-      tapgemm_kernel<TN, 0, false, 2, false>,       tapgemm_kernel<TN, 0, true, 0, false>,
-      tapgemm_kernel<TN, 0, true, 1, false>,        tapgemm_kernel<TN, 1, false, 0, false>,
-      tapgemm_kernel<TN, 2, false, 0, false>,       tapgemm_kernel<TN, 0, true, 2, true>,
-      tapgemm_kernel<TN, 3, false, 0, false>,       tapgemm_kernel<TN, 0, false, 0, false, true>,
-      tapgemm_kernel<TN, 0, false, 1, false, true>, tapgemm_kernel<TN, 0, true, 0, false, true>,
-      tapgemm_kernel<TN, 0, true, 2, true, false, true>};
+      tapgemm_kernel<TN, 0, false, 0, false, false, false, PP>, tapgemm_kernel<TN, 0, false, 1, false, false, false, PP>,
+      tapgemm_kernel<TN, 0, false, 2, false, false, false, PP>, tapgemm_kernel<TN, 0, true, 0, false, false, false, PP>,
+      tapgemm_kernel<TN, 0, true, 1, false, false, false, PP>,  tapgemm_kernel<TN, 1, false, 0, false, false, false, PP>,
+      tapgemm_kernel<TN, 2, false, 0, false, false, false, PP>, tapgemm_kernel<TN, 0, true, 2, true, false, false, PP>,
+      tapgemm_kernel<TN, 3, false, 0, false, false, false, PP>, tapgemm_kernel<TN, 0, false, 0, false, true, false, PP>,
+      tapgemm_kernel<TN, 0, false, 1, false, true, false, PP>,  tapgemm_kernel<TN, 0, true, 0, false, true, false, PP>,
+      tapgemm_kernel<TN, 0, true, 2, true, false, true, PP>};
   return v;
 }
 
diff --git a/vista_b200/lib.py b/vista_b200/lib.py
--- a/vista_b200/lib.py
+++ b/vista_b200/lib.py
@@ -12,7 +12,7 @@
 CSRC = os.path.join(PKG_DIR, "csrc")
 LIB_PATH = os.path.join(PKG_DIR, "libvista_b200.so")
 SOURCES = ["host.cu", "gemm_tc.cu", "gemm_tn_32_256.cu", "gemm_tn_64_224.cu", "gemm_tn_96_192.cu", "gemm_tn_128_160.cu",
-           "attn_tc.cu", "misc.cu", "glue.cu", "peer.cu", "clip.cu"]
+           "gemm_pp_32_128.cu", "gemm_pp_64_96.cu", "attn_tc.cu", "misc.cu", "glue.cu", "peer.cu", "clip.cu"]
 NVCC_FLAGS = ["-gencode", "arch=compute_90a,code=sm_90a", "-lineinfo", "-O3", "-std=c++17",
               "-Xcompiler", "-fPIC", "--expt-relaxed-constexpr"]
 
@@ -74,6 +74,7 @@
         ("res2", C.c_void_p), ("ld_res2", C.c_int64), ("s_res2", C.c_float),
         ("s_acc", C.c_float),
         ("stats", C.c_void_p), ("stats_ld", C.c_int64), ("stats_col0", C.c_int32), ("h_pad", C.c_int32),
+        ("schedule", C.c_int32),
     ]
 
 
diff --git a/vista_b200/ops.py b/vista_b200/ops.py
--- a/vista_b200/ops.py
+++ b/vista_b200/ops.py
@@ -122,13 +122,20 @@
     return best
 
 
+def gemm_config(N: int, K: int, taps: int = 1, act: int = 0, loads: bool = False) -> Tuple[int, int]:
+    pp = act != 2 and taps == 1 and K <= 640 and (N >= 640 or loads)
+    if not pp:
+        return pick_tile_n(N, act == 2), 0
+    return next((tn for tn in (128, 96, 64) if N % tn == 0), 128), 1
+
+
 def gemm(a: torch.Tensor, w: torch.Tensor, out: torch.Tensor, *, taps: Sequence[Tuple[int, int]] = TAPS_1,
          geom: Optional[Tuple[int, int, int]] = None, bias: Optional[torch.Tensor] = None,
          rowvec: Optional[torch.Tensor] = None, rv_div: int = 1, rv_mod: int = 1,
          res1: Optional[torch.Tensor] = None, s_res1: float = 1.0,
          res2: Optional[torch.Tensor] = None, s_res2: float = 1.0,
          s_acc: float = 1.0, act: int = 0, tile_n: Optional[int] = None, cin: Optional[int] = None,
-         stats: Optional[torch.Tensor] = None, h_pad: int = 0) -> torch.Tensor:
+         stats: Optional[torch.Tensor] = None, h_pad: int = 0, schedule: Optional[int] = None) -> torch.Tensor:
     tokens, lda = _rows(a)
     if h_pad:
         assert geom is not None and tokens == geom[2] * (geom[1] + 2 * h_pad) * geom[0]
@@ -151,7 +158,9 @@
     for i, (dh, dw) in enumerate(taps):
         d.dh[i], d.dw[i] = dh, dw
     d.b, d.N = w.data_ptr(), N
-    d.tile_n = tile_n if tile_n is not None else pick_tile_n(N, act == 2)
+    cfg_tn, cfg_sched = gemm_config(N, K, ntaps, act, rowvec is not None or res1 is not None)
+    d.tile_n = tile_n if tile_n is not None else cfg_tn
+    d.schedule = schedule if schedule is not None else (cfg_sched if d.tile_n == cfg_tn else 0)
     d.bf16 = 1 if a.dtype == torch.bfloat16 else 0
     _, ldo = _rows(out)
     d.out, d.ldo, d.out_f32, d.act = out.data_ptr(), ldo, int(out.dtype == torch.float32), act
diff --git a/vista_b200/sharded.py b/vista_b200/sharded.py
--- a/vista_b200/sharded.py
+++ b/vista_b200/sharded.py
@@ -234,7 +234,8 @@
         lin = L["tqkv"]
         sub = self._tap_w.get(("qkv", lin.w.data_ptr()))
         if sub is None:
-            sub = (Lin(lin.w[:Cc], None, ops.pick_tile_n(Cc)), Lin(lin.w[Cc:], None, ops.pick_tile_n(2 * Cc)))
+            sub = (Lin(lin.w[:Cc], None, ops.gemm_config(Cc, lin.w.shape[1])[0]),
+                   Lin(lin.w[Cc:], None, ops.gemm_config(2 * Cc, lin.w.shape[1])[0]))
             self._tap_w[("qkv", lin.w.data_ptr())] = sub
         qkv = self.buf("tr.qkv", M, 3 * Cc)
         send = self._kv_recv(nb, hw, Cc)[1] if self._peer_on(nb) else self.buf("kv.send", nb * self.T_pad * hw, 2 * Cc)
diff --git a/vista_b200/unet.py b/vista_b200/unet.py
--- a/vista_b200/unet.py
+++ b/vista_b200/unet.py
@@ -47,9 +47,10 @@
     def _lin(self, prefix, geglu=False, bias=True, tile_n=None) -> Lin:
         w = self._sd[f"{prefix}.weight"].detach().to(self.dev, torch.float32)
         b = self._f32(f"{prefix}.bias") if bias and f"{prefix}.bias" in self._sd else None
+        taps = w[0, 0].numel() if w.dim() > 2 else 1
         if w.dim() > 2:
             w = conv_weight_to_taps(w)
-        tn = tile_n or ops.pick_tile_n(w.shape[0], geglu)
+        tn = tile_n or ops.gemm_config(w.shape[0], w.shape[1], taps, 2 if geglu else 0)[0]
         if geglu:
             w, b = permute_geglu(w, b, tn)
         return Lin(w.to(torch.float16).contiguous(), b, tn, geglu)
@@ -93,7 +94,7 @@
                 def qkv(a):
                     w = torch.cat([sd[f"{a}.to_q.weight"], sd[f"{a}.to_k.weight"], sd[f"{a}.to_v.weight"]], 0)
                     w = w.detach().to(self.dev, torch.float16).contiguous()
-                    return Lin(w, None, ops.pick_tile_n(w.shape[0]))
+                    return Lin(w, None, ops.gemm_config(*w.shape)[0])
 
                 L = dict(spec=layer, norm=self._norm(f"{p}.norm"), proj_in=self._lin(f"{p}.proj_in"),
                          ln1=self._norm(f"{s}.norm1"), qkv=qkv(f"{s}.attn1"), out=self._lin(f"{s}.attn1.to_out.0"),
@@ -117,11 +118,11 @@
                     b = self._f32(f"{layer.prefix}.bias")
                     self.layers[layer.prefix] = dict(spec=layer, w=w, b=b,
                                                      conv=Lin(conv_weight_to_taps(wp).to(torch.float16).contiguous(), b,
-                                                              ops.pick_tile_n(w.shape[0])))
+                                                              ops.gemm_config(w.shape[0], 9 * IN_PAD, 9)[0]))
                 else:
                     self.layers[layer.prefix] = dict(spec=layer, conv=self._lin(layer.prefix))
-        self.emb_all = Lin(torch.cat(emb_w, 0).to(torch.float16).contiguous(), torch.cat(emb_b, 0).contiguous(),
-                           ops.pick_tile_n(off))
+        emb_w = torch.cat(emb_w, 0).to(torch.float16).contiguous()
+        self.emb_all = Lin(emb_w, torch.cat(emb_b, 0).contiguous(), ops.gemm_config(*emb_w.shape)[0])
         self.emb_total = off
         self.out_norm = self._norm("out.0")
         self.out_gn_idx = self.n_gn
@@ -144,7 +145,8 @@
         return t
 
     def gemm(self, a, lin: Lin, out, **kw):
-        return ops.gemm(a, lin.w, out, bias=lin.b, tile_n=lin.tile_n, act=2 if lin.geglu else kw.pop("act", 0), **kw)
+        return ops.gemm(a, lin.w, out, bias=lin.b, tile_n=lin.tile_n if lin.geglu else None,
+                        act=2 if lin.geglu else kw.pop("act", 0), **kw)
 
     def _gn(self, x, y, B, hw, norm, eps, silu, idx, fps=1, part=None):
         if fps != 1:
diff --git a/vista_b200/vae.py b/vista_b200/vae.py
--- a/vista_b200/vae.py
+++ b/vista_b200/vae.py
@@ -26,8 +26,10 @@
 
     def _lin(self, prefix) -> Lin:
         w = self._sd[f"{prefix}.weight"].detach().to(self.dev, torch.float32)
+        taps = w[0, 0].numel() if w.dim() > 2 else 1
         w = conv_weight_to_taps(w) if w.dim() > 2 else w
-        return Lin(w.to(torch.float16).contiguous(), self._f32(f"{prefix}.bias"), ops.pick_tile_n(w.shape[0]))
+        return Lin(w.to(torch.float16).contiguous(), self._f32(f"{prefix}.bias"),
+                   ops.gemm_config(w.shape[0], w.shape[1], taps)[0])
 
     def _norm(self, prefix):
         return self._f32(f"{prefix}.weight"), self._f32(f"{prefix}.bias")
@@ -82,7 +84,7 @@
         return t
 
     def gemm(self, a, lin: Lin, out, **kw):
-        return ops.gemm(a, lin.w, out, bias=lin.b, tile_n=lin.tile_n, **kw)
+        return ops.gemm(a, lin.w, out, bias=lin.b, **kw)
 
     def _gn(self, x, y, T, hw, norm, eps, idx, fps=1, part=None, silu=True):
         stats = self.gn_stats[idx, : T // fps]
```
